# set-soft/ComfyUI-FLOAT_Optimized

Measured on AMD Instinct MI355X. Metric: 512x512 frames/sec end-to-end audio->video @50 ODE steps, higher is better.
Workload: dtype fp16; 1 GPU; configs[1]: 10 s audio + 512x512 portrait in HBM -> 250 frames in pinned host memory; appearance encoder + wav2vec2 audio encoder + FMT sampling (50 Euler evaluations/window, CFG a=2.0 e=1.0) + decode + D2H, through InferenceAgent.infer_device (the product call); nfe=51, frames_per_clip=250, fmt_dtype=fp16, dec_dtype=fp16, decode_batch=32, hip_graph=True, parallelism=replicas x1 (one clip per GPU), stage_overlap=off

## Files before the change

### comfyui-float_optimized_amd/csrc/fmt_api.hip

```cpp
#include <math.h>
#include <stdlib.h>

#include "fmt_gemm.hpp"
#include "fmt_kernels.hpp"
#include "fmt_rb_kernels.hpp"
#include "fmt_big_kernels.hpp"
#include "fmt_launch.hpp"

namespace {

struct Blk {
  Lin qkv, proj, fc1, fc2;
};

constexpr int kMaxTok = 80;
constexpr int kMaxSteps = 1024;

}

struct float_fmt {
  float_fmt_cfg_t cfg;
  DevicePool pool;
  int D, ntok, Mpad, Kc, Ntot, Kx;
  int Bmax = 1;
  Lin x_embed, t0, t2, c_embed, adaln_all, final_lin;
  std::vector<Blk> blk;
  float* pos = nullptr;
  float* freqs = nullptr;
  u16 *cond16, *sc16, *h16, *hfin16, *qkv16, *att16, *hid16, *xin16, *tsin16, *th16;
  float *ccond, *xres, *xcur, *temb, *vout;
  unsigned long long* sat = nullptr;
  float* slab = nullptr;
  float *wa_c, *we_c, *prev_x, *prev_wa, *prev_we, *x0_c;
  float* wr_c = nullptr;
  int method = 0;
  FmtTune tune;
  int n_cu = 0;
  struct MegaPlan {
    MegaStage* dev = nullptr;
    int nstage = 0, bc = 0, tried = 0;
    MegaCtx ctx{};
  } mega[5];
  unsigned* mega_sync = nullptr;
  unsigned* mega_err_host = nullptr;
  u16* mega_ws = nullptr;
  float* kbuf = nullptr;
  float* modall = nullptr;
  int Mmod = 0;
  size_t mod_zs = 0;
  struct GraphKey {
    int nfe, bc, we_len, method;
    int prio;
    float a, r, e;
    bool operator==(const GraphKey& o) const { return memcmp(this, &o, sizeof(GraphKey)) == 0; }
  };
  struct GraphEntry {
    GraphKey key;
    hipGraphExec_t exec[kFmtMaxClips + 1];
    uint64_t used;
  };
  std::vector<GraphEntry> graphs;
  uint64_t graph_clock = 0;
  hipStream_t cap_stream = nullptr;
  int cap_prio = 0;
  struct {
    const float *wr, *wa, *we, *noise;
    float* r_d;
    int T, we_len, nfe, include_r, next, n_chunks, B;
    int first = 0, total = 0;
    const float *hist_x = nullptr, *hist_wa = nullptr, *hist_we = nullptr;
    float a, r, e;
    std::vector<float> ts;
    bool active = false;
    bool ragged = false;
    FmtClipTab<const float*> rg_wr, rg_wa, rg_we, rg_noise;
    FmtClipTab<float*> rg_rd;
    int rg_win[kFmtMaxClips];
  } job;
};

#include "fmt_mega.hpp"

namespace {

int dev_copy2d(float* dst, size_t dpitch, const float* src, size_t spitch, int width, int rows, hipStream_t s) {
  if (width <= 0 || rows <= 0) return FLOAT_OK;
  hipLaunchKernelGGL(fmt_copy_kernel, dim3((unsigned)(((size_t)rows * width + 255) / 256)), dim3(256), 0, s, dst, dpitch, src, spitch, width, rows);
  FH_CHECK_HIP(hipGetLastError());
  return FLOAT_OK;
}
int dev_copy(float* dst, const float* src, size_t n, hipStream_t s) { return dev_copy2d(dst, n, src, n, (int)n, 1, s); }
int dev_zero(float* dst, size_t n, hipStream_t s) { return dev_copy2d(dst, n, nullptr, n, (int)n, 1, s); }
int copy_or_zero(float* dst, const float* src, size_t n, hipStream_t s) { return src ? dev_copy(dst, src, n, s) : dev_zero(dst, n, s); }

FmtLaunch launch_ctx(const float_fmt* h, hipStream_t s) {
  return FmtLaunch{h->tune, s, h->sat, h->xres, h->slab, h->h16, h->qkv16, h->att16, h->D, h->ntok, h->Ntot, h->Mpad, h->cfg.heads,
                   h->cfg.attn_window};
}


constexpr int kScSteps = 64;

static int stream_priority(hipStream_t s) {
  int prio = 0;
  if (hipStreamGetPriority(s, &prio) != hipSuccess) {
    (void)hipGetLastError();
    prio = 0;
  }
  return prio;
}

template <class T>
int run_mod_all(float_fmt* h, int M, int e0, int n, hipStream_t s) {
  const int D = h->D;
  const FmtTune& tn = h->tune;
  FH_REQUIRE(n >= 1 && n <= kScSteps, "modulation batch of %d evaluations (max %d)", n, kScSteps);
  const int prio = (s == h->cap_stream && s) ? h->cap_prio : stream_priority(s);
  const bool big = !T::is32 && tn.wide && prio == 0 && big_shape_ok(tn, n * M, h->adaln_all.N, h->adaln_all.K, h->n_cu);
  hipLaunchKernelGGL((fmt_silu_c_kernel<T>), dim3((M * D / 8 + 255) / 256, n), dim3(256), 0, s, h->sc16, h->temb + (size_t)e0 * D,
                     h->ccond, M, D, (size_t)h->Mpad * D, big ? M : 0, h->sat);
  h->mod_zs = big ? (size_t)M * h->Ntot : (size_t)h->Mmod * h->Ntot;
  if constexpr (!T::is32) {
    if (big) return launch_big4<T>(h->sc16, h->adaln_all, h->modall, n * M, h->Ntot, h->n_cu, s);
  }
  GemmArgs g = base_args(h->sc16, h->adaln_all, M);
  g.sat = h->sat, g.out_f32 = h->modall, g.ldo = h->Ntot, g.zcount = n;
  const bool dma = (tn.wide_variant == 6 || tn.wide_variant == 7) && (M + 15) / 16 > 4 && dma_shape_ok(g, 320);
  g.zgroup = tn.zgroup > 0 ? tn.zgroup : (dma ? 2 : 4);
  g.a_zstride = (size_t)h->Mpad * D;
  g.o_zstride = (size_t)h->Mmod * h->Ntot;
  if constexpr (!T::is32) {
    if (tn.wide && g.N % 128 == 0 && g.K % 128 == 0) return launch_wide<T>(g, tn.wide_variant, s);
  }
  for (int z = 0; z < n; ++z) {
    GemmArgs gz = g;
    gz.A = g.A + (size_t)z * g.a_zstride * (sizeof(typename T::elem) / sizeof(u16));
    gz.out_f32 = g.out_f32 + (size_t)z * g.o_zstride;
    gz.zcount = 0;
    int rc = run_gemm<T, EPI_F32>(tn, gz, s);
    if (rc) return rc;
  }
  return FLOAT_OK;
}

bool split_ok(int ks, const Lin& L) { return (ks == 1 || ks == 2 || ks == 4) && L.K % (128 * ks) == 0; }

template <class T>
int run_proj(const FmtLaunch& cx, const Blk& B, int M, const float* gate, const RbPlan& rb, PendingRed* pend) {
  const FmtTune& tn = cx.tn;
  const int hpw = attnproj_hpw(tn, cx.D, cx.heads);
  const int ks = rb.shape >= 0 ? rb.ksplit : (hpw ? cx.heads / hpw : (split_ok(tn.proj_split, B.proj) ? tn.proj_split : 0));
  int rc;
  if (rb.shape < 0 && hpw) {
    rc = launch_attnproj<T>(cx, M, B.proj);
  } else {
    launch_attn<T>(cx, M, (!ks && (tn.touch & 2)) ? &B.proj : nullptr);
    GemmArgs g = base_args(cx.att16, B.proj, M);
    if (rb.shape >= 0) {
      to_slab(g, cx.slab, cx.Mpad, ks);
      rc = launch_rbs<T, EPI_PARTIAL>(g, rb.shape, cx.s);
    } else if (ks) {
      rc = run_gemm_partial<T>(cx, g, ks);
    } else {
      g.sat = cx.sat, g.out_f32 = cx.xres, g.ldo = cx.D;
      g.gate = gate, g.ldg = cx.Ntot;
      if (tn.touch & 16) g.touch = make_touch(tn, B.fc1, M, 0, gemm_lanes_per_xcd(tn, M, g.N, g.K), 2);
      rc = run_gemm<T, EPI_GATE_RES>(tn, g, cx.s, false, &tn.plan_layer[RB_PROJ]);
    }
  }
  if (!rc && ks) *pend = pending_red(cx.slab, cx.Mpad, cx.D, B.proj.b, gate, ks);
  return rc;
}

template <class T>
int run_fc2(const FmtLaunch& cx, const Blk& B, const u16* hid16, int M, const float* gate, const RbPlan& rb, const Lin& after,
            int after_nt, PendingRed* pend) {
  const FmtTune& tn = cx.tn;
  const int ks = rb.shape >= 0 ? rb.ksplit : (split_ok(tn.fc2_split, B.fc2) ? tn.fc2_split : 0);
  GemmArgs g = base_args(hid16, B.fc2, M);
  int rc;
  if (rb.shape >= 0) {
    to_slab(g, cx.slab, cx.Mpad, ks);
    rc = launch_rbs<T, EPI_PARTIAL>(g, rb.shape, cx.s);
  } else if (ks) {
    g.sat = cx.sat;
    if (tn.touch & 32) g.touch = make_touch(tn, after, M, 0, gemm_lanes_per_xcd(tn, M, g.N * ks, g.K / ks), 2, after_nt);
    rc = run_gemm_partial<T>(cx, g, ks, &tn.plan_layer[RB_FC2]);
  } else {
    g.sat = cx.sat, g.out_f32 = cx.xres, g.ldo = cx.D;
    g.gate = gate, g.ldg = cx.Ntot;
    rc = run_gemm<T, EPI_GATE_RES>(tn, g, cx.s);
  }
  if (!rc && ks) *pend = pending_red(cx.slab, cx.Mpad, cx.D, B.fc2.b, gate, ks);
  return rc;
}

template <class T>
int run_blocks(float_fmt* h, int nclip, int bc, const float* modbuf, bool euler, float dt, float a, float r, float e, hipStream_t s,
               float* vout_to = nullptr) {
  const float_fmt_cfg_t& c = h->cfg;
  const FmtTune& tn = h->tune;
  const FmtLaunch cx = launch_ctx(h, s);
  const int D = h->D, ntok = h->ntok, M = nclip * bc * ntok;
  int rc;
  if constexpr (!T::is32) {
    if (bc <= 4 && mega_shape_ok<T>(h, nclip, bc)) {
      if (h->mega[bc].dev) return run_mega<T>(h, bc, modbuf, euler, dt, a, r, e, s, vout_to);
    }
  }
  {
    GemmArgs g = base_args(h->xin16, h->x_embed, nclip * ntok);
    g.sat = h->sat, g.out_f32 = h->xres, g.ldo = D;
    g.pos = h->pos, g.bc = bc, g.ntok = ntok;
    if ((rc = run_gemm<T, EPI_XEMBED>(tn, g, s))) return rc;
  }
  PendingRed pend;
  RbPlan rb_qkv, rb_proj, rb_fc1, rb_fc2;
  if constexpr (!T::is32) {
    rb_qkv = pick_rb(tn, RB_QKV, M), rb_proj = pick_rb(tn, RB_PROJ, M), rb_fc1 = pick_rb(tn, RB_FC1, M), rb_fc2 = pick_rb(tn, RB_FC2, M);
  }
  const int hpw = attnproj_hpw(tn, D, c.heads);
  for (int b = 0; b < c.depth; ++b) {
    const float* mod = modbuf + (size_t)b * 6 * D;
    const Blk& B = h->blk[b];
    const bool last = b + 1 == c.depth;
    if ((rc = launch_lnmod<T>(cx, M, mod, mod + D, &pend, &B.qkv, nullptr, 0, 128, rb_qkv.shape))) return rc;
    {
      GemmArgs g = base_args(h->h16, B.qkv, M);
      g.sat = h->sat, g.out16 = h->qkv16, g.ldo16 = 3 * D;
      if ((tn.touch & 8) && hpw) g.touch = make_touch(tn, B.proj, M, c.heads / hpw, gemm_lanes_per_xcd(tn, M, g.N, g.K), 2, 8 / hpw);
      else if ((tn.touch & 8) && !split_ok(tn.proj_split, B.proj)) g.touch = make_touch(tn, B.proj, M, 0, gemm_lanes_per_xcd(tn, M, g.N, g.K), 2);
      if (rb_qkv.shape >= 0) rc = launch_rbs<T, EPI_T16>(g, rb_qkv.shape, s);
      else rc = run_gemm<T, EPI_T16>(tn, g, s, false, &tn.plan_layer[RB_QKV]);
      if (rc) return rc;
    }
    if ((rc = run_proj<T>(cx, B, M, mod + 2 * D, rb_proj, &pend))) return rc;
    if ((rc = launch_lnmod<T>(cx, M, mod + 3 * D, mod + 4 * D, &pend, &B.fc1, nullptr, 0, 64, rb_fc1.shape))) return rc;
    {
      GemmArgs g = base_args(h->h16, B.fc1, M);
      g.sat = h->sat, g.out16 = h->hid16, g.ldo16 = B.fc2.K / 32;
      if ((tn.touch & 4) && rb_fc2.shape < 0)
        g.touch = make_touch(tn, B.fc2, M, split_ok(tn.fc2_split, B.fc2) ? tn.fc2_split : 0, gemm_lanes_per_xcd(tn, M, g.N, g.K), 2);
      if (rb_fc1.shape >= 0) rc = launch_rbs<T, EPI_GELU_P16>(g, rb_fc1.shape, s);
      else rc = run_gemm<T, EPI_GELU_P16>(tn, g, s, false, &tn.plan_layer[RB_FC1]);
      if (rc) return rc;
    }
    if ((rc = run_fc2<T>(cx, B, h->hid16, M, mod + 5 * D, rb_fc2, last ? h->final_lin : h->blk[b + 1].qkv, last ? 1 : 0, &pend))) return rc;
  }
  {
    const float* mod = modbuf + (size_t)c.depth * 6 * D;
    const bool tokblk = (!tn.no_tokblk || nclip > 1) && (bc == 1 || bc == 3 || bc == 4) && h->final_lin.K % 256 == 0;
    FH_REQUIRE(tokblk || nclip == 1, "batched sampling needs the token-blocked head GEMM");
    const int nblk = (ntok + 15) / 16, seqs = nclip * bc;
    if ((rc = launch_lnmod<T>(cx, M, mod, mod + D, &pend, nullptr, tokblk ? h->hfin16 : nullptr, tokblk ? seqs * 16 : 0))) return rc;
    GemmArgs g = base_args(tokblk ? h->hfin16 : h->h16, h->final_lin, tokblk ? nblk * seqs * 16 : M);
    g.sat = h->sat, g.tokblk = tokblk ? 1 : 0;
    g.nclip = nclip, g.bc = bc, g.ntok = ntok, g.n_prev = c.n_prev;
    g.a_cfg = a, g.r_cfg = r, g.e_cfg = e, g.dt = dt;
    if (euler) g.xcur = h->xcur, g.xin16 = h->xin16, g.ldx = h->Kx / 32;
    else g.vout = vout_to ? vout_to : h->vout;
    if (tokblk) rc = launch_gemm<T, EPI_CFG>(g, bc, 1, 8, s);
    else rc = run_gemm<T, EPI_CFG>(tn, g, s, true);
    if (rc) return rc;
  }
  FH_CHECK_HIP(hipGetLastError());
  return FLOAT_OK;
}

void linspace01(int n, std::vector<float>* ts) {
  ts->resize(n);
  if (n == 1) {
    (*ts)[0] = 0.f;
    return;
  }
  const float step = 1.0f / (float)(n - 1);
  const int half = n / 2;
  for (int i = 0; i < n; ++i) (*ts)[i] = (i < half) ? (0.f + step * (float)i) : (1.0f - step * (float)(n - 1 - i));
}

struct TimeSpec {
  float t;
  int nfe, stages;
  float c[4];
};
template <class T>
int prepare_time(float_fmt* h, const TimeSpec& ts, int n, hipStream_t s) {
  int rc;
  hipLaunchKernelGGL((fmt_tsin_kernel<T>), dim3(n), dim3(256), 0, s, h->tsin16, h->freqs, n, ts.t, ts.nfe, ts.stages, ts.c[0],
                     ts.c[1], ts.c[2], ts.c[3]);
  GemmArgs g = base_args(h->tsin16, h->t0, n);
  g.sat = h->sat, g.out16 = h->th16, g.ldo16 = h->t2.K / 32;
  if ((rc = launch_gemm<T, EPI_SILU_P16>(g, 4, 1, T::is32 ? 4 : pick_nw(g.K, 0), s))) return rc;
  GemmArgs g2 = base_args(h->th16, h->t2, n);
  g2.sat = h->sat, g2.out_f32 = h->temb, g2.ldo = h->D;
  if ((rc = launch_gemm<T, EPI_F32>(g2, 4, 1, T::is32 ? 4 : pick_nw(g2.K, 0), s))) return rc;
  return FLOAT_OK;
}

struct CfgMode {
  int bc;
  unsigned wr_mask, wa_mask, we_mask;
  int nclip = 1;
};

CfgMode cfg_mode(float a, float r, float e, int include_r) {
  if (a == 1.0f && r == 1.0f && e == 1.0f) return {1, 1u, 1u, 1u, 1};
  if (!include_r) return {3, 0b111u, 0b110u, 0b010u, 1};
  return {4, 0b1110u, 0b1100u, 0b0100u, 1};
}

template <class T>
int stage_window(float_fmt* h, const CfgMode& m, const float* x0, const float* wa, const float* wr, const float* we,
                 int we_len, const float* prev_x, const float* prev_wa, const float* prev_we, hipStream_t s) {
  const float_fmt_cfg_t& c = h->cfg;
  const int M = m.nclip * m.bc * h->ntok;
  hipLaunchKernelGGL((fmt_build_cond_kernel<T>), dim3(M), dim3(256), 0, s, h->cond16, h->Kc, m.bc, h->ntok, c.n_prev,
                     c.dim_w, c.dim_a, c.dim_e, wr, wa, prev_wa, we, we_len, prev_we, m.wr_mask, m.wa_mask, m.we_mask, h->sat);
  GemmArgs g = base_args(h->cond16, h->c_embed, M);
  g.sat = h->sat, g.out_f32 = h->ccond, g.ldo = h->D;
  int rc;
  if ((rc = run_gemm<T, EPI_F32>(h->tune, g, s))) return rc;
  const int n = m.nclip * h->ntok * c.dim_w;
  hipLaunchKernelGGL((fmt_init_x_kernel<T>), dim3((n + 255) / 256), dim3(256), 0, s, h->xcur, h->xin16, h->Kx / 32, x0, prev_x,
                     c.n_prev, c.n_cur, c.dim_w, m.nclip, h->sat);
  FH_CHECK_HIP(hipGetLastError());
  return FLOAT_OK;
}

int check_cfg_rows(const float_fmt* h, const CfgMode& m) {
  FH_REQUIRE(!h->tune.no_tokblk || m.bc * h->ntok <= 240,
             "%d-way CFG of %d tokens is %d rows; the all-rows CFG epilogue GEMM holds at most 240 (15 row tiles)", m.bc, h->ntok,
             m.bc * h->ntok);
  return FLOAT_OK;
}

int check_common(float_fmt* h, const void* we, int we_len, const void* prev_we) {
  FH_REQUIRE(h != nullptr, "null FMT handle");
  FH_REQUIRE(we_len == 1 || we_len == h->cfg.n_cur,
             "Dynamic emotion latent `we` time dimension (%d) does not match audio latent `wa` time dimension (%d).",
             we_len, h->cfg.n_cur);
  FH_REQUIRE(!(we_len > 1 && prev_we == nullptr),
             "`we` is dynamic (T>1), but prev_we was not provided with prev_x/prev_wa.");
  (void)we;
  return FLOAT_OK;
}

struct Tableau {
  int s;
  float c[4], a[4][3], b[4];
};
const Tableau& tableau(int method) {
  static const Tableau T[5] = {
      {1, {0.f}, {{0.f}}, {1.f}},
      {2, {0.f, 0.5f}, {{0.f}, {0.5f}}, {0.f, 1.f}},
      {4, {0.f, 1.f / 3, 2.f / 3, 1.f}, {{0.f}, {1.f / 3}, {-1.f / 3, 1.f}, {1.f, -1.f, 1.f}}, {0.125f, 0.375f, 0.375f, 0.125f}},
      {2, {0.f, 1.f}, {{0.f}, {1.f}}, {0.5f, 0.5f}},
      {3, {0.f, 1.f / 3, 2.f / 3}, {{0.f}, {1.f / 3}, {0.f, 2.f / 3}}, {0.25f, 0.f, 0.75f}},
  };
  return T[method];
}

TimeSpec time_spec(int method, int nfe) {
  const Tableau& tb = tableau(method);
  TimeSpec ts{};
  ts.nfe = nfe;
  ts.stages = tb.s;
  for (int j = 0; j < 4; ++j) ts.c[j] = tb.c[j];
  return ts;
}
int n_evals(int method, int nfe) { return (nfe - 1) * tableau(method).s; }

template <class T>
int run_window_steps(float_fmt* h, const CfgMode& m, int nfe, const std::vector<float>& ts, float a, float r, float e,
                     hipStream_t s) {
  const Tableau& tb = tableau(h->method);
  const float_fmt_cfg_t& c = h->cfg;
  const size_t kstride = (size_t)h->Bmax * kMaxTok * c.dim_w;
  const int n = m.nclip * c.n_cur * c.dim_w, rows = m.nclip * m.bc * h->ntok;
  const int nev = n_evals(h->method, nfe), batch = h->tune.hoist ? kScSteps : 1;
  const bool euler = h->method == FLOAT_ODE_EULER;
  int rc;
  for (int ev = 0; ev < nev; ++ev) {
    const int i = ev / tb.s, j = ev - i * tb.s, z = ev % batch;
    const float dt = ts[i + 1] - ts[i];
    if (z == 0 && (rc = run_mod_all<T>(h, rows, ev, std::min(batch, nev - ev), s))) return rc;
    const float* mod = h->modall + (size_t)z * h->mod_zs;
    if (euler) {
      if ((rc = run_blocks<T>(h, m.nclip, m.bc, mod, true, dt, a, r, e, s))) return rc;
      continue;
    }
    if (j > 0) {
      hipLaunchKernelGGL((fmt_rk_combine_kernel<T>), dim3((n + 255) / 256), dim3(256), 0, s, h->xcur, h->kbuf, kstride, j,
                         dt * tb.a[j][0], dt * tb.a[j][1], dt * tb.a[j][2], 0.f, 0, h->xin16, h->Kx / 32, c.n_prev, c.n_cur,
                         c.dim_w, m.nclip, h->sat);
    }
    if ((rc = run_blocks<T>(h, m.nclip, m.bc, mod, false, 0.f, a, r, e, s, h->kbuf + (size_t)j * kstride))) return rc;
    if (j == tb.s - 1) {
      hipLaunchKernelGGL((fmt_rk_combine_kernel<T>), dim3((n + 255) / 256), dim3(256), 0, s, h->xcur, h->kbuf, kstride, tb.s,
                         dt * tb.b[0], dt * tb.b[1], dt * tb.b[2], dt * tb.b[3], 1, h->xin16, h->Kx / 32, c.n_prev, c.n_cur,
                         c.dim_w, m.nclip, h->sat);
    }
  }
  FH_CHECK_HIP(hipGetLastError());
  return FLOAT_OK;
}

constexpr size_t kMaxGraphs = 8;
void destroy_graphs(float_fmt::GraphEntry& g) {
  for (hipGraphExec_t& e : g.exec)
    if (e) {
      (void)hipGraphExecDestroy(e);
      e = nullptr;
    }
}
template <class T>
int run_window_steps_graph(float_fmt* h, const CfgMode& m, int we_len, int nfe, const std::vector<float>& ts, float a,
                           float r, float e, hipStream_t s) {
  float_fmt::GraphKey key;
  memset(&key, 0, sizeof(key));
  key.nfe = nfe;
  key.method = h->method;
  key.bc = m.bc;
  key.we_len = we_len;
  key.a = a;
  key.r = r;
  key.e = e;
  key.prio = stream_priority(s);
  FH_REQUIRE(m.nclip >= 1 && m.nclip <= kFmtMaxClips, "chain of %d clips (max %d)", m.nclip, kFmtMaxClips);
  float_fmt::GraphEntry* hit = nullptr;
  for (auto& g : h->graphs)
    if (g.key == key) hit = &g;
  if (!hit || !hit->exec[m.nclip]) {
    if (!h->cap_stream) FH_CHECK_HIP(hipStreamCreateWithFlags(&h->cap_stream, hipStreamNonBlocking));
    hipGraph_t graph = nullptr;
    h->cap_prio = key.prio;
    FH_CHECK_HIP(hipStreamBeginCapture(h->cap_stream, hipStreamCaptureModeThreadLocal));
    int rc = run_window_steps<T>(h, m, nfe, ts, a, r, e, h->cap_stream);
    hipError_t ce = hipStreamEndCapture(h->cap_stream, &graph);
    if (rc) {
      if (graph) (void)hipGraphDestroy(graph);
      return rc;
    }
    FH_CHECK_HIP(ce);
    hipGraphExec_t exec = nullptr;
    FH_CHECK_HIP(hipGraphInstantiate(&exec, graph, nullptr, nullptr, 0));
    (void)hipGraphDestroy(graph);
    if (!hit) {
      if (h->graphs.size() >= kMaxGraphs) {
        size_t lru = 0;
        for (size_t i = 1; i < h->graphs.size(); ++i)
          if (h->graphs[i].used < h->graphs[lru].used) lru = i;
        hipError_t se = hipDeviceSynchronize();
        if (se != hipSuccess) {
          (void)hipGraphExecDestroy(exec);
          FH_CHECK_HIP(se);
        }
        destroy_graphs(h->graphs[lru]);
        h->graphs.erase(h->graphs.begin() + lru);
      }
      float_fmt::GraphEntry fresh;
      memset(&fresh, 0, sizeof(fresh));
      fresh.key = key;
      h->graphs.push_back(fresh);
      hit = &h->graphs.back();
    }
    hit->exec[m.nclip] = exec;
  }
  hit->used = ++h->graph_clock;
  FH_CHECK_HIP(hipGraphLaunch(hit->exec[m.nclip], s));
  return FLOAT_OK;
}

template <class T>
int window_impl(float_fmt* h, const float* x0, const float* wa, const float* wr, const float* we, int we_len,
                const float* prev_x, const float* prev_wa, const float* prev_we, int nfe, const std::vector<float>& ts,
                float a, float r, float e, int include_r, hipStream_t s, int nclip = 1) {
  CfgMode m = cfg_mode(a, r, e, include_r);
  m.nclip = nclip;
  int rc = check_cfg_rows(h, m);
  if (rc) return rc;
  if ((rc = stage_window<T>(h, m, x0, wa, wr, we, we_len, prev_x, prev_wa, prev_we, s))) return rc;
  if (nfe <= 1) return FLOAT_OK;
  hipStreamCaptureStatus cs = hipStreamCaptureStatusNone;
  if (hipStreamIsCapturing(s, &cs) != hipSuccess) {
    (void)hipGetLastError();
    cs = hipStreamCaptureStatusNone;
  }
  if (h->cfg.use_graph && !g_fh_profiling && cs == hipStreamCaptureStatusNone)
    return run_window_steps_graph<T>(h, m, we_len, nfe, ts, a, r, e, s);
  return run_window_steps<T>(h, m, nfe, ts, a, r, e, s);
}

template <class T>
int eval_impl(float_fmt* h, float t, const float* x, const float* wa, const float* wr, const float* we, int we_len,
              const float* prev_x, const float* prev_wa, const float* prev_we, float a, float r, float e, int include_r,
              float* out, hipStream_t s) {
  TimeSpec tsp{};
  tsp.t = t;
  int rc = prepare_time<T>(h, tsp, 1, s);
  if (rc) return rc;
  const CfgMode m = cfg_mode(a, r, e, include_r);
  if ((rc = check_cfg_rows(h, m))) return rc;
  if ((rc = stage_window<T>(h, m, x, wa, wr, we, we_len, prev_x, prev_wa, prev_we, s))) return rc;
  if ((rc = run_mod_all<T>(h, m.bc * h->ntok, 0, 1, s))) return rc;
  if ((rc = run_blocks<T>(h, 1, m.bc, h->modall, false, 0.f, a, r, e, s))) return rc;
  return dev_copy(out, h->vout, (size_t)h->ntok * h->cfg.dim_w, s);
}

template <class T>
int sample_window(float_fmt* h, int k, hipStream_t s) {
  const float_fmt_cfg_t& c = h->cfg;
  auto& J = h->job;
  const int L = c.n_cur, P = c.n_prev, Tn = J.T, B = J.B;
  const bool dynamic = J.we_len > 1;
  int rc;
  auto blocks = [](int n) { return dim3((n + 255) / 256); };
  if (k == J.first) {
    if ((rc = prepare_time<T>(h, time_spec(h->method, J.nfe), std::max(1, n_evals(h->method, J.nfe)), s))) return rc;
    if ((rc = copy_or_zero(h->prev_x, J.hist_x, (size_t)B * P * c.dim_w, s))) return rc;
    if ((rc = copy_or_zero(h->prev_wa, J.hist_wa, (size_t)B * P * c.dim_a, s))) return rc;
    if ((rc = copy_or_zero(h->prev_we, J.hist_we, (size_t)B * P * c.dim_e, s))) return rc;
  } else if (P > 0) {
    hipLaunchKernelGGL(fmt_tail_kernel, blocks(B * P * c.dim_w), dim3(256), 0, s, h->prev_x, h->xcur, P, L, c.dim_w, B);
    hipLaunchKernelGGL(fmt_tail_kernel, blocks(B * P * c.dim_a), dim3(256), 0, s, h->prev_wa, h->wa_c, P, L, c.dim_a, B);
    if (dynamic) hipLaunchKernelGGL(fmt_tail_kernel, blocks(B * P * c.dim_e), dim3(256), 0, s, h->prev_we, h->we_c, P, L, c.dim_e, B);
  }
  hipLaunchKernelGGL(fmt_slice_pad_kernel, blocks(B * L * c.dim_a), dim3(256), 0, s, h->wa_c, J.wa, k * L, Tn, L, c.dim_a, B);
  if (dynamic) hipLaunchKernelGGL(fmt_slice_pad_kernel, blocks(B * L * c.dim_e), dim3(256), 0, s, h->we_c, J.we, k * L, Tn, L, c.dim_e, B);
  if ((rc = dev_copy(h->x0_c, J.noise + (size_t)k * B * L * c.dim_w, (size_t)B * L * c.dim_w, s))) return rc;
  rc = window_impl<T>(h, h->x0_c, h->wa_c, J.wr, dynamic ? h->we_c : J.we, dynamic ? L : 1, h->prev_x, h->prev_wa,
                      dynamic ? h->prev_we : nullptr, J.nfe, J.ts, J.a, J.r, J.e, J.include_r, s, B);
  if (rc) return rc;
  const int rows = (k == J.total - 1) ? (Tn - k * L) : L;
  return dev_copy2d(J.r_d + (size_t)k * L * c.dim_w, (size_t)Tn * c.dim_w, h->xcur, (size_t)L * c.dim_w, rows * c.dim_w, B, s);
}

template <class T>
int sample_window_ragged(float_fmt* h, int k, hipStream_t s) {
  const float_fmt_cfg_t& c = h->cfg;
  auto& J = h->job;
  const int L = c.n_cur, P = c.n_prev;
  const bool dynamic = J.we_len > 1;
  int nact = 0;
  while (nact < J.B && J.rg_win[nact] > k) ++nact;
  int rc;
  auto blocks = [](int n) { return dim3((n + 255) / 256); };
  auto grid = [nact](int n) { return dim3((n + 255) / 256, nact); };
  if (k == 0) {
    if ((rc = prepare_time<T>(h, time_spec(h->method, J.nfe), std::max(1, n_evals(h->method, J.nfe)), s))) return rc;
    if ((rc = dev_zero(h->prev_x, (size_t)nact * P * c.dim_w, s))) return rc;
    if ((rc = dev_zero(h->prev_wa, (size_t)nact * P * c.dim_a, s))) return rc;
    if ((rc = dev_zero(h->prev_we, (size_t)nact * P * c.dim_e, s))) return rc;
    hipLaunchKernelGGL(fmt_gather_pad_kernel, grid(c.dim_w), dim3(256), 0, s, h->wr_c, J.rg_wr, 0, 1, c.dim_w);
    if (!dynamic) hipLaunchKernelGGL(fmt_gather_pad_kernel, grid(c.dim_e), dim3(256), 0, s, h->we_c, J.rg_we, 0, 1, c.dim_e);
  } else if (P > 0) {
    hipLaunchKernelGGL(fmt_tail_kernel, blocks(nact * P * c.dim_w), dim3(256), 0, s, h->prev_x, h->xcur, P, L, c.dim_w, nact);
    hipLaunchKernelGGL(fmt_tail_kernel, blocks(nact * P * c.dim_a), dim3(256), 0, s, h->prev_wa, h->wa_c, P, L, c.dim_a, nact);
    if (dynamic) hipLaunchKernelGGL(fmt_tail_kernel, blocks(nact * P * c.dim_e), dim3(256), 0, s, h->prev_we, h->we_c, P, L, c.dim_e, nact);
  }
  hipLaunchKernelGGL(fmt_gather_pad_kernel, grid(L * c.dim_a), dim3(256), 0, s, h->wa_c, J.rg_wa, k * L, L, c.dim_a);
  if (dynamic) hipLaunchKernelGGL(fmt_gather_pad_kernel, grid(L * c.dim_e), dim3(256), 0, s, h->we_c, J.rg_we, k * L, L, c.dim_e);
  hipLaunchKernelGGL(fmt_gather_pad_kernel, grid(L * c.dim_w), dim3(256), 0, s, h->x0_c, J.rg_noise, k * L, L, c.dim_w);
  FH_CHECK_HIP(hipGetLastError());
  rc = window_impl<T>(h, h->x0_c, h->wa_c, h->wr_c, h->we_c, dynamic ? L : 1, h->prev_x, h->prev_wa,
                      dynamic ? h->prev_we : nullptr, J.nfe, J.ts, J.a, J.r, J.e, J.include_r, s, nact);
  if (rc) return rc;
  hipLaunchKernelGGL(fmt_scatter_trim_kernel, grid(L * c.dim_w), dim3(256), 0, s, J.rg_rd, h->xcur, k * L, L, c.dim_w);
  FH_CHECK_HIP(hipGetLastError());
  return FLOAT_OK;
}

template <class T>
int create_impl(float_fmt* h, const TensorTable& tt) {
  const float_fmt_cfg_t& c = h->cfg;
  const int D = c.dim_h;
  int rc;
  prime_kernels<T>();
  auto pack = [&](const std::vector<std::string>& names, int N_each, int K, Lin* out) {
    return pack_linear_pool<T>(h->tune, &h->pool, tt, names, N_each, K, out);
  };
  if ((rc = pack({"x_embedder.proj"}, D, c.dim_w, &h->x_embed))) return rc;
  if ((rc = pack({"t_embedder.mlp.0"}, D, 256, &h->t0))) return rc;
  if ((rc = pack({"t_embedder.mlp.2"}, D, D, &h->t2))) return rc;
  if ((rc = pack({"c_embedder"}, D, c.dim_w + c.dim_a + c.dim_e, &h->c_embed))) return rc;
  h->blk.resize(c.depth);
  std::vector<std::string> ada;
  for (int b = 0; b < c.depth; ++b) {
    const std::string p = "blocks." + std::to_string(b) + ".";
    if ((rc = pack({p + "attn.qkv"}, 3 * D, D, &h->blk[b].qkv))) return rc;
    if ((rc = pack({p + "attn.proj"}, D, D, &h->blk[b].proj))) return rc;
    if ((rc = pack({p + "mlp.fc1"}, c.mlp_hidden, D, &h->blk[b].fc1))) return rc;
    if ((rc = pack({p + "mlp.fc2"}, D, c.mlp_hidden, &h->blk[b].fc2))) return rc;
    ada.push_back(p + "adaLN_modulation.1");
  }
  if ((rc = pack(ada, 6 * D, D, &h->adaln_all))) return rc;
  Lin tail;
  if ((rc = pack(std::vector<std::string>{"decoder.adaLN_modulation.1"}, 2 * D, D, &tail))) return rc;
  if ((rc = concat_linear_rows<T>(&h->pool, h->adaln_all, tail, &h->adaln_all))) return rc;
  if ((rc = pack({"decoder.linear"}, c.dim_w, D, &h->final_lin))) return rc;
  return FLOAT_OK;
}

}


int fmt_pack_linear(const FmtTune& tn, DevicePool* pool, int dtype, const TensorTable& tt, const std::vector<std::string>& names,
                    int N_each, int K, FmtLin* out) {
  FH_REQUIRE(dtype == FLOAT_DT_BF16 || dtype == FLOAT_DT_FP16 || dtype == FLOAT_DT_FP32, "the GEMM service: unknown dtype %d", dtype);
  return fmt_by_dtype(dtype, [&](auto t) { return pack_linear_pool<decltype(t)>(tn, pool, tt, names, N_each, K, out); });
}

int fmt_pack_linear_raw(const FmtTune& tn, DevicePool* pool, int dtype, const float* w, const float* b, int N, int K, FmtLin* out) {
  std::vector<float> zeros;
  if (!b) {
    zeros.assign(N, 0.f);
    b = zeros.data();
  }
  float_tensor_t t[2];
  memset(t, 0, sizeof(t));
  t[0].name = "raw.weight";
  t[0].data = w;
  t[0].ndim = 2;
  t[0].shape[0] = N;
  t[0].shape[1] = K;
  t[1].name = "raw.bias";
  t[1].data = b;
  t[1].ndim = 1;
  t[1].shape[0] = N;
  TensorTable tt(t, 2);
  return fmt_pack_linear(tn, pool, dtype, tt, {"raw"}, N, K, out);
}

GemmArgs fmt_gemm_args(const u16* A, const FmtLin& L, int M) { return base_args(A, L, M); }

void fmt_gemm_prime(int dtype) {
  fmt_by_dtype(dtype, [](auto t) { prime_kernels<decltype(t)>(); });
}

template <class T>
static int gemm_run_t(const FmtTune& tn, int epi, const GemmArgs& g, hipStream_t s) {
  switch (epi) {
    case EPI_F32: return run_gemm<T, EPI_F32>(tn, g, s);
    case EPI_T16: return run_gemm<T, EPI_T16>(tn, g, s);
    case EPI_SILU_P16: return run_gemm<T, EPI_SILU_P16>(tn, g, s);
    case EPI_GELU_P16: return run_gemm<T, EPI_GELU_P16>(tn, g, s);
    case EPI_GELUERF_P16: return run_gemm<T, EPI_GELUERF_P16>(tn, g, s);
    default: fh_set_error("fmt_gemm_run: epilogue %d is not exported", epi); return FLOAT_E_INVALID;
  }
}

int fmt_gemm_run(const FmtTune& tn, int dtype, int epi, GemmArgs g, hipStream_t s) {
  return fmt_by_dtype(dtype, [&](auto t) { return gemm_run_t<decltype(t)>(tn, epi, g, s); });
}

template <class T>
static int debug_impl(float_fmt* h, int what, const float* in, float* out, hipStream_t s) {
  const int D = h->D, ntok = h->ntok;
  if (what == 0) {
    return dev_copy(out, h->pos, (size_t)ntok * D, s);
  }
  if (what == 2) {
    FH_REQUIRE(h->mega_sync && h->mega[3].nstage > 0 && h->mega[3].nstage <= 64, "no persistent-kernel plan");
    FH_CHECK_HIP(hipStreamSynchronize(s));
    const int n = h->mega[3].nstage * 3;
    std::vector<unsigned long long> st(n);
    FH_CHECK_HIP(hipMemcpy(st.data(), h->mega_sync + 20 * 32, n * 8, hipMemcpyDeviceToHost));
    std::vector<float> us(n);
    for (int i = 0; i < n; ++i) us[i] = st[i] ? (float)((double)(st[i] - st[0]) * 0.01) : -1.f;
    FH_CHECK_HIP(hipMemcpy(out, us.data(), n * 4, hipMemcpyHostToDevice));
    return FLOAT_OK;
  }
  FH_REQUIRE(what == 1 && in != nullptr, "float_fmt_debug: unknown request %d (or null input)", what);
  const int n = ntok * 3 * D;
  hipLaunchKernelGGL((fmt_dbg_to16_kernel<T>), dim3((n + 255) / 256), dim3(256), 0, s, h->qkv16, in, n);
  launch_attn<T>(launch_ctx(h, s), ntok, nullptr);
  hipLaunchKernelGGL((fmt_dbg_unpack_kernel<T>), dim3((ntok * D + 255) / 256), dim3(256), 0, s, out, h->att16, ntok, D);
  FH_CHECK_HIP(hipGetLastError());
  return FLOAT_OK;
}

static int drain_job(float_fmt_t* h, void* stream) {
  int32_t left = 1;
  while (left > 0)
    if (int rc = float_fmt_sample_next(h, stream, nullptr, &left)) return rc;
  return FLOAT_OK;
}

extern "C" {

int float_fmt_create(const float_fmt_cfg_t* cfg, const float_tensor_t* tensors, int32_t n_tensors, float_fmt_t** out) {
  FH_REQUIRE(cfg && tensors && out, "null argument to float_fmt_create");
  FH_REQUIRE(cfg->dim_h % 256 == 0 && cfg->dim_h / 256 <= 8 && ((cfg->dim_h / 256) & (cfg->dim_h / 256 - 1)) == 0,
             "dim_h=%d unsupported", cfg->dim_h);
  FH_REQUIRE(cfg->dim_h / cfg->heads == 128, "head_dim must be 128 (dim_h=%d heads=%d)", cfg->dim_h, cfg->heads);
  FH_REQUIRE(cfg->dim_w % 128 == 0 && cfg->mlp_hidden % 128 == 0, "dim_w / mlp_hidden must be multiples of 128");
  FH_REQUIRE(cfg->n_prev + cfg->n_cur <= kMaxTok, "at most %d tokens per window (got %d)", kMaxTok, cfg->n_prev + cfg->n_cur);
  FH_REQUIRE(cfg->n_prev >= 0 && cfg->n_prev <= cfg->n_cur, "n_prev must be in [0, n_cur]");
  FH_REQUIRE(cfg->dtype == FLOAT_DT_BF16 || cfg->dtype == FLOAT_DT_FP16 || cfg->dtype == FLOAT_DT_FP32, "unknown dtype %d", cfg->dtype);
  FH_REQUIRE(cfg->max_batch >= 0 && cfg->max_batch <= 16, "max_batch must be in [0, 16] (got %d)", cfg->max_batch);
  float_fmt* h = new float_fmt();
  h->tune = FmtTune::from_env();
  h->cfg = *cfg;
  h->D = cfg->dim_h;
  h->ntok = cfg->n_prev + cfg->n_cur;
  h->Bmax = cfg->max_batch > 0 ? cfg->max_batch : 1;
  h->Mpad = 16 * ((h->Bmax * 4 * h->ntok + 15) / 16 + 12);
  h->Kc = round_up(cfg->dim_w + cfg->dim_a + cfg->dim_e, 128);
  h->Kx = round_up(cfg->dim_w, 128);
  {
    int dev = 0, ncu = 0;
    if (hipGetDevice(&dev) == hipSuccess && hipDeviceGetAttribute(&ncu, hipDeviceAttributeMultiprocessorCount, dev) == hipSuccess) h->n_cu = ncu;
    else (void)hipGetLastError();
  }
  h->Ntot = cfg->depth * 6 * h->D + 2 * h->D;
  TensorTable tt(tensors, n_tensors);
  int rc = fmt_by_dtype(cfg->dtype, [&](auto t) { return create_impl<decltype(t)>(h, tt); });
  const int D = h->D, Mp = h->Mpad;
  const size_t esz = cfg->dtype == FLOAT_DT_FP32 ? 2 : 1;
  auto A = [&](auto** p, size_t n) {
    if (!rc) rc = h->pool.alloc(p, std::is_same<std::remove_reference_t<decltype(**p)>, u16>::value ? n * esz : n, true);
  };
  A(&h->pos, (size_t)kMaxTok * D);
  A(&h->freqs, 128);
  A(&h->cond16, (size_t)Mp * h->Kc);
  A(&h->sc16, (size_t)kScSteps * Mp * D + (size_t)12 * 16 * D);
  A(&h->h16, (size_t)Mp * D);
  A(&h->hfin16, (size_t)h->Bmax * 64 * ((kMaxTok + 15) / 16) * D);
  A(&h->qkv16, (size_t)Mp * 3 * D);
  A(&h->att16, (size_t)Mp * D);
  A(&h->hid16, (size_t)Mp * cfg->mlp_hidden);
  A(&h->xin16, (size_t)(h->Bmax * kMaxTok + 6 * 16) * h->Kx);
  A(&h->tsin16, (size_t)kMaxSteps * 256);
  A(&h->th16, (size_t)kMaxSteps * D);
  A(&h->ccond, (size_t)Mp * D);
  h->Mmod = 16 * ((h->Bmax * 4 * h->ntok + 15) / 16);
  if (!rc) rc = h->pool.alloc(&h->modall, (size_t)kScSteps * h->Mmod * h->Ntot, false);
  A(&h->kbuf, (size_t)4 * h->Bmax * kMaxTok * cfg->dim_w);
  A(&h->xres, (size_t)Mp * D);
  A(&h->slab, (size_t)8 * Mp * D);
  A(&h->sat, 1);
  A(&h->xcur, (size_t)h->Bmax * cfg->n_cur * cfg->dim_w);
  A(&h->temb, (size_t)kMaxSteps * D);
  A(&h->vout, (size_t)h->Bmax * kMaxTok * cfg->dim_w);
  A(&h->wa_c, (size_t)h->Bmax * cfg->n_cur * cfg->dim_a);
  A(&h->we_c, (size_t)h->Bmax * cfg->n_cur * cfg->dim_e);
  A(&h->x0_c, (size_t)h->Bmax * cfg->n_cur * cfg->dim_w);
  A(&h->wr_c, (size_t)h->Bmax * cfg->dim_w);
  A(&h->prev_x, (size_t)h->Bmax * cfg->n_cur * cfg->dim_w);
  A(&h->prev_wa, (size_t)h->Bmax * cfg->n_cur * cfg->dim_a);
  A(&h->prev_we, (size_t)h->Bmax * cfg->n_cur * cfg->dim_e);
  if (!rc) {
    std::vector<float> pos((size_t)h->ntok * D);
    const float_tensor_t* pe = tt.find("pos_embed");
    if (pe && TensorTable::numel(pe) == (int64_t)h->ntok * D) {
      memcpy(pos.data(), pe->data, pos.size() * sizeof(float));
    } else {
      for (int p = 0; p < h->ntok; ++p)
        for (int j = 0; j < D; ++j) {
          const float ang = (float)((double)p / pow(10000.0, 2.0 * (double)(j / 2) / (double)D));
          pos[(size_t)p * D + j] = (j & 1) ? cosf(ang) : sinf(ang);
        }
    }
    std::vector<float> fr(128);
    for (int k = 0; k < 128; ++k) fr[k] = expf(-logf(10000.0f) * (float)k / 128.0f);
    if (hipMemcpy(h->pos, pos.data(), pos.size() * sizeof(float), hipMemcpyHostToDevice) != hipSuccess ||
        hipMemcpy(h->freqs, fr.data(), fr.size() * sizeof(float), hipMemcpyHostToDevice) != hipSuccess) {
      fh_set_error("hipMemcpy of FMT tables failed");
      rc = FLOAT_E_HIP;
    }
  }
  if (!rc) rc = fmt_by_dtype(cfg->dtype, [&](auto t) { return prepare_mega<decltype(t)>(h, 3); });
  if (rc) {
    float_fmt_destroy(h);
    return rc;
  }
  *out = h;
  return FLOAT_OK;
}

void float_fmt_destroy(float_fmt_t* h) {
  if (!h) return;
  for (auto& g : h->graphs) destroy_graphs(g);
  if (h->cap_stream) (void)hipStreamDestroy(h->cap_stream);
  if (h->mega_err_host) (void)hipHostFree(h->mega_err_host);
  h->pool.release();
  delete h;
}

int float_fmt_eval(float_fmt_t* h, float t, const float* x, const float* wa, const float* wr, const float* we,
                   int32_t we_len, const float* prev_x, const float* prev_wa, const float* prev_we, float a_cfg,
                   float r_cfg, float e_cfg, int32_t include_r_cfg, float* out, void* stream) {
  int rc = check_common(h, we, we_len, prev_we);
  if (rc) return rc;
  if ((rc = mega_poll(h))) return rc;
  FH_REQUIRE(x && wa && wr && we && prev_x && prev_wa && out, "null tensor argument to float_fmt_eval");
  hipStream_t s = (hipStream_t)stream;
  return fmt_by_dtype(h->cfg.dtype, [&](auto tag) {
    return eval_impl<decltype(tag)>(h, t, x, wa, wr, we, we_len, prev_x, prev_wa, prev_we, a_cfg, r_cfg, e_cfg, include_r_cfg, out, s);
  });
}

int float_fmt_sample_chunk(float_fmt_t* h, const float* x0, const float* wa, const float* wr, const float* we,
                           int32_t we_len, const float* prev_x, const float* prev_wa, const float* prev_we, int32_t nfe,
                           float a_cfg, float r_cfg, float e_cfg, int32_t include_r_cfg, float* out, void* stream) {
  int rc = check_common(h, we, we_len, prev_we);
  if (rc) return rc;
  if ((rc = mega_poll(h))) return rc;
  FH_REQUIRE(x0 && wa && wr && we && prev_x && prev_wa && out, "null tensor argument to float_fmt_sample_chunk");
  FH_REQUIRE(nfe >= 1 && n_evals(h->method, nfe) < kMaxSteps, "nfe=%d: too many evaluations (max %d)", nfe, kMaxSteps);
  hipStream_t s = (hipStream_t)stream;
  std::vector<float> ts;
  linspace01(nfe, &ts);
  const float_fmt_cfg_t& c = h->cfg;
  if ((rc = dev_copy(h->x0_c, x0, (size_t)c.n_cur * c.dim_w, s))) return rc;
  if ((rc = dev_copy(h->wa_c, wa, (size_t)c.n_cur * c.dim_a, s))) return rc;
  if ((rc = dev_copy(h->prev_x, prev_x, (size_t)c.n_prev * c.dim_w, s))) return rc;
  if ((rc = dev_copy(h->prev_wa, prev_wa, (size_t)c.n_prev * c.dim_a, s))) return rc;
  if (we_len > 1) {
    if ((rc = dev_copy(h->we_c, we, (size_t)c.n_cur * c.dim_e, s))) return rc;
    if ((rc = dev_copy(h->prev_we, prev_we, (size_t)c.n_prev * c.dim_e, s))) return rc;
  }
  const float* we_p = we_len > 1 ? h->we_c : we;
  const float* pwe_p = we_len > 1 ? h->prev_we : nullptr;
  const TimeSpec tsp = time_spec(h->method, nfe);
  const int nev = std::max(1, n_evals(h->method, nfe));
  rc = fmt_by_dtype(c.dtype, [&](auto t) {
    typedef decltype(t) T;
    if (int prc = prepare_time<T>(h, tsp, nev, s)) return prc;
    return window_impl<T>(h, h->x0_c, h->wa_c, wr, we_p, we_len, h->prev_x, h->prev_wa, pwe_p, nfe, ts, a_cfg, r_cfg, e_cfg,
                          include_r_cfg, s);
  });
  if (rc) return rc;
  return dev_copy(out, h->xcur, (size_t)c.n_cur * c.dim_w, s);
}

int float_fmt_debug(float_fmt_t* h, int32_t what, const float* in, float* out, void* stream) {
  FH_REQUIRE(h != nullptr && out != nullptr, "null argument to float_fmt_debug");
  return fmt_by_dtype(h->cfg.dtype, [&](auto t) { return debug_impl<decltype(t)>(h, what, in, out, (hipStream_t)stream); });
}

int float_fmt_saturation(float_fmt_t* h, uint64_t* total, int32_t reset, void* stream) {
  FH_REQUIRE(h && total, "null argument to float_fmt_saturation");
  FH_CHECK_HIP(hipStreamSynchronize((hipStream_t)stream));
  unsigned long long v = 0;
  FH_CHECK_HIP(hipMemcpy(&v, h->sat, sizeof(v), hipMemcpyDeviceToHost));
  *total = v;
  if (reset) {
    FH_CHECK_HIP(hipMemsetAsync(h->sat, 0, sizeof(v), (hipStream_t)stream));
    FH_CHECK_HIP(hipStreamSynchronize((hipStream_t)stream));
  }
  if (int rc = mega_poll(h)) return rc;
  return FLOAT_OK;
}

int float_fmt_set_method(float_fmt_t* h, int32_t method) {
  FH_REQUIRE(h != nullptr, "null FMT handle");
  FH_REQUIRE(method >= FLOAT_ODE_EULER && method <= FLOAT_ODE_HEUN3, "unknown ODE method %d", method);
  h->method = method;
  return FLOAT_OK;
}

int float_fmt_sample_begin(float_fmt_t* h, const float* wr, const float* wa, int32_t T, const float* we, int32_t we_len,
                           const float* noise, int32_t nfe, float a_cfg, float r_cfg, float e_cfg, int32_t include_r_cfg,
                           float* r_d) {
  FH_REQUIRE(h != nullptr, "null FMT handle");
  FH_REQUIRE(wr && wa && we && noise && r_d, "null tensor argument to float_fmt_sample");
  FH_REQUIRE(T >= 1, "T must be >= 1 (got %d)", T);
  FH_REQUIRE(we_len == 1 || we_len == T,
             "Dynamic emotion latent `we` time dimension (%d) does not match audio latent `wa` time dimension (%d).",
             we_len, T);
  FH_REQUIRE(nfe >= 1 && n_evals(h->method, nfe) < kMaxSteps, "nfe=%d: too many evaluations (max %d)", nfe, kMaxSteps);
  auto& J = h->job;
  J.wr = wr;
  J.wa = wa;
  J.we = we;
  J.noise = noise;
  J.r_d = r_d;
  J.T = T;
  J.we_len = we_len;
  J.nfe = nfe;
  J.include_r = include_r_cfg;
  J.a = a_cfg;
  J.r = r_cfg;
  J.e = e_cfg;
  J.B = 1;
  J.ragged = false;
  J.next = 0;
  J.n_chunks = (T + h->cfg.n_cur - 1) / h->cfg.n_cur;
  J.first = 0;
  J.total = J.n_chunks;
  J.hist_x = J.hist_wa = J.hist_we = nullptr;
  linspace01(nfe, &J.ts);
  J.active = true;
  return FLOAT_OK;
}

int float_fmt_sample_begin_range(float_fmt_t* h, const float* wr, const float* wa, int32_t T, const float* we, int32_t we_len,
                                 const float* noise, int32_t nfe, float a_cfg, float r_cfg, float e_cfg, int32_t include_r_cfg,
                                 float* r_d, int32_t first_window, int32_t end_window, const float* hist_x, const float* hist_wa,
                                 const float* hist_we) {
  int rc = float_fmt_sample_begin(h, wr, wa, T, we, we_len, noise, nfe, a_cfg, r_cfg, e_cfg, include_r_cfg, r_d);
  if (rc) return rc;
  auto& J = h->job;
  J.active = false;
  FH_REQUIRE(first_window >= 0 && first_window < end_window && end_window <= J.total,
             "window range [%d, %d) outside the clip's %d windows", first_window, end_window, J.total);
  FH_REQUIRE(we_len == 1 || hist_we != nullptr || hist_x == nullptr,
             "a dynamic-emotion job that starts from a history needs hist_we too");
  J.first = J.next = first_window;
  J.n_chunks = end_window;
  J.hist_x = hist_x;
  J.hist_wa = hist_wa;
  J.hist_we = we_len > 1 ? hist_we : nullptr;
  J.active = true;
  return FLOAT_OK;
}

int float_fmt_sample_next(float_fmt_t* h, void* stream, int32_t* window_done, int32_t* windows_left) {
  FH_REQUIRE(h != nullptr && h->job.active, "float_fmt_sample_next without float_fmt_sample_begin");
  if (int prc = mega_poll(h)) return prc;
  auto& J = h->job;
  hipStream_t s = (hipStream_t)stream;
  const int k = J.next;
  int rc = fmt_by_dtype(h->cfg.dtype, [&](auto t) {
    return J.ragged ? sample_window_ragged<decltype(t)>(h, k, s) : sample_window<decltype(t)>(h, k, s);
  });
  if (rc) {
    J.active = false;
    return rc;
  }
  J.next = k + 1;
  if (window_done) *window_done = k;
  if (windows_left) *windows_left = J.n_chunks - J.next;
  if (J.next >= J.n_chunks) J.active = false;
  return FLOAT_OK;
}

int float_fmt_sample_batch(float_fmt_t* h, int32_t n_clips, const float* wr, const float* wa, int32_t T, const float* we,
                           int32_t we_len, const float* noise, int32_t nfe, float a_cfg, float r_cfg, float e_cfg,
                           int32_t include_r_cfg, float* r_d, void* stream) {
  FH_REQUIRE(h != nullptr, "null FMT handle");
  FH_REQUIRE(n_clips >= 1 && n_clips <= h->Bmax, "batch of %d clips, the handle was created with max_batch = %d", n_clips, h->Bmax);
  int rc = float_fmt_sample_begin(h, wr, wa, T, we, we_len, noise, nfe, a_cfg, r_cfg, e_cfg, include_r_cfg, r_d);
  if (rc) return rc;
  h->job.B = n_clips;
  return drain_job(h, stream);
}

int float_fmt_sample_begin_ragged(float_fmt_t* h, int32_t n_clips, const int32_t* T, const float* const* wr,
                                  const float* const* wa, const float* const* we, int32_t we_dynamic,
                                  const float* const* noise, int32_t nfe, float a_cfg, float r_cfg, float e_cfg,
                                  int32_t include_r_cfg, float* const* r_d) {
  FH_REQUIRE(h != nullptr, "null FMT handle");
  FH_REQUIRE(T && wr && wa && we && noise && r_d, "null array argument to float_fmt_sample_begin_ragged");
  FH_REQUIRE(n_clips >= 1 && n_clips <= h->Bmax, "batch of %d clips, the handle was created with max_batch = %d", n_clips, h->Bmax);
  for (int i = 0; i < n_clips; ++i) {
    FH_REQUIRE(wr[i] && wa[i] && we[i] && noise[i] && r_d[i], "null tensor argument to float_fmt_sample_begin_ragged (clip %d)", i);
    FH_REQUIRE(T[i] >= 1, "T must be >= 1 (got %d for clip %d)", T[i], i);
  }
  FH_REQUIRE(nfe >= 1 && n_evals(h->method, nfe) < kMaxSteps, "nfe=%d: too many evaluations (max %d)", nfe, kMaxSteps);
  auto& J = h->job;
  J.active = false;
  const int L = h->cfg.n_cur;
  int order[kFmtMaxClips];
  for (int i = 0; i < n_clips; ++i) order[i] = i;
  std::stable_sort(order, order + n_clips, [&](int x, int y) { return (T[x] + L - 1) / L > (T[y] + L - 1) / L; });
  memset(&J.rg_wr, 0, sizeof(J.rg_wr));
  memset(&J.rg_wa, 0, sizeof(J.rg_wa));
  memset(&J.rg_we, 0, sizeof(J.rg_we));
  memset(&J.rg_noise, 0, sizeof(J.rg_noise));
  memset(&J.rg_rd, 0, sizeof(J.rg_rd));
  for (int q = 0; q < n_clips; ++q) {
    const int i = order[q], Ti = T[i], win = (Ti + L - 1) / L;
    J.rg_win[q] = win;
    J.rg_wr.p[q] = wr[i], J.rg_wr.T[q] = 1;
    J.rg_wa.p[q] = wa[i], J.rg_wa.T[q] = Ti;
    J.rg_we.p[q] = we[i], J.rg_we.T[q] = we_dynamic ? Ti : 1;
    J.rg_noise.p[q] = noise[i], J.rg_noise.T[q] = win * L;
    J.rg_rd.p[q] = r_d[i], J.rg_rd.T[q] = Ti;
  }
  J.wr = J.wa = J.we = J.noise = nullptr;
  J.r_d = nullptr;
  J.T = 0;
  J.we_len = we_dynamic ? L : 1;
  J.nfe = nfe;
  J.include_r = include_r_cfg;
  J.a = a_cfg;
  J.r = r_cfg;
  J.e = e_cfg;
  J.B = n_clips;
  J.ragged = true;
  J.next = J.first = 0;
  J.n_chunks = J.total = J.rg_win[0];
  J.hist_x = J.hist_wa = J.hist_we = nullptr;
  linspace01(nfe, &J.ts);
  J.active = true;
  return FLOAT_OK;
}

int float_fmt_sample_batch_ragged(float_fmt_t* h, int32_t n_clips, const int32_t* T, const float* const* wr,
                                  const float* const* wa, const float* const* we, int32_t we_dynamic,
                                  const float* const* noise, int32_t nfe, float a_cfg, float r_cfg, float e_cfg,
                                  int32_t include_r_cfg, float* const* r_d, void* stream) {
  int rc = float_fmt_sample_begin_ragged(h, n_clips, T, wr, wa, we, we_dynamic, noise, nfe, a_cfg, r_cfg, e_cfg, include_r_cfg, r_d);
  if (rc) return rc;
  return drain_job(h, stream);
}

int float_fmt_sample(float_fmt_t* h, const float* wr, const float* wa, int32_t T, const float* we, int32_t we_len,
                     const float* noise, int32_t nfe, float a_cfg, float r_cfg, float e_cfg, int32_t include_r_cfg,
                     float* r_d, void* stream) {
  int rc = float_fmt_sample_begin(h, wr, wa, T, we, we_len, noise, nfe, a_cfg, r_cfg, e_cfg, include_r_cfg, r_d);
  if (rc) return rc;
  return drain_job(h, stream);
}

}
```

### comfyui-float_optimized_amd/csrc/fmt_kernels.hpp

```cpp
#pragma once
#include "common.hpp"
#include "fmt_pack.hpp"

template <class T, int MTW, int NT, int NW, int EPI, bool COH>
__device__ __forceinline__ void fmt_gemm_body(const GemmArgs& g, const unsigned bid, const unsigned nblk) {
  constexpr int BN = NT * 16;
  constexpr int ROWS = MTW * 16;
  constexpr bool WT = NW >= 8 || COH;
  auto ldA = [](const typename T::elem* p) -> typename T::pack8 { return T::load8(p); };
  constexpr int NTHR = NW * 64;
  constexpr int PF = T::is32 ? 1 : ((MTW + NT <= 7) ? 4 : ((MTW + NT <= 8) ? 3 : 2));
  typedef typename T::elem E;
  typedef typename T::pack8 P8;
  extern __shared__ __attribute__((aligned(16))) float red[];
  const int lane = threadIdx.x & 63;
  const int w = threadIdx.x >> 6;
  const int r16 = lane & 15, q = lane >> 4;
  int bx, by, ks = 0;
  {
    const int nbn = g.N / BN, id = (int)bid;
    const int nbx = (EPI == EPI_PARTIAL) ? nbn * g.ksplit : nbn;
    if ((nbx & 7) == 0) {
      const int slot = id >> 3;
      by = slot % g.mblk;
      bx = (slot / g.mblk) * 8 + (id & 7);
    } else {
      bx = id % nbx;
      by = id / nbx;
    }
    if constexpr (EPI == EPI_PARTIAL) {
      if ((nbx & 7) == 0 && (8 % g.ksplit) == 0) {
        const int P = 8 / g.ksplit, x = bx & 7;
        ks = x / P;
        bx = (bx >> 3) * P + (x % P);
      } else {
        ks = bx / nbn;
        bx = bx % nbn;
      }
    }
  }
  const int nb0 = bx * NT;
  const int mt0 = by * MTW;
  const int n0 = nb0 * 16, m0 = mt0 * 16;

  f32x4 acc[MTW][NT];
#pragma unroll
  for (int i = 0; i < MTW; ++i)
#pragma unroll
    for (int j = 0; j < NT; ++j) acc[i][j] = f32x4{0.f, 0.f, 0.f, 0.f};

  const int KB = g.K >> 5;
  const int KBs = (EPI == EPI_PARTIAL) ? KB / g.ksplit : KB;
  const int KBw = KBs / NW;
  const E* Ap = reinterpret_cast<const E*>(g.A) + ((size_t)mt0 * KB + ks * KBs + w * KBw) * 512 + lane * 8;
  const E* Wp = reinterpret_cast<const E*>(g.W) + ((size_t)nb0 * KB + ks * KBs + w * KBw) * 512 + lane * 8;
  const size_t tstride = (size_t)KB * 512;
  constexpr bool kEarlyRes = (EPI == EPI_GATE_RES) && (MTW * 16 * (NT * 2) <= NW * 64);
  float4 res_pf[2], gate_pf[2];
  if constexpr (kEarlyRes) {
    const int r = threadIdx.x / (NT * 2), cg = threadIdx.x % (NT * 2);
    const int row = m0 + r, nb = n0 + cg * 8;
    if (r < ROWS && row < g.M) {
      const float* o = g.out_f32 + (size_t)row * g.ldo + nb;
      const float* gt = g.gate + (size_t)row * g.ldg + nb;
      res_pf[0] = fh_load_f4<COH>(o);
      res_pf[1] = fh_load_f4<COH>(o + 4);
      gate_pf[0] = fh_load_f4_stream(gt);
      gate_pf[1] = fh_load_f4_stream(gt + 4);
    }
  }

  P8 a[PF][MTW], b[PF][NT];
#pragma unroll
  for (int p = 0; p < PF; ++p) {
    if (p < KBw) {
#pragma unroll
      for (int j = 0; j < NT; ++j) b[p][j] = T::load8_nt(Wp + j * tstride + (size_t)p * 512);
#pragma unroll
      for (int i = 0; i < MTW; ++i) a[p][i] = ldA(Ap + i * tstride + (size_t)p * 512);
    }
  }
  constexpr bool kTouch = (EPI == EPI_GELU_P16 || EPI == EPI_T16 || EPI == EPI_GATE_RES || EPI == EPI_PARTIAL);
  unsigned touched[2] = {0u, 0u};
  if constexpr (kTouch) {
    if (g.touch.W) fmt_touch(g.touch, bid & 7, (bid >> 3) * NTHR + threadIdx.x, (nblk >> 3) * NTHR, touched);
  }
  for (int kb0 = 0; kb0 < KBw; kb0 += PF) {
#pragma unroll
    for (int p = 0; p < PF; ++p) {
      const int kb = kb0 + p;
      if (kb < KBw) {
#pragma unroll
        for (int i = 0; i < MTW; ++i)
#pragma unroll
          for (int j = 0; j < NT; ++j) acc[i][j] = T::mfma(a[p][i], b[p][j], acc[i][j]);
        if (kb + PF < KBw) {
#pragma unroll
          for (int j = 0; j < NT; ++j)
            b[p][j] = T::load8_nt(Wp + j * tstride + (size_t)(kb + PF) * 512);
#pragma unroll
          for (int i = 0; i < MTW; ++i) a[p][i] = ldA(Ap + i * tstride + (size_t)(kb + PF) * 512);
        }
      }
    }
  }

  if constexpr (kTouch) {
    if (g.touch.W) fmt_touch_retire(touched);
  }
  float* my = red + w * (ROWS * BN);
#pragma unroll
  for (int i = 0; i < MTW; ++i)
#pragma unroll
    for (int j = 0; j < NT; ++j)
#pragma unroll
      for (int r = 0; r < 4; ++r) my[(i * 16 + q * 4 + r) * BN + j * 16 + r16] = acc[i][j][r];
  __syncthreads();

  constexpr int S = ROWS * BN;
  constexpr int CG = BN / 8;
  unsigned rm = 0u;
  auto slab_sum = [&](int o) {
    float a = red[o];
#pragma unroll
    for (int ww = 1; ww < NW; ++ww) a += red[ww * S + o];
    return a;
  };
  if constexpr (EPI == EPI_CFG) {
    const int nclip = g.nclip > 1 ? g.nclip : 1;
    const int tb = g.tokblk ? by / nclip : 0, q = g.tokblk ? by - tb * nclip : 0;
    const int ni = g.tokblk ? 16 : g.ntok, i0 = tb * 16, rstride = g.tokblk ? 16 : g.ntok;
    float* const vout_q = g.vout ? g.vout + (size_t)q * g.ntok * g.N : nullptr;
    float* const xcur_q = g.xcur ? g.xcur + (size_t)q * (g.ntok - g.n_prev) * g.N : nullptr;
    for (int idx = threadIdx.x; idx < ni * BN; idx += NTHR) {
      const int il = idx / BN, i = i0 + il, c = idx % BN, n = n0 + c;
      if (i >= g.ntok) break;
      const float bias = g.bias[n];
      float v[4];
#pragma unroll
      for (int b2 = 0; b2 < 4; ++b2) {
        if (b2 < g.bc) {
          const int o = (b2 * rstride + il) * BN + c;
          v[b2] = slab_sum(o) + bias;
        } else {
          v[b2] = 0.f;
        }
      }
      float out;
      if (g.bc == 1) {
        out = v[0];
      } else if (g.bc == 3) {
        out = v[0] + g.a_cfg * (v[2] - v[0]) + g.e_cfg * (v[1] - v[2]);
      } else {
        out = v[0] + g.r_cfg * (v[1] - v[0]) + g.a_cfg * (v[3] - v[1]) + g.e_cfg * (v[2] - v[3]);
      }
      if (vout_q) vout_q[(size_t)i * g.N + n] = out;
      if (xcur_q && i >= g.n_prev) {
        const size_t xo = (size_t)(i - g.n_prev) * g.N + n;
        const float xn = xcur_q[xo] + g.dt * out;
        xcur_q[xo] = xn;
        reinterpret_cast<E*>(g.xin16)[fmt_pack_off(q * g.ntok + i, n, g.ldx)] = fh_cvt<T>(xn, rm);
      }
    }
  } else {
    for (int idx = threadIdx.x; idx < ROWS * CG; idx += NTHR) {
      const int r = idx / CG, cg = idx % CG;
      const int row = m0 + r, nb = n0 + cg * 8;
      if (row >= g.M) continue;
      float v[8];
      {
        const float* p0 = red + r * BN + cg * 8;
#pragma unroll
        for (int e = 0; e < 8; e += 4) {
          float4 a4 = *reinterpret_cast<const float4*>(p0 + e);
#pragma unroll
          for (int ww = 1; ww < NW; ++ww) {
            const float4 t4 = *reinterpret_cast<const float4*>(p0 + ww * S + e);
            a4.x += t4.x;
            a4.y += t4.y;
            a4.z += t4.z;
            a4.w += t4.w;
          }
          float4 bb = float4{0.f, 0.f, 0.f, 0.f};
          if constexpr (EPI != EPI_PARTIAL) bb = *reinterpret_cast<const float4*>(g.bias + nb + e);
          v[e + 0] = a4.x + bb.x;
          v[e + 1] = a4.y + bb.y;
          v[e + 2] = a4.z + bb.z;
          v[e + 3] = a4.w + bb.w;
        }
      }
      if constexpr (EPI == EPI_F32 || EPI == EPI_PARTIAL) {
        float* o = g.out_f32 + (size_t)ks * g.slab_stride + (size_t)row * g.ldo + nb;
        fh_store_f4_wt<fh_site<COH>(4), WT>(o, float4{v[0], v[1], v[2], v[3]});
        fh_store_f4_wt<fh_site<COH>(4), WT>(o + 4, float4{v[4], v[5], v[6], v[7]});
      } else if constexpr (EPI == EPI_T16 || EPI == EPI_SILU_P16 || EPI == EPI_GELU_P16 || EPI == EPI_GELUERF_P16) {
        P8 u;
#pragma unroll
        for (int i = 0; i < 8; ++i) {
          float x = v[i];
          if constexpr (EPI == EPI_SILU_P16) x = fh_silu(x);
          if constexpr (EPI == EPI_GELU_P16) x = fh_gelu_tanh(x);
          if constexpr (EPI == EPI_GELUERF_P16) x = fh_gelu_erf(x);
          T::set(u, i, x);
        }
        fh_track_pack<T>(rm, u);
        E* const o16 = reinterpret_cast<E*>(g.out16);
        if constexpr (EPI == EPI_T16) T::template store8_wt<fh_site<COH>(8), WT>(o16 + (size_t)row * g.ldo16 + nb, u);
        else T::template store8_wt<fh_site<COH>(8), WT>(o16 + fmt_pack_off(row, nb, g.ldo16), u);
      } else if constexpr (EPI == EPI_GATE_RES) {
        float* o = g.out_f32 + (size_t)row * g.ldo + nb;
        const float* gt = g.gate + (size_t)row * g.ldg + nb;
#pragma unroll
        for (int e = 0; e < 8; e += 4) {
          float4 x, gg;
          if constexpr (kEarlyRes) {
            x = res_pf[e / 4];
            gg = gate_pf[e / 4];
          } else {
            x = fh_load_f4<COH>(o + e);
            gg = fh_load_f4_stream(gt + e);
          }
          x.x += gg.x * v[e + 0];
          x.y += gg.y * v[e + 1];
          x.z += gg.z * v[e + 2];
          x.w += gg.w * v[e + 3];
          fh_store_f4_wt<fh_site<COH>(16), WT>(o + e, x);
        }
      } else if constexpr (EPI == EPI_XEMBED) {
        const int q = row / g.ntok, tok = row - q * g.ntok;
        const float* ps = g.pos + (size_t)tok * g.N + nb;
#pragma unroll
        for (int i = 0; i < 8; ++i) v[i] += ps[i];
        for (int b2 = 0; b2 < g.bc; ++b2) {
          float* o = g.out_f32 + (size_t)((q * g.bc + b2) * g.ntok + tok) * g.ldo + nb;
          fh_store_f4_wt<fh_site<COH>(32), WT>(o, float4{v[0], v[1], v[2], v[3]});
          fh_store_f4_wt<fh_site<COH>(32), WT>(o + 4, float4{v[4], v[5], v[6], v[7]});
        }
      }
    }
  }
  if constexpr (EPI == EPI_CFG || EPI == EPI_T16 || EPI == EPI_SILU_P16 || EPI == EPI_GELU_P16 || EPI == EPI_GELUERF_P16) fh_range_flush<T>(g.sat, rm);
}

template <class T, int MTW, int NT, int NW, int EPI>
__global__ __launch_bounds__(NW * 64) void fmt_gemm_kernel(GemmArgs g) {
  fmt_gemm_body<T, MTW, NT, NW, EPI, false>(g, blockIdx.x, gridDim.x);
}

template <class T, int MTW, int KCH , int NWV = 4>
__global__ __launch_bounds__(NWV * 64) void fmt_gemm_wide_kernel(GemmArgs g) {
  constexpr int EPI = EPI_F32;
  constexpr int NF = MTW * KCH;
  constexpr int NFW = (NF + NWV - 1) / NWV;
  constexpr int WR = NWV / 4, MTR = MTW / WR;
  static_assert(MTW % WR == 0, "row tiles must split evenly over the wave rows");
  extern __shared__ __attribute__((aligned(16))) unsigned char sA[];
  const int lane = threadIdx.x & 63, w = threadIdx.x >> 6, wc = w & 3, wr = w >> 2;
  const int r16 = lane & 15, q = lane >> 4;
  const int nbn = g.N >> 7;
  const int nbx = (EPI == EPI_PARTIAL) ? nbn * g.ksplit : nbn;
  int bx, by, bz = 0, ks = 0;
  {
    const int id = blockIdx.x;
    const int nz = g.zcount > 1 ? g.zcount : 1;
    if (nz > 1 && (nbx & 7) == 0 && g.zgroup > 1) {
      const int slot = id >> 3, G = g.zgroup, ncx = nbx >> 3, rows = g.mblk * nz;
      const int full = ncx / G, per_grp = G * rows;
      int grp = slot / per_grp, rem = slot - grp * per_grp, gw = G;
      if (grp >= full) {
        grp = full;
        rem = slot - full * per_grp;
        gw = ncx - full * G;
      }
      const int zy = rem / gw;
      bz = zy / g.mblk;
      by = zy - bz * g.mblk;
      bx = (grp * G + (rem - zy * gw)) * 8 + (id & 7);
    } else if ((nbx & 7) == 0) {
      const int slot = id >> 3, zy = slot % (g.mblk * nz);
      bz = zy / g.mblk;
      by = zy - bz * g.mblk;
      bx = (slot / (g.mblk * nz)) * 8 + (id & 7);
    } else {
      bx = id % nbx;
      const int zy = id / nbx;
      bz = zy / g.mblk;
      by = zy - bz * g.mblk;
    }
    if constexpr (EPI == EPI_PARTIAL) {
      if ((nbx & 7) == 0 && (8 % g.ksplit) == 0) {
        const int P = 8 / g.ksplit, x = bx & 7;
        ks = x / P;
        bx = (bx >> 3) * P + (x % P);
      } else {
        ks = bx / nbn;
        bx = bx % nbn;
      }
    }
  }
  const int mt0 = by * MTW;
  const int nb0 = bx * 8 + wc * 2;
  const int KB = g.K >> 5;
  const int KBs = (EPI == EPI_PARTIAL) ? KB / g.ksplit : KB;
  const int nchunk = KBs / KCH;
  const size_t tstride = (size_t)KB * 512;
  const u16* Wp = g.W + (size_t)nb0 * tstride + (size_t)ks * KBs * 512 + lane * 8;
  const u16* Ag = g.A + (size_t)bz * g.a_zstride + (size_t)mt0 * tstride + (size_t)ks * KBs * 512 + lane * 8;
  float* const outz = g.out_f32 + (size_t)bz * g.o_zstride + (size_t)ks * g.slab_stride;

  f32x4 acc[MTR][2];
#pragma unroll
  for (int i = 0; i < MTR; ++i) acc[i][0] = acc[i][1] = f32x4{0.f, 0.f, 0.f, 0.f};

  u32x4 an[NFW], bn[KCH][2], bc[KCH][2];
  auto issue = [&](int c) {
    const int kc = c * KCH;
#pragma unroll
    for (int f = 0; f < NFW; ++f) {
      const int fi = f * NWV + w;
      if (fi < NF) {
        const int i = fi / KCH, kk = fi % KCH;
        an[f] = *reinterpret_cast<const u32x4*>(Ag + i * tstride + (size_t)(kc + kk) * 512);
      }
    }
#pragma unroll
    for (int kk = 0; kk < KCH; ++kk) {
      bn[kk][0] = __builtin_nontemporal_load(reinterpret_cast<const u32x4*>(Wp + (size_t)(kc + kk) * 512));
      bn[kk][1] = __builtin_nontemporal_load(reinterpret_cast<const u32x4*>(Wp + tstride + (size_t)(kc + kk) * 512));
    }
  };
  auto commit = [&](int buf) {
#pragma unroll
    for (int f = 0; f < NFW; ++f) {
      const int fi = f * NWV + w;
      if (fi < NF) *reinterpret_cast<u32x4*>(sA + (buf * NF + fi) * 1024 + lane * 16) = an[f];
    }
#pragma unroll
    for (int kk = 0; kk < KCH; ++kk) {
      bc[kk][0] = bn[kk][0];
      bc[kk][1] = bn[kk][1];
    }
  };
  issue(0);
  commit(0);
  __syncthreads();
  for (int c = 0; c < nchunk; ++c) {
    const int buf = c & 1;
    if (c + 1 < nchunk) issue(c + 1);
#pragma unroll
    for (int kk = 0; kk < KCH; ++kk) {
#pragma unroll
      for (int i = 0; i < MTR; ++i) {
        const u32x4 a = *reinterpret_cast<const u32x4*>(sA + (buf * NF + (wr * MTR + i) * KCH + kk) * 1024 + lane * 16);
        acc[i][0] = T::mfma(bc[kk][0], a, acc[i][0]);
        acc[i][1] = T::mfma(bc[kk][1], a, acc[i][1]);
      }
    }
    if (c + 1 < nchunk) {
      commit(buf ^ 1);
      __syncthreads();
    }
  }
#pragma unroll
  for (int i = 0; i < MTR; ++i) {
    const int row = (mt0 + wr * MTR + i) * 16 + r16;
    if (row >= g.M) continue;
#pragma unroll
    for (int j = 0; j < 2; ++j) {
      const int n = (nb0 + j) * 16 + q * 4;
      float4 o = float4{acc[i][j][0], acc[i][j][1], acc[i][j][2], acc[i][j][3]};
      if constexpr (EPI != EPI_PARTIAL) {
        const float4 bb = *reinterpret_cast<const float4*>(g.bias + n);
        o.x += bb.x;
        o.y += bb.y;
        o.z += bb.z;
        o.w += bb.w;
      }
      if constexpr (EPI == EPI_F32 || EPI == EPI_PARTIAL) {
        *reinterpret_cast<float4*>(outz + (size_t)row * g.ldo + n) = o;
      } else if constexpr (EPI == EPI_T16) {
        T::store4(g.out16 + (size_t)row * g.ldo16 + n, o.x, o.y, o.z, o.w);
      } else {
        static_assert(EPI == EPI_GELU_P16, "epilogue not built for the wide GEMM");
        T::store4(g.out16 + fmt_pack_off(row, n, g.ldo16), fh_gelu_tanh(o.x), fh_gelu_tanh(o.y), fh_gelu_tanh(o.z), fh_gelu_tanh(o.w));
      }
    }
  }
}

template <int OFF>
__device__ __forceinline__ u32x4 fh_ds_read128(unsigned addr) {
  u32x4 v;
  asm volatile("ds_read_b128 %0, %1 offset:%2" : "=v"(v) : "v"(addr), "n"(OFF));
  return v;
}
template <int N>
__device__ __forceinline__ void fh_wait_vmcnt() {
  asm volatile("s_waitcnt vmcnt(%0)" ::"n"(N) : "memory");
}

template <class T, int NWC , int NS ,
          int STG >
__global__ __launch_bounds__(NWC * 128) void fmt_gemm_dma_kernel(GemmArgs g) {
  constexpr int RT = 12, CT = 5 * NWC, NF = RT + CT, NW = 2 * NWC, STAGE = NF * 1024;
  constexpr int IMAX = (NF + NW - 1) / NW, ILO = NF / NW, NHI = NF % NW;
  static_assert(NS >= 3 && NS <= 4, "ring of 3 or 4 stages");
  extern __shared__ __attribute__((aligned(1024))) unsigned char ring[];
  const int lane = threadIdx.x & 63, w = threadIdx.x >> 6, wr = w / NWC, wc = w % NWC;
  const int r16 = lane & 15, q = lane >> 4;
  const int nbx = g.N / (CT * 16);
  int bx, by, bz;
  {
    const int id = blockIdx.x, nz = g.zcount > 1 ? g.zcount : 1;
    if ((nbx & 7) == 0 && g.zgroup > 1) {
      const int slot = id >> 3, G = g.zgroup, ncx = nbx >> 3, rows = g.mblk * nz;
      const int full = ncx / G, per_grp = G * rows;
      int grp = slot / per_grp, rem = slot - grp * per_grp, gw = G;
      if (grp >= full) {
        grp = full;
        rem = slot - full * per_grp;
        gw = ncx - full * G;
      }
      const int zy = rem / gw;
      bz = zy / g.mblk;
      by = zy - bz * g.mblk;
      bx = (grp * G + (rem - zy * gw)) * 8 + (id & 7);
    } else {
      bx = id % nbx;
      const int zy = id / nbx;
      bz = zy / g.mblk;
      by = zy - bz * g.mblk;
    }
  }
  const int KB = g.K >> 5;
  const size_t tstride = (size_t)KB * 512;
  const u16* src[IMAX];
#pragma unroll
  for (int i = 0; i < IMAX; ++i) {
    const int fi = min(w + NW * i, NF - 1);
    src[i] = (fi < RT ? g.A + (size_t)bz * g.a_zstride + (size_t)(by * RT + fi) * tstride
                      : g.W + (size_t)(bx * CT + fi - RT) * tstride) + lane * 8;
  }
  auto issue = [&](int s) {
    unsigned char* dst = ring + (s % NS) * STAGE + w * 1024;
#pragma unroll
    for (int i = 0; i < IMAX; ++i)
      if (i < ILO || w < NHI)
        __builtin_amdgcn_global_load_lds((const __attribute__((address_space(1))) void*)(src[i] + (size_t)s * 512),
                                         (__attribute__((address_space(3))) void*)(dst + i * NW * 1024), 16, 0, 0);
  };
#define DMA_WAIT(K)                                   \
  do {                                                \
    if (NHI == 0 || w < NHI) fh_wait_vmcnt<(K)*IMAX>(); \
    else fh_wait_vmcnt<(K)*ILO>();                    \
  } while (0)
  const unsigned abase = (unsigned)(lane * 16 + wr * 6 * 1024), bbase = (unsigned)(lane * 16 + (RT + wc * 5) * 1024);

  f32x4 acc[6][5];
#pragma unroll
  for (int i = 0; i < 6; ++i)
#pragma unroll
    for (int j = 0; j < 5; ++j) acc[i][j] = f32x4{0.f, 0.f, 0.f, 0.f};
  u32x4 a0[6], b0[5], a1[6], b1[5];

#define DMA_READ(S, AR, BR)                                        \
  do {                                                             \
    const unsigned so = (unsigned)(((S) % NS) * STAGE);            \
    AR[0] = fh_ds_read128<0>(abase + so);                          \
    AR[1] = fh_ds_read128<1024>(abase + so);                       \
    AR[2] = fh_ds_read128<2048>(abase + so);                       \
    AR[3] = fh_ds_read128<3072>(abase + so);                       \
    AR[4] = fh_ds_read128<4096>(abase + so);                       \
    AR[5] = fh_ds_read128<5120>(abase + so);                       \
    BR[0] = fh_ds_read128<0>(bbase + so);                          \
    BR[1] = fh_ds_read128<1024>(bbase + so);                       \
    BR[2] = fh_ds_read128<2048>(bbase + so);                       \
    BR[3] = fh_ds_read128<3072>(bbase + so);                       \
    BR[4] = fh_ds_read128<4096>(bbase + so);                       \
  } while (0)
#define DMA_STEP(S, AC, BC, AN, BN)                                                            \
  do {                                                                                         \
    const int s_ = (S);                                                                        \
    if (s_ + 1 < KB) {                                                                         \
      const int rem = KB - 2 - s_;                               \
      if (NS == 4 && rem >= 2) DMA_WAIT(2);                                                    \
      else if (rem >= 1) DMA_WAIT(1);                                                          \
      else DMA_WAIT(0);                                                                        \
    }                                                                                          \
    __builtin_amdgcn_s_barrier();                                                              \
    if (s_ + NS < KB) issue(s_ + NS);                                                          \
    if (s_ + 1 < KB) DMA_READ(s_ + 1, AN, BN);                                                 \
    __builtin_amdgcn_sched_barrier(0);                                                         \
    _Pragma("unroll") for (int i = 0; i < 6; ++i)                                              \
      _Pragma("unroll") for (int j = 0; j < 5; ++j) acc[i][j] = T::mfma(BC[j], AC[i], acc[i][j]); \
    __builtin_amdgcn_sched_barrier(0);                                                         \
    asm volatile("s_waitcnt lgkmcnt(0)" ::: "memory");                                         \
    __builtin_amdgcn_sched_barrier(0);                                                         \
  } while (0)

#define DMA_WAIT_UPTO(K)                      \
  do {                                        \
    const int k_ = (K);                       \
    if (NS == 4 && k_ >= 2) DMA_WAIT(2);      \
    else if (k_ >= 1) DMA_WAIT(1);            \
    else DMA_WAIT(0);                         \
  } while (0)
#define DMA_STEP_STG(S, AC, BC, AN, BN)                                                        \
  do {                                                                                         \
    const int s_ = (S);                                                                        \
    if (!g1 && s_ + 1 < KB) DMA_WAIT_UPTO(KB - 2 - s_);                                        \
    __builtin_amdgcn_s_barrier();                                                              \
    if (s_ + NS < KB) issue(s_ + NS);                                                          \
    if (s_ + 1 < KB) DMA_READ(s_ + 1, AN, BN);                                                 \
    asm volatile("s_waitcnt lgkmcnt(0)" ::: "memory");                                         \
    __builtin_amdgcn_sched_barrier(0);                                                         \
    if (g1 && s_ + 2 < KB) {                                                                   \
      DMA_WAIT_UPTO(KB - 3 - s_);                                                              \
    }                                                                                          \
    __builtin_amdgcn_s_barrier();                                                              \
    __builtin_amdgcn_sched_barrier(0);                                                         \
    _Pragma("unroll") for (int i = 0; i < 6; ++i)                                              \
      _Pragma("unroll") for (int j = 0; j < 5; ++j) acc[i][j] = T::mfma(BC[j], AC[i], acc[i][j]); \
    __builtin_amdgcn_sched_barrier(0);                                                         \
  } while (0)

  const bool g1 = wr == 1;
#ifdef DMA_CLK
  const unsigned long long c0 = clock64(), w0 = wall_clock64();
#endif
#pragma unroll
  for (int s = 0; s < NS; ++s) issue(s);
  if constexpr (STG) DMA_WAIT(NS - 2);
  else DMA_WAIT(NS - 1);
  __builtin_amdgcn_s_barrier();
  DMA_READ(0, a0, b0);
  asm volatile("s_waitcnt lgkmcnt(0)" ::: "memory");
  __builtin_amdgcn_sched_barrier(0);
  if constexpr (STG) {
    if (g1) __builtin_amdgcn_s_barrier();
    for (int s = 0; s < KB; s += 2) {
      DMA_STEP_STG(s, a0, b0, a1, b1);
      DMA_STEP_STG(s + 1, a1, b1, a0, b0);
    }
    if (!g1) __builtin_amdgcn_s_barrier();
  } else {
    for (int s = 0; s < KB; s += 2) {
      DMA_STEP(s, a0, b0, a1, b1);
      DMA_STEP(s + 1, a1, b1, a0, b0);
    }
  }
#ifdef DMA_CLK
  if ((blockIdx.x == 3000 || blockIdx.x == 6001) && threadIdx.x == 0) {
    const unsigned long long c1 = clock64(), w1 = wall_clock64();
    printf("tile loop: %llu core clocks, %llu wall ticks\n", c1 - c0, w1 - w0);
  }
#endif
#undef DMA_STEP_STG
#undef DMA_WAIT_UPTO
#undef DMA_STEP
#undef DMA_READ
#undef DMA_WAIT
  float* const outz = g.out_f32 + (size_t)bz * g.o_zstride;
  constexpr int OW = CT * 16, OSTR = OW + 4, C4 = OW / 4, NTHR = NW * 64;
  static_assert(96 * OSTR * 4 <= NS * STAGE, "output staging does not fit the ring");
  float* const so = reinterpret_cast<float*>(ring);
  float4 bb[5];
#pragma unroll
  for (int j = 0; j < 5; ++j) bb[j] = *reinterpret_cast<const float4*>(g.bias + (bx * CT + wc * 5 + j) * 16 + q * 4);
#pragma unroll
  for (int p = 0; p < 2; ++p) {
    if (wr == p) {
#pragma unroll
      for (int i = 0; i < 6; ++i)
#pragma unroll
        for (int j = 0; j < 5; ++j)
          *reinterpret_cast<float4*>(so + (i * 16 + r16) * OSTR + (wc * 5 + j) * 16 + q * 4) =
              float4{acc[i][j][0] + bb[j].x, acc[i][j][1] + bb[j].y, acc[i][j][2] + bb[j].z, acc[i][j][3] + bb[j].w};
    }
    __syncthreads();
    {
#pragma unroll
      for (int k = 0; k < (96 * C4) / NTHR; ++k) {
        const int idx = k * NTHR + threadIdx.x, rl = idx / C4, c4 = idx - rl * C4;
        const int row = by * (RT * 16) + p * 96 + rl;
        if (row < g.M)
          *reinterpret_cast<float4*>(outz + (size_t)row * g.ldo + bx * OW + c4 * 4) = *reinterpret_cast<const float4*>(so + rl * OSTR + c4 * 4);
      }
    }
    if (p == 0) __syncthreads();
  }
}

struct LnRed {
  const float* slab;
  size_t slab_stride;
  const float* bias;
  const float* gate;
};

constexpr int kLnTouch = 6;

template <class T, int NV, int KS, bool TOUCH, bool WT_, bool COH>
__device__ __forceinline__ void fmt_lnmod_body(float* __restrict__ x, int M, const float* __restrict__ shift,
                                               const float* __restrict__ scale, int ldm, u16* __restrict__ out, const LnRed& red,
                                               const TouchSpec& pf, int ntok, int perm, unsigned long long* sat, const unsigned bid,
                                               const unsigned nblk, const int wpb) {
  constexpr int D = NV * 256;
  constexpr bool WT = WT_ || COH;
  const int lane = threadIdx.x & 63;
  int row = bid * wpb + (threadIdx.x >> 6);
  unsigned touched[kLnTouch] = {};
  const unsigned tfirst = (bid >> 3) * 64 + lane, tstride = (nblk >> 3) * 64;
  const bool touch = TOUCH && wpb == 1;
  if (wpb == 1) {
    const int x = bid & 7, j = bid >> 3;
    row = (((j >> 3) * 8 + x) << 3) + (j & 7);
  }
  if (row >= M) {
    if (touch) {
      fmt_touch(pf, bid & 7, tfirst, tstride, touched);
      fmt_touch_retire(touched);
    }
    return;
  }
  float* xr = x + (size_t)row * D;
#ifdef FMT_DIAG_HOTMOD
  const size_t mrow = 0;
#else
  const size_t mrow = (size_t)row;
#endif
  const float* sh = shift + mrow * ldm;
  const float* sc = scale + mrow * ldm;
  float4 v[NV], a[NV], b[NV];
  float s = 0.f;
#pragma unroll
  for (int i = 0; i < NV; ++i) {
    const int c = i * 256 + lane * 4;
    v[i] = fh_load_f4<COH>(xr + c);
    a[i] = fh_load_f4_stream(sh + c);
    b[i] = fh_load_f4_stream(sc + c);
  }
  if (KS == 0 && touch) fmt_touch(pf, bid & 7, tfirst, tstride, touched);
  if constexpr (KS > 0) {
    float4 p[KS][NV], gt[NV], bi[NV];
#pragma unroll
    for (int i = 0; i < NV; ++i) {
      const int c = i * 256 + lane * 4;
#pragma unroll
      for (int k = 0; k < KS; ++k) {
        const float* ps = red.slab + k * red.slab_stride + (size_t)row * D + c;
        if constexpr (COH) p[k][i] = fh_load_f4<true>(ps);
        else p[k][i] = fh_load_f4_stream(ps);
      }
      gt[i] = fh_load_f4_stream(red.gate + mrow * ldm + c);
      bi[i] = *reinterpret_cast<const float4*>(red.bias + c);
    }
    if (touch) fmt_touch(pf, bid & 7, tfirst, tstride, touched);
#pragma unroll
    for (int i = 0; i < NV; ++i) {
      float4 t = p[0][i];
#pragma unroll
      for (int k = 1; k < KS; ++k) {
        t.x += p[k][i].x;
        t.y += p[k][i].y;
        t.z += p[k][i].z;
        t.w += p[k][i].w;
      }
      v[i].x += gt[i].x * (t.x + bi[i].x);
      v[i].y += gt[i].y * (t.y + bi[i].y);
      v[i].z += gt[i].z * (t.z + bi[i].z);
      v[i].w += gt[i].w * (t.w + bi[i].w);
      fh_store_f4_wt<fh_site<COH>(1), WT>(xr + i * 256 + lane * 4, v[i]);
    }
  }
#pragma unroll
  for (int i = 0; i < NV; ++i) s += (v[i].x + v[i].y) + (v[i].z + v[i].w);
  const float mu = wave_sum(s) * (1.f / D);
  float s2 = 0.f;
#pragma unroll
  for (int i = 0; i < NV; ++i) {
    const float d0 = v[i].x - mu, d1 = v[i].y - mu, d2 = v[i].z - mu, d3 = v[i].w - mu;
    s2 += (d0 * d0 + d1 * d1) + (d2 * d2 + d3 * d3);
  }
  const float rstd = rsqrtf(wave_sum(s2) * (1.f / D) + 1e-6f);
  unsigned rm = 0u;
  int orow = row;
  if (perm) {
    const int b = row / ntok, i = row - b * ntok;
    orow = (i >> 4) * perm + b * 16 + (i & 15);
  }
#pragma unroll
  for (int i = 0; i < NV; ++i) {
    const int c = i * 256 + lane * 4;
    fh_store4_wt<T, fh_site<COH>(1), WT>(reinterpret_cast<typename T::elem*>(out) + fmt_pack_off(orow, c, D / 32),
              (v[i].x - mu) * rstd * (1.f + b[i].x) + a[i].x, (v[i].y - mu) * rstd * (1.f + b[i].y) + a[i].y,
              (v[i].z - mu) * rstd * (1.f + b[i].z) + a[i].z, (v[i].w - mu) * rstd * (1.f + b[i].w) + a[i].w, rm);
  }
  fh_range_flush<T>(sat, rm);
  if (touch) fmt_touch_retire(touched);
}

template <class T, int NV, int KS, bool TOUCH, bool WT>
__global__ __launch_bounds__(256) void fmt_lnmod_kernel(float* __restrict__ x, int M, const float* __restrict__ shift,
                                                        const float* __restrict__ scale, int ldm, u16* __restrict__ out,
                                                        LnRed red, TouchSpec pf, int ntok, int perm, unsigned long long* sat) {
  fmt_lnmod_body<T, NV, KS, TOUCH, WT, false>(x, M, shift, scale, ldm, out, red, pf, ntok, perm, sat, blockIdx.x, gridDim.x,
                                              (int)(blockDim.x >> 6));
}

template <class T, int LPQ, bool TOUCH, bool WT_, bool COH>
__device__ __forceinline__ void fmt_attn_body(const u16* __restrict__ qkv, int ld, u16* __restrict__ out, int ntok, int M, int D,
                                              int window, const TouchSpec& pf, unsigned long long* sat, const int h, const int run,
                                              const int nthr, const unsigned lin, const unsigned nwg) {
  constexpr int HD = 128, PD = HD / LPQ, NU = PD / 8;
  constexpr bool WT = WT_ || COH;
  auto ld8 = [](const typename T::elem* p) -> typename T::pack8 {
    if constexpr (COH && !T::is32) return fh_load16<true>(p);
    else return T::load8(p);
  };
  const int row_ = run * (nthr / LPQ) + threadIdx.x / LPQ, part = threadIdx.x % LPQ;
  unsigned touched[2] = {0u, 0u};
  auto touch = [&]() {
    if constexpr (TOUCH) {
      fmt_touch(pf, lin & 7, (lin >> 3) * nthr + threadIdx.x, (nwg >> 3) * nthr, touched);
    }
  };
  if (row_ >= M) {
    touch();
    if constexpr (TOUCH) fmt_touch_retire(touched);
    return;
  }
  const int b = row_ / ntok, qi = row_ - b * ntok;
  const int d0 = h * HD + part * PD;
  const float scale = rsqrtf((float)HD);
  typedef typename T::elem E;
  typedef typename T::pack8 P8;
  const E* base = reinterpret_cast<const E*>(qkv) + (size_t)(b * ntok) * ld + d0;
  float qf[PD], o[PD];
#pragma unroll
  for (int u = 0; u < NU; ++u) {
    const P8 uu = ld8(base + (size_t)qi * ld + u * 8);
#pragma unroll
    for (int j = 0; j < 8; ++j) qf[u * 8 + j] = T::get(uu, j) * scale;
  }
#pragma unroll
  for (int i = 0; i < PD; ++i) o[i] = 0.f;
  float m = -INFINITY, l = 0.f;
  auto fold = [&](const P8* k, const P8* v, bool valid) {
    float dot = 0.f;
#pragma unroll
    for (int u = 0; u < NU; ++u) {
#pragma unroll
      for (int j = 0; j < 8; ++j) dot += qf[u * 8 + j] * T::get(k[u], j);
    }
#pragma unroll
    for (int d = 1; d < LPQ; d <<= 1) dot += __shfl_xor(dot, d, 64);
    if (!valid) return;
    const float mn = fmaxf(m, dot);
    const float alpha = __expf(m - mn), p = __expf(dot - mn);
    l = l * alpha + p;
    m = mn;
#pragma unroll
    for (int u = 0; u < NU; ++u) {
#pragma unroll
      for (int j = 0; j < 8; ++j) o[u * 8 + j] = o[u * 8 + j] * alpha + p * T::get(v[u], j);
    }
  };
  if (window <= 2) {
    P8 kk[5][NU], vv[5][NU];
#pragma unroll
    for (int t = 0; t < 5; ++t) {
      const int kj = min(max(qi + t - 2, 0), ntok - 1);
      const E* kp = base + (size_t)kj * ld + D;
#pragma unroll
      for (int u = 0; u < NU; ++u) {
        kk[t][u] = ld8(kp + u * 8);
        vv[t][u] = ld8(kp + D + u * 8);
      }
    }
    touch();
#pragma unroll
    for (int t = 0; t < 5; ++t) {
      const int kj = qi + t - 2;
      const bool valid = kj >= 0 && kj < ntok && (t - 2 >= -window) && (t - 2 <= window);
      fold(kk[t], vv[t], valid);
    }
  } else {
    touch();
    for (int kj = qi - window; kj <= qi + window; ++kj) {
      const int kc = min(max(kj, 0), ntok - 1);
      const E* kp = base + (size_t)kc * ld + D;
      P8 k[NU], v[NU];
#pragma unroll
      for (int u = 0; u < NU; ++u) {
        k[u] = ld8(kp + u * 8);
        v[u] = ld8(kp + D + u * 8);
      }
      fold(k, v, kj >= 0 && kj < ntok);
    }
  }
  const float inv = 1.f / l;
  const int row = b * ntok + qi;
  unsigned rm = 0u;
#pragma unroll
  for (int u = 0; u < NU; ++u) {
    P8 uo;
#pragma unroll
    for (int j = 0; j < 8; ++j) T::set(uo, j, o[u * 8 + j] * inv);
    fh_track_pack<T>(rm, uo);
    T::template store8_wt<fh_site<COH>(2), WT>(reinterpret_cast<E*>(out) + fmt_pack_off(row, d0 + u * 8, D / 32), uo);
  }
  fh_range_flush<T>(sat, rm);
  if constexpr (TOUCH) fmt_touch_retire(touched);
}

template <class T, int LPQ, bool TOUCH, bool WT>
__global__ __launch_bounds__(512) void fmt_attn_kernel(const u16* __restrict__ qkv, int ld, u16* __restrict__ out, int ntok,
                                                       int M, int D, int window, TouchSpec pf, unsigned long long* sat) {
  fmt_attn_body<T, LPQ, TOUCH, WT, false>(qkv, ld, out, ntok, M, D, window, pf, sat, blockIdx.x, blockIdx.y, blockDim.x,
                                          blockIdx.x + gridDim.x * blockIdx.y, gridDim.x * gridDim.y);
}

__device__ __forceinline__ float fh_sum8_dpp(float v) {
  v += __builtin_bit_cast(float, __builtin_amdgcn_mov_dpp(__builtin_bit_cast(int, v), 0xB1, 0xF, 0xF, true));
  v += __builtin_bit_cast(float, __builtin_amdgcn_mov_dpp(__builtin_bit_cast(int, v), 0x4E, 0xF, 0xF, true));
  v += __builtin_bit_cast(float, __builtin_amdgcn_mov_dpp(__builtin_bit_cast(int, v), 0x141, 0xF, 0xF, true));
  return v;
}

template <class T, int MTW, int HPW >
__global__ __launch_bounds__(512) void fmt_attnproj_kernel(const u16* __restrict__ qkv, int ld, GemmArgs g, int ntok, int D, int window) {
  constexpr int HD = 128, LPQ = 8, NU = HD / (LPQ * 8), KBH = HD / 32, NWV = 8, ROWS = MTW * 16;
  constexpr int NCT = NWV / HPW;
  constexpr int NPAIR = ROWS * HPW, NPASS = (NPAIR * LPQ + NWV * 64 - 1) / (NWV * 64);
  typedef typename T::elem E;
  typedef typename T::pack8 P8;
  __shared__ __attribute__((aligned(16))) E sO[HPW * MTW * KBH * 512];
  __shared__ __attribute__((aligned(16))) float sR[(HPW > 1 ? (HPW - 1) : 1) * NCT * MTW * 256];
  const int lane = threadIdx.x & 63, w = threadIdx.x >> 6, r16 = lane & 15, q4 = lane >> 4;
  const int ct = w % NCT, hh = w / NCT;
  int ks, bx, by;
  {
    const int id = blockIdx.x, nbn = g.N / (NCT * 16), nbx = nbn * g.ksplit;
    if ((nbx & 7) == 0 && (8 % g.ksplit) == 0) {
      const int slot = id >> 3, P = 8 / g.ksplit, x = id & 7;
      by = slot % g.mblk;
      ks = x / P;
      bx = (slot / g.mblk) * P + (x % P);
    } else {
      const int bxl = id % nbx;
      by = id / nbx;
      ks = bxl / nbn;
      bx = bxl - ks * nbn;
    }
  }
  const int KB = g.K >> 5;
  const int h0 = ks * HPW;
  const int nt = bx * NCT + ct;
  const E* Wp = reinterpret_cast<const E*>(g.W) + ((size_t)nt * KB + (h0 + hh) * KBH) * 512 + lane * 8;
  P8 b[KBH];
#pragma unroll
  for (int kk = 0; kk < KBH; ++kk) b[kk] = T::load8_nt(Wp + (size_t)kk * 512);

  const float scale = rsqrtf((float)HD);
  unsigned rm = 0u;
#pragma unroll
  for (int pass = 0; pass < NPASS; ++pass) {
    const int pair = pass * (NWV * 64 / LPQ) + threadIdx.x / LPQ, part = threadIdx.x % LPQ;
    if (pair < NPAIR) {
      const int ah = pair / ROWS, qslot = pair - ah * ROWS;
      const int row_ = by * ROWS + qslot;
      P8 uo[NU];
#pragma unroll
      for (int u = 0; u < NU; ++u) uo[u] = T::zero8();
      if (row_ < g.M) {
        const int bq = row_ / ntok, qi = row_ - bq * ntok;
        const E* base = reinterpret_cast<const E*>(qkv) + (size_t)(bq * ntok) * ld + (h0 + ah) * HD + part * 8;
        float qf[NU * 8], o[NU * 8];
        P8 qq[NU];
#pragma unroll
        for (int u = 0; u < NU; ++u) qq[u] = T::load8(base + (size_t)qi * ld + u * 64);
#pragma unroll
        for (int i = 0; i < NU * 8; ++i) o[i] = 0.f;
        float l = 0.f;
        auto dotk = [&](const P8* k) {
          float dot = 0.f;
#pragma unroll
          for (int u = 0; u < NU; ++u) {
#pragma unroll
            for (int j = 0; j < 8; ++j) dot += qf[u * 8 + j] * T::get(k[u], j);
          }
          return fh_sum8_dpp(dot);
        };
        if (window <= 2) {
          P8 kk[5][NU], vv[5][NU];
#pragma unroll
          for (int t = 0; t < 5; ++t) {
            const int kj = min(max(qi + t - 2, 0), ntok - 1);
            const E* kp = base + (size_t)kj * ld + D;
#pragma unroll
            for (int u = 0; u < NU; ++u) {
              kk[t][u] = T::load8(kp + u * 64);
              vv[t][u] = T::load8(kp + D + u * 64);
            }
          }
#pragma unroll
          for (int u = 0; u < NU; ++u) {
#pragma unroll
            for (int j = 0; j < 8; ++j) qf[u * 8 + j] = T::get(qq[u], j) * scale;
          }
          float dot[5], m = -INFINITY;
#pragma unroll
          for (int t = 0; t < 5; ++t) {
            const int kj = qi + t - 2;
            const bool valid = kj >= 0 && kj < ntok && (t - 2 >= -window) && (t - 2 <= window);
            dot[t] = valid ? dotk(kk[t]) : -INFINITY;
            m = fmaxf(m, dot[t]);
          }
#pragma unroll
          for (int t = 0; t < 5; ++t) {
            const float p = __expf(dot[t] - m);
            l += p;
#pragma unroll
            for (int u = 0; u < NU; ++u) {
#pragma unroll
              for (int j = 0; j < 8; ++j) o[u * 8 + j] += p * T::get(vv[t][u], j);
            }
          }
        } else {
#pragma unroll
          for (int u = 0; u < NU; ++u) {
#pragma unroll
            for (int j = 0; j < 8; ++j) qf[u * 8 + j] = T::get(qq[u], j) * scale;
          }
          float m = -INFINITY;
          for (int kj = max(qi - window, 0); kj <= min(qi + window, ntok - 1); ++kj) {
            const E* kp = base + (size_t)kj * ld + D;
            P8 k[NU], v[NU];
#pragma unroll
            for (int u = 0; u < NU; ++u) {
              k[u] = T::load8(kp + u * 64);
              v[u] = T::load8(kp + D + u * 64);
            }
            const float dot = dotk(k);
            const float mn = fmaxf(m, dot);
            const float alpha = __expf(m - mn), p = __expf(dot - mn);
            l = l * alpha + p;
            m = mn;
#pragma unroll
            for (int u = 0; u < NU; ++u) {
#pragma unroll
              for (int j = 0; j < 8; ++j) o[u * 8 + j] = o[u * 8 + j] * alpha + p * T::get(v[u], j);
            }
          }
        }
        const float inv = 1.f / l;
#pragma unroll
        for (int u = 0; u < NU; ++u) {
#pragma unroll
          for (int j = 0; j < 8; ++j) T::set(uo[u], j, o[u * 8 + j] * inv);
          fh_track_pack<T>(rm, uo[u]);
        }
      }
#pragma unroll
      for (int u = 0; u < NU; ++u) T::store8(sO + ah * (MTW * KBH * 512) + fmt_pack_off(qslot, u * 64 + part * 8, KBH), uo[u]);
    }
  }
  fh_range_flush<T>(g.sat, rm);
  __syncthreads();

  f32x4 acc[MTW];
#pragma unroll
  for (int i = 0; i < MTW; ++i) acc[i] = f32x4{0.f, 0.f, 0.f, 0.f};
  const E* const sOh = sO + hh * (MTW * KBH * 512);
#pragma unroll
  for (int kk = 0; kk < KBH; ++kk) {
#pragma unroll
    for (int i = 0; i < MTW; ++i) acc[i] = T::mfma(b[kk], T::load8(sOh + (i * KBH + kk) * 512 + lane * 8), acc[i]);
  }
  if constexpr (HPW > 1) {
    if (hh > 0) {
#pragma unroll
      for (int i = 0; i < MTW; ++i) *reinterpret_cast<f32x4*>(sR + (((hh - 1) * NCT + ct) * MTW + i) * 256 + lane * 4) = acc[i];
    }
    __syncthreads();
    if (hh > 0) return;
#pragma unroll
    for (int o = 1; o < HPW; ++o) {
#pragma unroll
      for (int i = 0; i < MTW; ++i) {
        const f32x4 t = *reinterpret_cast<const f32x4*>(sR + (((o - 1) * NCT + ct) * MTW + i) * 256 + lane * 4);
        acc[i] += t;
      }
    }
  }
  float* const outp = g.out_f32 + (size_t)ks * g.slab_stride + nt * 16 + q4 * 4;
#pragma unroll
  for (int i = 0; i < MTW; ++i) {
    const int row = (by * MTW + i) * 16 + r16;
    if (row < g.M) __builtin_nontemporal_store(acc[i], reinterpret_cast<f32x4*>(outp + (size_t)row * g.ldo));
  }
}

enum { MS_XEMBED = 0, MS_LN, MS_QKV, MS_ATTN, MS_PROJ, MS_FC1, MS_FC2, MS_HEAD };
struct MegaStage {
  int kind;
  unsigned nblk;
  GemmArgs g;
  long long gate_off;
  long long shift_off, scale_off, red_gate_off;
  int ks;
  const float* red_bias;
  u16* ln_out;
  int perm;
  TouchSpec pf;
  u16* att_out;
};
struct MegaCtx {
  float* xres;
  const u16* qkv16;
  const float* slab;
  size_t slab_stride;
  int M, D, ntok, ldm, window, heads;
  unsigned long long* sat;
};
struct MegaDyn {
  const float* mod;
  float dt, a, r, e;
  int euler;
  float* vout;
};
struct MegaSync {
  unsigned* grp;
  unsigned* top;
  unsigned* rel;
  unsigned* seq;
  unsigned* err;
  unsigned* err_host;
  unsigned long long* stamps;
  unsigned stamp_wg;
};

__device__ __forceinline__ bool fmt_grid_barrier(const MegaSync& sy, unsigned gen, unsigned nwg) {
  typedef __attribute__((address_space(1))) unsigned int gu32;
  const unsigned g = blockIdx.x & 7u, per = nwg >> 3;
  const unsigned old = __hip_atomic_fetch_add((gu32*)(sy.grp + g * 32), 1u, __ATOMIC_RELAXED, __HIP_MEMORY_SCOPE_AGENT);
  if (old + 1u == gen * per) {
    const unsigned t = __hip_atomic_fetch_add((gu32*)sy.top, 1u, __ATOMIC_RELAXED, __HIP_MEMORY_SCOPE_AGENT);
    if (t + 1u == gen * 8u) {
#pragma unroll
      for (int i = 0; i < 8; ++i) __hip_atomic_store((gu32*)(sy.rel + i * 32), gen, __ATOMIC_RELAXED, __HIP_MEMORY_SCOPE_AGENT);
    }
  }
  unsigned spins = 0;
  while ((int)(__hip_atomic_load((gu32*)(sy.rel + g * 32), __ATOMIC_RELAXED, __HIP_MEMORY_SCOPE_AGENT) - gen) < 0) {
    if (++spins > (1u << 18) || ((spins & 63u) == 0u && __hip_atomic_load((gu32*)sy.err, __ATOMIC_RELAXED, __HIP_MEMORY_SCOPE_AGENT) != 0u)) {
      __hip_atomic_store((gu32*)sy.err, 1u, __ATOMIC_RELAXED, __HIP_MEMORY_SCOPE_AGENT);
      if (sy.err_host) __hip_atomic_store((gu32*)sy.err_host, 1u, __ATOMIC_RELAXED, __HIP_MEMORY_SCOPE_SYSTEM);
      return false;
    }
    __builtin_amdgcn_s_sleep(1);
  }
  return true;
}

template <class T>
__global__ __launch_bounds__(512) void fmt_mega_kernel(const MegaStage* __restrict__ tab, int nstage, MegaDyn d, MegaCtx c,
                                                       MegaSync sy) {
  typedef __attribute__((address_space(1))) unsigned int gu32;
  __shared__ unsigned s_flag[2];
  const unsigned bid = blockIdx.x, nwg = gridDim.x;
  if (threadIdx.x == 0) {
    s_flag[0] = __hip_atomic_load((gu32*)sy.seq, __ATOMIC_RELAXED, __HIP_MEMORY_SCOPE_AGENT);
    s_flag[1] = 1u;
  }
  __syncthreads();
  const unsigned seq0 = s_flag[0];
  const unsigned gen0 = seq0 * (unsigned)(nstage - 1);
#ifdef MEGA_STAMPS
#define MEGA_STAMP(k) do { if (sy.stamps && bid == sy.stamp_wg && threadIdx.x == 0) sy.stamps[s * 3 + (k)] = __builtin_amdgcn_s_memrealtime(); } while (0)
#else
#define MEGA_STAMP(k) do { } while (0)
#endif
  for (int s = 0; s < nstage; ++s) {
    const MegaStage& st = tab[s];
    MEGA_STAMP(0);
    if (bid < st.nblk) {
      switch (st.kind) {
        case MS_XEMBED:
          fmt_gemm_body<T, 4, 1, 8, EPI_XEMBED, true>(st.g, bid, st.nblk);
          break;
        case MS_LN:
          if (threadIdx.x < 64) {
            const LnRed red{c.slab, c.slab_stride, st.red_bias, d.mod + st.red_gate_off};
            if (st.ks == 0)
              fmt_lnmod_body<T, 4, 0, true, true, true>(c.xres, c.M, d.mod + st.shift_off, d.mod + st.scale_off, c.ldm, st.ln_out, red,
                                                        st.pf, c.ntok, st.perm, c.sat, bid, st.nblk, 1);
            else
              fmt_lnmod_body<T, 4, 4, true, true, true>(c.xres, c.M, d.mod + st.shift_off, d.mod + st.scale_off, c.ldm, st.ln_out, red,
                                                        st.pf, c.ntok, st.perm, c.sat, bid, st.nblk, 1);
          }
          break;
        case MS_QKV:
          fmt_gemm_body<T, 3, 4, 8, EPI_T16, true>(st.g, bid, st.nblk);
          break;
        case MS_ATTN:
          if (threadIdx.x < 128)
            fmt_attn_body<T, 16, true, true, true>(c.qkv16, 3 * c.D, st.att_out, c.ntok, c.M, c.D, c.window, st.pf, c.sat,
                                                   (int)(bid % (unsigned)c.heads), (int)(bid / (unsigned)c.heads), 128, bid, st.nblk);
          break;
        case MS_PROJ: {
          GemmArgs g = st.g;
          g.gate = d.mod + st.gate_off;
          fmt_gemm_body<T, 3, 1, 8, EPI_GATE_RES, true>(g, bid, st.nblk);
          break;
        }
        case MS_FC1:
          fmt_gemm_body<T, 3, 4, 8, EPI_GELU_P16, true>(st.g, bid, st.nblk);
          break;
        case MS_FC2:
          fmt_gemm_body<T, 3, 4, 8, EPI_PARTIAL, true>(st.g, bid, st.nblk);
          break;
        default: {
          GemmArgs g = st.g;
          g.a_cfg = d.a;
          g.r_cfg = d.r;
          g.e_cfg = d.e;
          g.dt = d.dt;
          if (!d.euler) {
            g.xcur = nullptr;
            g.xin16 = nullptr;
            g.vout = d.vout;
          }
          fmt_gemm_body<T, 3, 1, 8, EPI_CFG, true>(g, bid, st.nblk);
          break;
        }
      }
    }
    MEGA_STAMP(1);
    if (s + 1 < nstage) {
      asm volatile("s_waitcnt vmcnt(0)" ::: "memory");
      __syncthreads();
      MEGA_STAMP(2);
      if (threadIdx.x == 0) {
        int pre = 0;
#pragma unroll
        for (int i = 0; i < (int)(sizeof(MegaStage) + 63) / 64; ++i) pre ^= reinterpret_cast<const int*>(&tab[s + 1])[i * 16];
        asm volatile("" ::"s"(pre));
        if (!fmt_grid_barrier(sy, gen0 + (unsigned)s + 1u, nwg)) s_flag[1] = 0u;
      }
      __syncthreads();
      if (s_flag[1] == 0u) return;
    }
  }
  if (bid == 0 && threadIdx.x == 0) __hip_atomic_store((gu32*)sy.seq, seq0 + 1u, __ATOMIC_RELAXED, __HIP_MEMORY_SCOPE_AGENT);
}

template <class T>
__global__ void fmt_build_cond_kernel(u16* __restrict__ out, int ld, int bc, int ntok, int n_prev, int dim_w, int dim_a,
                                      int dim_e, const float* __restrict__ wr, const float* __restrict__ wa,
                                      const float* __restrict__ prev_wa, const float* __restrict__ we, int we_len,
                                      const float* __restrict__ prev_we, unsigned wr_mask, unsigned wa_mask,
                                      unsigned we_mask, unsigned long long* sat) {
  const int row = blockIdx.x;
  const int s = row / ntok, i = row % ntok, q = s / bc, b = s - q * bc, n_cur = ntok - n_prev;
  const bool on_r = (wr_mask >> b) & 1, on_a = (wa_mask >> b) & 1, on_e = (we_mask >> b) & 1;
  wr += (size_t)q * dim_w;
  wa += (size_t)q * n_cur * dim_a;
  prev_wa += (size_t)q * n_prev * dim_a;
  we += (size_t)q * we_len * dim_e;
  if (prev_we) prev_we += (size_t)q * n_prev * dim_e;
  unsigned rm = 0u;
  for (int c = threadIdx.x; c < ld; c += blockDim.x) {
    float v = 0.f;
    if (c < dim_w) {
      v = on_r ? wr[c] : 0.f;
    } else if (c < dim_w + dim_a) {
      const int k = c - dim_w;
      if (i < n_prev) v = prev_wa[i * dim_a + k];
      else if (on_a) v = wa[(i - n_prev) * dim_a + k];
    } else if (c < dim_w + dim_a + dim_e) {
      const int k = c - dim_w - dim_a;
      if (on_e) {
        if (we_len == 1) v = we[k];
        else v = (i < n_prev) ? prev_we[i * dim_e + k] : we[(i - n_prev) * dim_e + k];
      }
    }
    reinterpret_cast<typename T::elem*>(out)[fmt_pack_off(row, c, ld / 32)] = fh_cvt<T>(v, rm);
  }
  fh_range_flush<T>(sat, rm);
}

__device__ __forceinline__ float fmt_linspace01(int i, int n) {
  if (n <= 1) return 0.f;
  const float step = __fdiv_rn(1.0f, (float)(n - 1));
  return (i < n / 2) ? __fmul_rn(step, (float)i) : __fsub_rn(1.0f, __fmul_rn(step, (float)(n - 1 - i)));
}
template <class T>
__global__ void fmt_tsin_kernel(u16* __restrict__ out, const float* __restrict__ freqs, int n_steps, float t0, int nfe,
                                int stages, float c0, float c1, float c2, float c3) {
  const int s = blockIdx.x;
  if (s >= n_steps) return;
  float t = t0;
  if (nfe > 0) {
    const int i = s / stages, j = s - i * stages;
    const float gi = fmt_linspace01(i, nfe);
    t = gi;
    if (j > 0) {
      const float cj = j == 1 ? c1 : (j == 2 ? c2 : c3);
      t = __fadd_rn(gi, __fmul_rn(__fsub_rn(fmt_linspace01(i + 1, nfe), gi), cj));
    }
  }
  (void)c0;
  const int k = threadIdx.x;
  const float arg = t * freqs[k & 127];
  reinterpret_cast<typename T::elem*>(out)[fmt_pack_off(s, k, 8)] = T::from_float(k < 128 ? cosf(arg) : sinf(arg));
}

template <class T>
__global__ void fmt_silu_c_kernel(u16* __restrict__ out, const float* __restrict__ temb, const float* __restrict__ ccond,
                                  int M, int D, size_t step_stride, int dense_rows, unsigned long long* sat) {
  const int idx = (blockIdx.x * blockDim.x + threadIdx.x) * 8;
  if (idx >= M * D) return;
  const int c = idx % D, row = idx / D + (int)blockIdx.y * dense_rows;
  typename T::elem* const o = reinterpret_cast<typename T::elem*>(out) + (dense_rows ? (size_t)0 : (size_t)blockIdx.y * step_stride);
  temb += (size_t)blockIdx.y * D;
  typename T::pack8 u;
#pragma unroll
  for (int h = 0; h < 2; ++h) {
    const float4 a = *reinterpret_cast<const float4*>(ccond + idx + 4 * h);
    const float4 t = *reinterpret_cast<const float4*>(temb + c + 4 * h);
    T::set(u, 4 * h + 0, fh_silu(a.x + t.x));
    T::set(u, 4 * h + 1, fh_silu(a.y + t.y));
    T::set(u, 4 * h + 2, fh_silu(a.z + t.z));
    T::set(u, 4 * h + 3, fh_silu(a.w + t.w));
  }
  unsigned rm = 0u;
  fh_track_pack<T>(rm, u);
  fh_range_flush<T>(sat, rm);
  T::store8(o + fmt_pack_off(row, c, D / 32), u);
}

template <class T>
__global__ void fmt_init_x_kernel(float* __restrict__ xcur, u16* __restrict__ xin16, int ldx, const float* __restrict__ x0,
                                  const float* __restrict__ prev_x, int n_prev, int n_cur, int dim_w, int nclip,
                                  unsigned long long* sat) {
  const int idx = blockIdx.x * blockDim.x + threadIdx.x;
  const int ntok = n_prev + n_cur;
  if (idx >= nclip * ntok * dim_w) return;
  const int q = idx / (ntok * dim_w), r = idx - q * ntok * dim_w;
  const int i = r / dim_w, c = r % dim_w;
  float v;
  if (i < n_prev) {
    v = prev_x[((size_t)q * n_prev + i) * dim_w + c];
  } else {
    v = x0[((size_t)q * n_cur + (i - n_prev)) * dim_w + c];
    xcur[((size_t)q * n_cur + (i - n_prev)) * dim_w + c] = v;
  }
  unsigned rm = 0u;
  reinterpret_cast<typename T::elem*>(xin16)[fmt_pack_off(q * ntok + i, c, ldx)] = fh_cvt<T>(v, rm);
  fh_range_flush<T>(sat, rm);
}

template <class T>
__global__ void fmt_rk_combine_kernel(float* __restrict__ xcur, const float* __restrict__ kbuf, size_t kstride, int nk, float c0,
                                      float c1, float c2, float c3, int final, u16* __restrict__ xin16, int ldx, int n_prev,
                                      int n_cur, int W, int nclip, unsigned long long* sat) {
  const int idx = blockIdx.x * blockDim.x + threadIdx.x;
  if (idx >= nclip * n_cur * W) return;
  const int q = idx / (n_cur * W), r = idx - q * n_cur * W;
  const int i = r / W, c = r % W, ntok = n_prev + n_cur;
  const float cf[4] = {c0, c1, c2, c3};
  float y = xcur[idx];
  for (int m = 0; m < nk; ++m) y += cf[m] * kbuf[(size_t)m * kstride + ((size_t)q * ntok + n_prev + i) * W + c];
  if (final) xcur[idx] = y;
  unsigned rm = 0u;
  reinterpret_cast<typename T::elem*>(xin16)[fmt_pack_off(q * ntok + n_prev + i, c, ldx)] = fh_cvt<T>(y, rm);
  fh_range_flush<T>(sat, rm);
}

__global__ void fmt_slice_pad_kernel(float* __restrict__ dst, const float* __restrict__ src, int t0, int T, int n, int dim,
                                     int nclip) {
  const int idx = blockIdx.x * blockDim.x + threadIdx.x;
  if (idx >= nclip * n * dim) return;
  const int q = idx / (n * dim), r = idx - q * n * dim;
  const int i = r / dim, c = r % dim;
  const int t = min(t0 + i, T - 1);
  dst[idx] = src[((size_t)q * T + t) * dim + c];
}

__global__ void fmt_tail_kernel(float* __restrict__ dst, const float* __restrict__ src, int n_prev, int n_cur, int dim, int nclip) {
  const int idx = blockIdx.x * blockDim.x + threadIdx.x;
  if (idx >= nclip * n_prev * dim) return;
  const int q = idx / (n_prev * dim), r = idx - q * n_prev * dim;
  dst[idx] = src[((size_t)q * n_cur + (n_cur - n_prev)) * dim + r];
}

constexpr int kFmtMaxClips = 16;
template <class P>
struct FmtClipTab {
  P p[kFmtMaxClips];
  int T[kFmtMaxClips];
};

__global__ void fmt_gather_pad_kernel(float* __restrict__ dst, const FmtClipTab<const float*> src, int t0, int n, int dim) {
  const int r = blockIdx.x * blockDim.x + threadIdx.x, q = blockIdx.y;
  if (r >= n * dim) return;
  const int i = r / dim, c = r - i * dim;
  const int t = min(t0 + i, src.T[q] - 1);
  dst[(size_t)q * n * dim + r] = src.p[q][(size_t)t * dim + c];
}

__global__ void fmt_scatter_trim_kernel(const FmtClipTab<float*> dst, const float* __restrict__ src, int t0, int n, int dim) {
  const int r = blockIdx.x * blockDim.x + threadIdx.x, q = blockIdx.y;
  if (r >= n * dim) return;
  const int i = r / dim, c = r - i * dim;
  if (t0 + i >= dst.T[q]) return;
  dst.p[q][(size_t)(t0 + i) * dim + c] = src[(size_t)q * n * dim + r];
}

template <class T>
__global__ void fmt_dbg_to16_kernel(u16* __restrict__ dst, const float* __restrict__ src, int n) {
  const int i = blockIdx.x * blockDim.x + threadIdx.x;
  if (i < n) reinterpret_cast<typename T::elem*>(dst)[i] = T::from_float(src[i]);
}
template <class T>
__global__ void fmt_dbg_unpack_kernel(float* __restrict__ dst, const u16* __restrict__ src, int rows, int D) {
  const int i = blockIdx.x * blockDim.x + threadIdx.x;
  if (i >= rows * D) return;
  const int r = i / D, c = i - r * D;
  dst[i] = T::to_float(reinterpret_cast<const typename T::elem*>(src)[fmt_pack_off(r, c, D / 32)]);
}

__global__ void fmt_copy_kernel(float* __restrict__ dst, size_t dpitch, const float* __restrict__ src, size_t spitch, int width, int rows) {
  const int idx = blockIdx.x * blockDim.x + threadIdx.x;
  if (idx >= rows * width) return;
  const int r = idx / width, c = idx - r * width;
  dst[(size_t)r * dpitch + c] = src ? src[(size_t)r * spitch + c] : 0.f;
}
```

### comfyui-float_optimized_amd/csrc/fmt_launch.hpp

```cpp
#pragma once
#include <type_traits>

#include "fmt_weights.hpp"

namespace {

constexpr int kLdsMax = 160 * 1024;
constexpr int kWtRows = 256;

typedef void (*GemmKernel)(GemmArgs);

template <class K>
void raise_lds(K kern, int bytes) {
  if (hipFuncSetAttribute(reinterpret_cast<const void*>(kern), hipFuncAttributeMaxDynamicSharedMemorySize, bytes) != hipSuccess)
    (void)hipGetLastError();
}

template <int... Vs, class F>
bool with_const(int v, F&& f) {
  return ((v == Vs && (f(std::integral_constant<int, Vs>{}), true)) || ...);
}

struct FmtLaunch {
  const FmtTune& tn;
  hipStream_t s;
  unsigned long long* sat;
  float *xres, *slab;
  u16 *h16, *qkv16, *att16;
  int D, ntok, Ntot, Mpad, heads, attn_window;
};


template <int MTW, int NT>
struct Tile {};
template <class T, int EPI, int NW, class F, int... MTW, int... NT>
void gemm_tiles(F& f, Tile<MTW, NT>...) {
  (f(fmt_gemm_kernel<T, MTW, NT, NW, EPI>, MTW, NT, NW, NW * MTW * 16 * NT * 16 * (int)sizeof(float)), ...);
}
template <class T, int EPI, int NW, class F>
void gemm_split_tiles(F& f) {
  gemm_tiles<T, EPI, NW>(f, Tile<3, 1>{}, Tile<3, 2>{}, Tile<3, 4>{}, Tile<5, 1>{}, Tile<5, 2>{}, Tile<5, 4>{}, Tile<4, 1>{},
                         Tile<4, 2>{}, Tile<6, 2>{}, Tile<2, 1>{}, Tile<1, 1>{});
}
template <class T, int EPI, class F>
void for_each_gemm(F&& f) {
  if constexpr (T::is32) {
    gemm_tiles<T, EPI, 4>(f, Tile<1, 1>{}, Tile<2, 1>{}, Tile<3, 1>{}, Tile<4, 1>{}, Tile<5, 1>{});
    if constexpr (EPI == EPI_CFG) gemm_tiles<T, EPI, 8>(f, Tile<1, 1>{}, Tile<3, 1>{}, Tile<4, 1>{});
  } else {
    gemm_split_tiles<T, EPI, 4>(f);
    gemm_split_tiles<T, EPI, 8>(f);
    gemm_split_tiles<T, EPI, 16>(f);
    if constexpr (EPI == EPI_F32 || EPI == EPI_CFG) {
      gemm_tiles<T, EPI, 4>(f, Tile<12, 2>{}, Tile<15, 2>{}, Tile<12, 1>{}, Tile<15, 1>{});
      gemm_tiles<T, EPI, 8>(f, Tile<12, 1>{}, Tile<15, 1>{});
    }
  }
}
template <int MTW, int KCH, int NWV>
struct WideTile {};
template <class T, class F, int... MTW, int... KCH, int... NWV>
void wide_tiles(F& f, WideTile<MTW, KCH, NWV>...) {
  (f(fmt_gemm_wide_kernel<T, MTW, KCH, NWV>, MTW, KCH, NWV, 2 * MTW * KCH * 1024), ...);
}
template <class T, class F>
void for_each_wide(F&& f) {
  wide_tiles<T>(f, WideTile<4, 4, 4>{}, WideTile<5, 4, 4>{}, WideTile<6, 4, 4>{}, WideTile<6, 2, 4>{}, WideTile<12, 2, 4>{},
                WideTile<12, 4, 4>{}, WideTile<12, 2, 8>{}, WideTile<12, 4, 8>{});
}
template <class T, int NWC, int NS, int STG, class F>
void dma_tile(F& f) {
  f(fmt_gemm_dma_kernel<T, NWC, NS, STG>, NWC, NS, STG, NS * (12 + 5 * NWC) * 1024);
}
template <class T, class F>
void for_each_dma(F&& f) {
  dma_tile<T, 4, 4, 0>(f);
  dma_tile<T, 4, 4, 1>(f);
}
template <class T, int EPI, int MI, int NJ, int KPS, int NS, class F>
void rbs_tile(F& f, int shape) {
  f(fmt_gemm_rbs_kernel<T, MI, NJ, KPS, NS, EPI>, shape, 32 * MI, 32 * NJ, KPS, fmt_rb_smem(MI, NJ, KPS, NS));
}
template <class T, int EPI, class F>
void for_each_rbs(F&& f) {
  rbs_tile<T, EPI, 3, 2, 2, 4>(f, 0);
  rbs_tile<T, EPI, 3, 4, 2, 4>(f, 1);
  rbs_tile<T, EPI, 6, 4, 2, 3>(f, 2);
}

constexpr int kBigSmem = 4 * 28 * 1024 + 4 * 4096;
constexpr int kMegaWgs = 256, kMegaSmem = 8 * 48 * 64 * 4;

template <class T>
void prime_kernels() {
  auto raise = [](GemmKernel kern, int, int, int, int smem) {
    if (smem <= kLdsMax) raise_lds(kern, smem);
  };
  for_each_gemm<T, EPI_F32>(raise);
  for_each_gemm<T, EPI_T16>(raise);
  for_each_gemm<T, EPI_SILU_P16>(raise);
  for_each_gemm<T, EPI_GELU_P16>(raise);
  for_each_gemm<T, EPI_GATE_RES>(raise);
  for_each_gemm<T, EPI_XEMBED>(raise);
  for_each_gemm<T, EPI_CFG>(raise);
  for_each_gemm<T, EPI_PARTIAL>(raise);
  for_each_gemm<T, EPI_GELUERF_P16>(raise);
  if constexpr (!T::is32) {
    auto raise_rb = [](GemmKernel kern, int, int, int, int, int smem) { raise_lds(kern, smem); };
    raise_lds(fmt_gemm_big4_kernel<T, 4>, kBigSmem);
    for_each_dma<T>(raise);
    for_each_wide<T>(raise);
    for_each_rbs<T, EPI_T16>(raise_rb);
    for_each_rbs<T, EPI_GELU_P16>(raise_rb);
    for_each_rbs<T, EPI_PARTIAL>(raise_rb);
    raise_lds(fmt_mega_kernel<T>, kMegaSmem);
  }
}


template <class T>
int launch_wide_tile(GemmArgs g, int mtw, int kch, int nwv, hipStream_t s) {
  GemmKernel kern = nullptr;
  int smem = 0;
  for_each_wide<T>([&](GemmKernel k, int m, int c, int w, int bytes) {
    if (m == mtw && c == kch && w == nwv) kern = k, smem = bytes;
  });
  FH_REQUIRE(kern, "no wide GEMM tiling (%d row tiles, %d k-blocks per chunk, %d waves)", mtw, kch, nwv);
  const int mt_total = (g.M + 15) / 16;
  g.mblk = (mt_total + mtw - 1) / mtw;
  g.ksplit = 1;
  const dim3 grid((g.N / 128) * g.mblk * (g.zcount > 1 ? g.zcount : 1));
  fh_launch_prof(2, kern, grid, dim3(nwv * 64), smem, s, g);
  FH_CHECK_HIP(hipGetLastError());
  return FLOAT_OK;
}
template <class T>
int launch_dma(GemmArgs g, int nwc, int ns, int stg, hipStream_t s) {
  GemmKernel kern = nullptr;
  int smem = 0;
  for_each_dma<T>([&](GemmKernel k, int c, int n, int st, int bytes) {
    if (c == nwc && n == ns && st == stg) kern = k, smem = bytes;
  });
  FH_REQUIRE(kern, "no LDS-DMA GEMM tile (%d wave columns, ring of %d, stagger %d)", nwc, ns, stg);
  g.mblk = ((g.M + 15) / 16 + 11) / 12;
  const dim3 grid((g.N / (80 * nwc)) * g.mblk * (g.zcount > 1 ? g.zcount : 1));
  fh_launch_prof(2, kern, grid, dim3(nwc * 128), smem, s, g);
  FH_CHECK_HIP(hipGetLastError());
  return FLOAT_OK;
}
bool dma_shape_ok(const GemmArgs& g, int bn) { return g.N % bn == 0 && g.K % 64 == 0 && g.K >= 128; }

constexpr int kBigMinRows = 1536;
bool big_shape_ok(const FmtTune& tn, int rows_total, int N, int K, int n_cu) {
  return tn.big && rows_total >= kBigMinRows && N % 2048 == 0 && K % 64 == 0 && K >= 128 && n_cu >= 8;
}
template <class T>
int launch_big4(const u16* A, const FmtLin& L, float* out, int rows_total, int ldo, int n_cu, hipStream_t s) {
  if constexpr (T::is32) {
    fh_set_error("the fp32 verification mode has no persistent projection kernel");
    return FLOAT_E_INVALID;
  } else {
    BigArgs g{A, L.W, L.b, out, rows_total, L.N, L.K, ldo, (rows_total + 191) / 192, L.N / 256};
    const dim3 grid((unsigned)((n_cu / 8) * 8));
    fh_launch_prof(2, fmt_gemm_big4_kernel<T, 4>, grid, dim3(256), kBigSmem, s, g);
    FH_CHECK_HIP(hipGetLastError());
    return FLOAT_OK;
  }
}

template <class T>
int launch_wide(const GemmArgs& g, int variant, hipStream_t s) {
  const int mt = (g.M + 15) / 16;
  if ((variant == 6 || variant == 7) && mt > 4 && dma_shape_ok(g, 320)) return launch_dma<T>(g, 4, 4, variant == 7 ? 1 : 0, s);
  if (mt <= 4) return launch_wide_tile<T>(g, 4, 4, 4, s);
  if (variant == 6 || variant == 7) variant = 2;
  static const int by_variant[6][3] = {{6, 4, 4}, {6, 2, 4}, {12, 2, 4}, {12, 4, 4}, {12, 2, 8}, {12, 4, 8}};
  if (mt <= 12 || variant == 2 || variant >= 4) {
    const int* t = by_variant[variant >= 1 && variant <= 5 ? variant : 0];
    return launch_wide_tile<T>(g, t[0], t[1], t[2], s);
  }
  return launch_wide_tile<T>(g, 5, 4, 4, s);
}

template <class T, int EPI>
int launch_gemm(GemmArgs g, int mtw, int nt, int nw, hipStream_t s) {
  FH_REQUIRE(g.N % (nt * 16) == 0 && g.K % (32 * nw * ((EPI == EPI_PARTIAL && g.ksplit > 1) ? g.ksplit : 1)) == 0,
             "gemm shape N=%d K=%d not tileable by %d columns / %d waves", g.N, g.K, nt * 16, nw);
  GemmKernel kern = nullptr;
  int smem = 0;
  for_each_gemm<T, EPI>([&](GemmKernel k, int m, int n, int w, int bytes) {
    if (m == mtw && n == nt && w == nw) kern = k, smem = bytes;
  });
  FH_REQUIRE(kern, "no GEMM tiling (%d x %d tiles, %d waves) for epilogue %d", mtw, nt, nw, EPI);
  FH_REQUIRE(smem <= kLdsMax, "GEMM tiling %dx%d tiles with %d waves needs %d B of LDS", mtw, nt, nw, smem);
  const int mt_total = (g.M + 15) / 16;
  g.mblk = (mt_total + mtw - 1) / mtw;
  if (EPI != EPI_PARTIAL || g.ksplit < 1) g.ksplit = 1;
  dim3 grid((g.N / (nt * 16)) * g.mblk * g.ksplit);
  fh_launch_prof(0, kern, grid, dim3(nw * 64), smem, s, g);
  FH_CHECK_HIP(hipGetLastError());
  return FLOAT_OK;
}

template <class T, int EPI>
int launch_rbs(GemmArgs g, int shape, hipStream_t s) {
  if constexpr (T::is32) {
    fh_set_error("the fp32 verification mode has no row-blocked tiling");
    return FLOAT_E_INVALID;
  } else {
    GemmKernel kern = nullptr;
    int rows = 0, bn = 0, kps = 0, smem = 0;
    const int want = (shape == 0 || shape == 1) ? shape : 2;
    for_each_rbs<T, EPI>([&](GemmKernel k, int sh, int r, int c, int kp, int bytes) {
      if (sh == want) kern = k, rows = r, bn = c, kps = kp, smem = bytes;
    });
    if (EPI != EPI_PARTIAL || g.ksplit < 1) g.ksplit = 1;
    FH_REQUIRE(g.N % bn == 0 && (g.K / 32) % (g.ksplit * kps) == 0 && g.K / 32 / g.ksplit / kps >= 1,
               "row-blocked GEMM: N=%d K=%d not tileable by %d columns / %d K slices of %d-k-block stages", g.N, g.K, bn, g.ksplit, kps);
    g.mblk = (g.M + rows - 1) / rows;
    g.touch.W = nullptr;
    const dim3 grid((unsigned)((g.N / bn) * g.mblk * g.ksplit));
    fh_launch_prof(3, kern, grid, dim3(512), smem, s, g);
    FH_CHECK_HIP(hipGetLastError());
    return FLOAT_OK;
  }
}
constexpr int kRbMinRows = 300;
struct RbPlan {
  int shape = -1, ksplit = 1;
};
RbPlan pick_rb(const FmtTune& tn, int layer, int M) {
  RbPlan p;
  if (!tn.rb || M < kRbMinRows) return p;
  const int tier = M < 540 ? 0 : (M < 1100 ? 1 : (M < 2200 ? 2 : 3));
  static const int shapes[4][4] = { {0, 1, 0, 2},  {-1, 0, 0, 2},  {0, 1, 2, 2},  {0, 1, 2, 2}};
  p.shape = shapes[layer][tier];
  p.ksplit = layer == RB_PROJ ? 2 : (layer == RB_FC2 ? (tier == 3 ? 2 : 4) : 1);
  const FmtTune::Rb& o = tn.rb_layer[layer];
  if (o.n >= 1) {
    p.shape = o.shape;
    const int ks = o.ksplit;
    if (o.n >= 2 && (layer == RB_PROJ || layer == RB_FC2) && (ks == 1 || ks == 2 || ks == 4 || ks == 8)) p.ksplit = ks;
  }
  return p;
}

struct Tiling {
  int mtw, nt, nw;
};
int pick_nw(int K, int forced) {
  const int KB = K / 32;
  if (forced && KB % forced == 0) return forced;
  if (KB >= 128 && KB % 16 == 0) return 16;
  if (KB >= 32 && KB % 8 == 0) return 8;
  return 4;
}
Tiling pick_tiling(const FmtTune& tn, int M, int N, int K, bool need_full_rows) {
  const int mt = (M + 15) / 16;
  if (need_full_rows) {
    if (mt <= 4) return {4, 1, pick_nw(K, 0)};
    return {mt <= 12 ? 12 : 15, 1, (tn.full_nw == 8 && (K / 32) % 8 == 0) ? 8 : 4};
  }
  int split = mt <= 4 ? 4 : (mt <= 12 ? 3 : 5);
  if (mt <= 2) split = mt;
  const int blocks = (mt + split - 1) / split;
  const bool wide = N >= 16384;
  if (mt >= 12) {
    const int* o = tn.plan + (wide ? 3 : 0);
    if (o[0]) {
      int nw = o[0] >= 12 ? 4 : pick_nw(K, o[2]);
      while (nw > 4 && nw * o[0] * 16 * o[1] * 16 * 4 > kLdsMax) nw >>= 1;
      return {o[0], o[1], nw};
    }
  }
  if (wide) return {mt <= 4 ? 4 : 6, 2, std::min(8, pick_nw(K, 0))};
  if (mt > 15 && N % 64 == 0) return {3, 4, 4};
  int nt = 1;
  if (mt >= 5) {
    if ((N / 64) * blocks >= 192 && N % 64 == 0) nt = 4;
    else if ((N / 32) * blocks >= 192 && N % 32 == 0) nt = 2;
  } else if ((N / 16) * blocks > 512) {
    nt = 2;
  }
  return {split, nt, pick_nw(K, 0)};
}
Tiling pick_tiling32(int M) {
  const int mt = (M + 15) / 16;
  return {mt <= 5 ? mt : (mt <= 12 ? 3 : 5), 1, 4};
}

GemmArgs base_args(const u16* A, const Lin& L, int M) {
  GemmArgs g;
  memset(&g, 0, sizeof(g));
  g.A = A, g.W = L.W, g.bias = L.b;
  g.K = L.K, g.N = L.N, g.M = M;
  return g;
}

template <class T, int EPI>
int run_gemm(const FmtTune& tn, GemmArgs g, hipStream_t s, bool need_full_rows = false, const LayerPlan* plan = nullptr) {
  if constexpr (T::is32) {
    FH_REQUIRE(!need_full_rows, "the fp32 mode has no all-rows CFG epilogue tiling (token-blocked head only)");
    const Tiling t = pick_tiling32(g.M);
    g.touch.W = nullptr;
    return launch_gemm<T, EPI>(g, t.mtw, t.nt, t.nw, s);
  }
  if (plan && plan->on() && (g.M + 15) / 16 <= 15) {
    g.touch.W = nullptr;
    return launch_gemm<T, EPI>(g, plan->v[0], plan->v[1], plan->v[2], s);
  }
  const Tiling t = pick_tiling(tn, g.M, g.N, g.K, need_full_rows);
  return launch_gemm<T, EPI>(g, t.mtw, t.nt, t.nw, s);
}

struct PendingRed {
  int ks = 0;
  LnRed red{};
};
void to_slab(GemmArgs& g, float* slab, int Mpad, int ks) {
  g.ksplit = ks, g.out_f32 = slab, g.ldo = g.N, g.slab_stride = (size_t)Mpad * g.N;
}
PendingRed pending_red(float* slab, int Mpad, int D, const float* bias, const float* gate, int ks) {
  return PendingRed{ks, LnRed{slab, (size_t)Mpad * D, bias, gate}};
}
template <class T>
int run_gemm_partial(const FmtLaunch& cx, GemmArgs g, int ksplit, const LayerPlan* plan = nullptr) {
  to_slab(g, cx.slab, cx.Mpad, ksplit);
  if (plan && plan->on() && !T::is32 && (g.M + 15) / 16 <= 15) {
    g.touch.W = nullptr;
    return launch_gemm<T, EPI_PARTIAL>(g, plan->v[0], plan->v[1], plan->v[2], cx.s);
  }
  Tiling t = T::is32 ? pick_tiling32(g.M) : pick_tiling(cx.tn, g.M, g.N * ksplit, g.K / ksplit, false);
  while (t.nt > 1 && g.N % (t.nt * 16)) t.nt >>= 1;
  if (T::is32) g.touch.W = nullptr;
  return launch_gemm<T, EPI_PARTIAL>(g, t.mtw, t.nt, t.nw, cx.s);
}

int log2_exact(unsigned v) {
  int n = 0;
  while ((1u << n) < v) ++n;
  return (1u << n) == v ? n : -1;
}

TouchSpec make_touch(const FmtTune& tn, const Lin& L, int M, int ksplit, unsigned lanes, unsigned per_lane, int force_nt = 0) {
  TouchSpec t{};
  Tiling tl = ksplit ? pick_tiling(tn, M, L.N * ksplit, L.K / ksplit, false) : pick_tiling(tn, M, L.N, L.K, false);
  if (force_nt) tl.nt = force_nt;
  if (ksplit)
    while (tl.nt > 1 && L.N % (tl.nt * 16)) tl.nt >>= 1;
  const int ks = ksplit ? ksplit : 1;
  if (L.N % (tl.nt * 16) || L.K % (32 * ks) || 8 % ks) return t;
  const int nbn = L.N / (tl.nt * 16);
  if ((nbn * ks) % 8) return t;
  const unsigned P = 8 / ks, run_lines = (unsigned)(L.K / 32 / ks) * 8u;
  if (log2_exact(run_lines) < 0 || log2_exact((unsigned)tl.nt) < 0) return t;
  t.run_shift = (unsigned)log2_exact(run_lines);
  t.nt_shift = (unsigned)log2_exact((unsigned)tl.nt);
  t.p_shift = (unsigned)log2_exact(P);
  t.tile_bytes = (unsigned)(L.K / 32) * 1024u;
  t.total = ((unsigned)nbn / P) * (unsigned)tl.nt * run_lines;
  if ((size_t)t.total > (size_t)lanes * per_lane) return t;
  t.W = reinterpret_cast<const char*>(L.W);
  return t;
}

TouchSpec make_touch_rb(const Lin& L, int shape, int kb, unsigned lanes, unsigned per_lane) {
  TouchSpec t{};
  const int ct = shape == 0 ? 4 : 8;
  if (kb <= 0 || (kb & (kb - 1)) || L.N % (ct * 16) || (L.N / (ct * 16)) % 8 || L.K / 32 < kb) return t;
  const unsigned run_lines = (unsigned)kb * 8u;
  t.run_shift = (unsigned)log2_exact(run_lines);
  t.nt_shift = (unsigned)log2_exact((unsigned)ct);
  t.p_shift = 3;
  t.tile_bytes = (unsigned)(L.K / 32) * 1024u;
  t.total = (unsigned)(L.N / (ct * 16) / 8) * (unsigned)ct * run_lines;
  if ((size_t)t.total > (size_t)lanes * per_lane) return t;
  t.W = reinterpret_cast<const char*>(L.W);
  return t;
}

unsigned gemm_lanes_per_xcd(const FmtTune& tn, int M, int N, int K) {
  const Tiling t = pick_tiling(tn, M, N, K, false);
  const int mblk = ((M + 15) / 16 + t.mtw - 1) / t.mtw;
  return (unsigned)((N / (t.nt * 16)) * mblk / 8) * (unsigned)(t.nw * 64);
}


template <class T>
int launch_lnmod(const FmtLaunch& cx, int M, const float* shift, const float* scale, PendingRed* pend = nullptr,
                 const Lin* next = nullptr, u16* out = nullptr, int perm = 0, int touch_bit = 1, int rb_shape = -1) {
  const int rpw = cx.tn.ln_rows;
  dim3 grid(rpw == 1 ? ((M + 63) / 64) * 64 : (M + rpw - 1) / rpw), block(64 * rpw);
  const int ks = pend ? pend->ks : 0;
  const bool wt = M <= kWtRows;
  LnRed red{};
  if (ks) red = pend->red;
  TouchSpec pf{};
  if (next && (cx.tn.touch & (1 | touch_bit)) && rpw == 1 && !T::is32)
    pf = rb_shape >= 0 ? make_touch_rb(*next, rb_shape, cx.tn.rb_touch, (grid.x / 8) * 64, 6)
                       : make_touch(cx.tn, *next, M, 0, (grid.x / 8) * 64, 6);
  decltype(&fmt_lnmod_kernel<T, 1, 0, false, false>) kern = nullptr;
  with_const<1, 2, 4, 8>(cx.D / 256, [&](auto NV) {
    with_const<0, 1, 2, 4, 8>((ks == 0 || ks == 1 || ks == 2 || ks == 4) ? ks : 8, [&](auto KS) {
      with_const<0, 1>(pf.W != nullptr, [&](auto TOUCH) {
        with_const<0, 1>(wt, [&](auto WT) {
          kern = fmt_lnmod_kernel<T, decltype(NV)::value, decltype(KS)::value, decltype(TOUCH)::value != 0, decltype(WT)::value != 0>;
        });
      });
    });
  });
  FH_REQUIRE(kern, "dim_h %d unsupported (must be 256*{1,2,4,8})", cx.D);
  hipLaunchKernelGGL(kern, grid, block, 0, cx.s, cx.xres, M, shift, scale, cx.Ntot, out ? out : cx.h16, red, pf, cx.ntok, perm, cx.sat);
  if (pend) pend->ks = 0;
  FH_CHECK_HIP(hipGetLastError());
  return FLOAT_OK;
}

template <class T>
void launch_attn(const FmtLaunch& cx, int M, const Lin* pull) {
  const int qpw = cx.tn.attn_qpw, lpq = cx.tn.attn_lpq;
  dim3 grid(cx.heads, (M + qpw - 1) / qpw), block(qpw * lpq);
  TouchSpec pf{};
  if (pull && !T::is32) pf = make_touch(cx.tn, *pull, M, 0, (grid.x * grid.y / 8) * block.x, 2);
  decltype(&fmt_attn_kernel<T, 8, false, false>) kern = nullptr;
  with_const<16, 8>(lpq == 16 ? 16 : 8, [&](auto LPQ) {
    with_const<0, 1>(pf.W != nullptr, [&](auto TOUCH) {
      with_const<0, 1>(M <= kWtRows, [&](auto WT) {
        kern = fmt_attn_kernel<T, decltype(LPQ)::value, decltype(TOUCH)::value != 0, decltype(WT)::value != 0>;
      });
    });
  });
  hipLaunchKernelGGL(kern, grid, block, 0, cx.s, cx.qkv16, 3 * cx.D, cx.att16, cx.ntok, M, cx.D, cx.attn_window, pf, cx.sat);
}

int attnproj_hpw(const FmtTune& tn, int D, int heads) {
  const int hpw = tn.attnproj;
  if (hpw <= 0 || D != heads * 128 || heads % hpw) return 0;
  const int ks = heads / hpw;
  return (ks == 1 || ks == 2 || ks == 4 || ks == 8) && (hpw == 1 || hpw == 2) ? hpw : 0;
}
template <class T>
int launch_attnproj(const FmtLaunch& cx, int M, const Lin& proj) {
  const int hpw = attnproj_hpw(cx.tn, cx.D, cx.heads);
  GemmArgs g = base_args(nullptr, proj, M);
  g.sat = cx.sat;
  to_slab(g, cx.slab, cx.Mpad, cx.heads / hpw);
  g.mblk = ((M + 15) / 16 + 2) / 3;
  const dim3 grid((unsigned)(g.ksplit * (g.N / (128 / hpw)) * g.mblk));
  fh_launch_prof(0, hpw == 2 ? fmt_attnproj_kernel<T, 3, 2> : fmt_attnproj_kernel<T, 3, 1>, grid, dim3(512), 0, cx.s, cx.qkv16, 3 * cx.D, g,
                 cx.ntok, cx.D, cx.attn_window);
  FH_CHECK_HIP(hipGetLastError());
  return FLOAT_OK;
}

}
```

### comfyui-float_optimized_amd/csrc/fmt_mega.hpp

```cpp
#pragma once
#include "fmt_launch.hpp"

namespace {

MegaSync mega_sync_of(const float_fmt* h) {
  unsigned* m = h->mega_sync;
  return MegaSync{m, m + 8 * 32, m + 9 * 32, m + 17 * 32, m + 18 * 32, h->mega_err_host, reinterpret_cast<unsigned long long*>(m + 20 * 32), (unsigned)h->tune.mega_stamp_wg};
}
int mega_poll(float_fmt* h) {
  if (!h->mega_err_host || *reinterpret_cast<volatile unsigned*>(h->mega_err_host) == 0u) return FLOAT_OK;
  FH_CHECK_HIP(hipDeviceSynchronize());
  for (auto& gr : h->graphs)
    for (hipGraphExec_t e : gr.exec)
      if (e) (void)hipGraphExecDestroy(e);
  h->graphs.clear();
  if (h->mega_sync) FH_CHECK_HIP(hipMemset(h->mega_sync, 0, (size_t)(32 * 20) * sizeof(unsigned)));
  *reinterpret_cast<volatile unsigned*>(h->mega_err_host) = 0u;
  h->tune.mega = 0;
  h->job.active = false;
  fh_set_error("fmt_mega_kernel: a grid barrier timed out in an earlier call (not all %d workgroups were resident) - the results of "
               "that call are invalid; the handle falls back to the launch chain (FLOAT_FMT_MEGA=0 selects it from the start)", 256);
  return FLOAT_E_HIP;
}
template <class T>
bool mega_shape_ok(const float_fmt* h, int nclip, int bc) {
  const FmtTune& tn = h->tune;
  if (T::is32 || !tn.mega || nclip != 1 || bc != 3 || h->D != 1024 || h->cfg.heads != 8 || h->n_cu < kMegaWgs) return false;
  if (attnproj_hpw(tn, h->D, h->cfg.heads) || tn.fc2_split != 4 || tn.proj_split != 0) return false;
  const int M = bc * h->ntok;
  auto is = [](Tiling t, int a, int b, int c) { return t.mtw == a && t.nt == b && t.nw == c; };
  const Blk& B = h->blk[0];
  return (M + 15) / 16 == 12 && (h->ntok + 15) / 16 == 4 && h->x_embed.K % 256 == 0 && h->final_lin.K % 256 == 0 &&
         is(pick_tiling(tn, M, B.qkv.N, B.qkv.K, false), 3, 4, 8) && is(pick_tiling(tn, M, B.proj.N, B.proj.K, false), 3, 1, 8) &&
         is(pick_tiling(tn, M, B.fc1.N, B.fc1.K, false), 3, 4, 8) && is(pick_tiling(tn, M, B.fc2.N * 4, B.fc2.K / 4, false), 3, 4, 8) &&
         B.fc2.K % 512 == 0;
}

template <class T>
int build_mega(float_fmt* h, int bc) {
  float_fmt::MegaPlan& P = h->mega[bc];
  P.tried = 1;
  {
    int per_cu = 0;
    if (hipOccupancyMaxActiveBlocksPerMultiprocessor(&per_cu, reinterpret_cast<const void*>(fmt_mega_kernel<T>), 512, kMegaSmem) != hipSuccess) {
      (void)hipGetLastError();
      per_cu = 0;
    }
    if (per_cu * h->n_cu < kMegaWgs) {
      h->tune.mega = 0;
      return FLOAT_OK;
    }
  }
  const float_fmt_cfg_t& c = h->cfg;
  const FmtTune& tn = h->tune;
  const int D = h->D, ntok = h->ntok, M = bc * ntok;
  std::vector<MegaStage> st;
  const size_t esz = sizeof(typename T::elem) / sizeof(u16);
  const size_t n_h = (size_t)h->Mpad * D * esz, n_hid = (size_t)h->Mpad * c.mlp_hidden * esz;
  if (!h->mega_ws) {
    int rc0 = h->pool.alloc(&h->mega_ws, (size_t)c.depth * (3 * n_h + n_hid), true);
    if (rc0) return rc0;
  }
  auto ws_h1 = [&](int b) { return h->mega_ws + (size_t)b * (3 * n_h + n_hid); };
  auto ws_h2 = [&](int b) { return ws_h1(b) + n_h; };
  auto ws_att = [&](int b) { return ws_h1(b) + 2 * n_h; };
  auto ws_hid = [&](int b) { return ws_h1(b) + 3 * n_h; };
  auto gemm_stage = [&](int kind, GemmArgs g, int mtw, int nt) {
    MegaStage m;
    memset(&m, 0, sizeof(m));
    m.kind = kind;
    g.sat = h->sat;
    g.mblk = ((g.M + 15) / 16 + mtw - 1) / mtw;
    if (g.ksplit < 1) g.ksplit = 1;
    m.g = g;
    m.nblk = (unsigned)((g.N / (nt * 16)) * g.mblk * g.ksplit);
    return m;
  };
  auto ln_stage = [&](int b_mod, int which, int ks, const float* bias, int gate_col, const Lin* next, int touch_bit, u16* out, int perm) {
    MegaStage m;
    memset(&m, 0, sizeof(m));
    m.kind = MS_LN;
    m.nblk = (unsigned)(((M + 63) / 64) * 64);
    m.shift_off = (long long)b_mod * 6 * D + (long long)which * D;
    m.scale_off = m.shift_off + D;
    m.ks = ks;
    m.red_bias = bias;
    m.red_gate_off = (long long)b_mod * 6 * D + (long long)gate_col * D;
    m.ln_out = out ? out : h->h16;
    m.perm = perm;
    if (next && (tn.touch & (1 | touch_bit))) m.pf = make_touch(tn, *next, M, 0, (m.nblk / 8) * 64, 6);
    return m;
  };
  {
    GemmArgs g = base_args(h->xin16, h->x_embed, ntok);
    g.out_f32 = h->xres;
    g.ldo = D;
    g.pos = h->pos;
    g.bc = bc;
    g.ntok = ntok;
    st.push_back(gemm_stage(MS_XEMBED, g, 4, 1));
  }
  for (int b = 0; b < c.depth; ++b) {
    const Blk& B = h->blk[b];
    if (b == 0) st.push_back(ln_stage(b, 0, 0, nullptr, 0, &B.qkv, 128, ws_h1(b), 0));
    else {
      MegaStage m = ln_stage(b, 0, 4, h->blk[b - 1].fc2.b, 0, &B.qkv, 128, ws_h1(b), 0);
      m.red_gate_off = (long long)(b - 1) * 6 * D + 5LL * D;
      st.push_back(m);
    }
    {
      GemmArgs g = base_args(ws_h1(b), B.qkv, M);
      g.out16 = h->qkv16;
      g.ldo16 = 3 * D;
      if (tn.touch & 8) g.touch = make_touch(tn, B.proj, M, 0, gemm_lanes_per_xcd(tn, M, g.N, g.K), 2);
      st.push_back(gemm_stage(MS_QKV, g, 3, 4));
    }
    {
      MegaStage m;
      memset(&m, 0, sizeof(m));
      m.kind = MS_ATTN;
      m.nblk = (unsigned)(c.heads * ((M + 7) / 8));
      if (tn.touch & 2) m.pf = make_touch(tn, B.proj, M, 0, (m.nblk / 8) * 128, 2);
      m.att_out = ws_att(b);
      st.push_back(m);
    }
    {
      GemmArgs g = base_args(ws_att(b), B.proj, M);
      g.out_f32 = h->xres;
      g.ldo = D;
      g.ldg = h->Ntot;
      if (tn.touch & 16) g.touch = make_touch(tn, B.fc1, M, 0, gemm_lanes_per_xcd(tn, M, g.N, g.K), 2);
      MegaStage m = gemm_stage(MS_PROJ, g, 3, 1);
      m.gate_off = (long long)b * 6 * D + 2LL * D;
      st.push_back(m);
    }
    st.push_back(ln_stage(b, 3, 0, nullptr, 0, &B.fc1, 64, ws_h2(b), 0));
    {
      GemmArgs g = base_args(ws_h2(b), B.fc1, M);
      g.out16 = ws_hid(b);
      g.ldo16 = B.fc2.K / 32;
      if (tn.touch & 4) g.touch = make_touch(tn, B.fc2, M, 4, gemm_lanes_per_xcd(tn, M, g.N, g.K), 2);
      st.push_back(gemm_stage(MS_FC1, g, 3, 4));
    }
    {
      GemmArgs g = base_args(ws_hid(b), B.fc2, M);
      to_slab(g, h->slab, h->Mpad, 4);
      if (tn.touch & 32) {
        const unsigned lanes = gemm_lanes_per_xcd(tn, M, g.N * 4, g.K / 4);
        if (b + 1 < c.depth) g.touch = make_touch(tn, h->blk[b + 1].qkv, M, 0, lanes, 2);
        else g.touch = make_touch(tn, h->final_lin, M, 0, lanes, 2, 1);
      }
      st.push_back(gemm_stage(MS_FC2, g, 3, 4));
    }
  }
  {
    const int nblk = (ntok + 15) / 16, seqs = bc;
    MegaStage m = ln_stage(c.depth, 0, 4, h->blk[c.depth - 1].fc2.b, 0, nullptr, 0, h->hfin16, seqs * 16);
    m.red_gate_off = (long long)(c.depth - 1) * 6 * D + 5LL * D;
    st.push_back(m);
    GemmArgs g = base_args(h->hfin16, h->final_lin, nblk * seqs * 16);
    g.tokblk = 1;
    g.nclip = 1;
    g.bc = bc;
    g.ntok = ntok;
    g.n_prev = c.n_prev;
    g.xcur = h->xcur;
    g.xin16 = h->xin16;
    g.ldx = h->Kx / 32;
    st.push_back(gemm_stage(MS_HEAD, g, bc, 1));
  }
  for (const MegaStage& m : st) FH_REQUIRE(m.nblk <= (unsigned)kMegaWgs, "persistent kernel: a stage needs %u workgroups", m.nblk);
  int rc;
  if (!h->mega_sync && (rc = h->pool.alloc(&h->mega_sync, 32 * 20 + 2 * 3 * 64, true))) return rc;
  if (!h->mega_err_host) {
    FH_CHECK_HIP(hipHostMalloc(reinterpret_cast<void**>(&h->mega_err_host), 64, hipHostMallocMapped));
    memset(h->mega_err_host, 0, 64);
  }
  if ((rc = h->pool.alloc(&P.dev, st.size(), false))) return rc;
  FH_CHECK_HIP(hipMemcpy(P.dev, st.data(), st.size() * sizeof(MegaStage), hipMemcpyHostToDevice));
  P.nstage = (int)st.size();
  P.bc = bc;
  P.ctx = MegaCtx{h->xres, h->qkv16, h->slab, (size_t)h->Mpad * D, M, D, ntok, h->Ntot, c.attn_window, c.heads, h->sat};
  return FLOAT_OK;
}

template <class T>
int run_mega(float_fmt* h, int bc, const float* modbuf, bool euler, float dt, float a, float r, float e, hipStream_t s, float* vout_to) {
  float_fmt::MegaPlan& P = h->mega[bc];
  MegaDyn d{modbuf, dt, a, r, e, euler ? 1 : 0, vout_to ? vout_to : h->vout};
  fh_launch_prof(0, (fmt_mega_kernel<T>), dim3(kMegaWgs), dim3(512), kMegaSmem, s, P.dev, P.nstage, d, P.ctx, mega_sync_of(h));
  FH_CHECK_HIP(hipGetLastError());
  return FLOAT_OK;
}

template <class T>
int prepare_mega(float_fmt* h, int bc) {
  if constexpr (T::is32) return FLOAT_OK;
  else return mega_shape_ok<T>(h, 1, bc) ? build_mega<T>(h, bc) : FLOAT_OK;
}

}
```

### comfyui-float_optimized_amd/csrc/fmt_pack.hpp

```cpp
#pragma once
#include "common.hpp"

enum {
  EPI_F32 = 0,
  EPI_T16 = 1,
  EPI_SILU_P16 = 2,
  EPI_GELU_P16 = 3,
  EPI_GATE_RES = 4,
  EPI_XEMBED = 5,
  EPI_CFG = 6,
  EPI_PARTIAL = 7,
  EPI_GELUERF_P16 = 8
};

__host__ __device__ __forceinline__ size_t fmt_pack_off(int row, int k, int KB) {
  return ((size_t)((row >> 4) * KB + (k >> 5)) * 64 + (row & 15) + 16 * ((k >> 3) & 3)) * 8 + (k & 7);
}

struct TouchSpec {
  const char* W;
  unsigned run_shift;
  unsigned nt_shift;
  unsigned p_shift;
  unsigned tile_bytes;
  unsigned total;
};

__device__ __forceinline__ unsigned fmt_touch_line(const TouchSpec& t, unsigned xcd, unsigned l) {
  if (l >= t.total) return 0u;
  const unsigned r = l >> t.run_shift, off = l & ((1u << t.run_shift) - 1u);
  const unsigned cb = r >> t.nt_shift, jn = r & ((1u << t.nt_shift) - 1u);
  const unsigned ks = xcd >> t.p_shift, bx = (cb << t.p_shift) + (xcd & ((1u << t.p_shift) - 1u));
  return *reinterpret_cast<const unsigned*>(t.W + (size_t)((bx << t.nt_shift) + jn) * t.tile_bytes +
                                            ((size_t)((ks << t.run_shift) + off) << 7));
}
template <int N>
__device__ __forceinline__ void fmt_touch(const TouchSpec& t, unsigned xcd, unsigned first, unsigned stride, unsigned (&v)[N]) {
#pragma unroll
  for (int i = 0; i < N; ++i) v[i] = fmt_touch_line(t, xcd, first + (unsigned)i * stride);
}
template <int N>
__device__ __forceinline__ void fmt_touch_retire(const unsigned (&v)[N]) {
  unsigned o = 0u;
#pragma unroll
  for (int i = 0; i < N; ++i) o |= v[i];
  asm volatile("" ::"v"(o));
}

struct GemmArgs {
  const u16* A;
  const u16* W;
  const float* bias;
  int K, M, N;
  int mblk;
  float* out_f32;
  int ldo;
  u16* out16;
  int ldo16;
  const float* gate;
  int ldg;
  const float* pos;
  int bc, ntok, n_prev;
  int nclip;
  float a_cfg, r_cfg, e_cfg, dt;
  float* vout;
  float* xcur;
  u16* xin16;
  int ldx;
  int ksplit;
  size_t slab_stride;
  TouchSpec touch;
  int zcount, zgroup;
  size_t a_zstride, o_zstride;
  int tokblk;
  unsigned long long* sat;
};
```

### comfyui-float_optimized_amd/csrc/tuning.hpp

```cpp
#pragma once
#include <stdio.h>
#include <stdlib.h>
#include <string.h>

#include <algorithm>
#include <string>

inline int env_int(const char* name, int dflt, int lo, int hi) {
  const char* v = getenv(name);
  if (!v || !*v) return dflt;
  char* end = nullptr;
  const long x = strtol(v, &end, 10);
  return (end && *end == 0 && x >= lo && x <= hi) ? (int)x : dflt;
}
inline int env_atoi(const char* name, int dflt) {
  const char* v = getenv(name);
  return v ? atoi(v) : dflt;
}
inline bool env_set(const char* name) { return getenv(name) != nullptr; }
inline int env_scan(const char* s, int* v) { int n = 0; return sscanf(s, "%d%n", v, &n) == 1 ? n : 0; }
inline int env_scan(const char* s, double* v) { int n = 0; return sscanf(s, "%lf%n", v, &n) == 1 ? n : 0; }
template <class V>
int env_list(const char* name, V* v, int n, char sep = ',') {
  const char* s = getenv(name);
  int got = 0;
  while (s && got < n) {
    const int used = env_scan(s, v + got);
    if (!used) break;
    ++got;
    s += used;
    if (sep == ',' && *s++ != ',') break;
  }
  return got;
}

struct LayerPlan {
  int v[3] = {0, 0, 0};
  bool on() const { return v[0] > 0; }
};

enum { RB_QKV = 0, RB_PROJ, RB_FC1, RB_FC2 };

struct FmtTune {
  bool wide = true;
  int wide_variant = 7;
  bool big = true;
  bool rb = true;
  int rb_touch = 16;
  struct Rb {
    int n = 0, shape = -1, ksplit = 1;
  } rb_layer[4];
  int full_nw = 8;
  int plan[6] = {0, 0, 0, 0, 0, 0};
  LayerPlan plan_layer[4];
  int fc2_split = 4;
  int proj_split = 0;
  int touch = 230;
  bool hoist = true;
  int zgroup = 0;
  int ln_rows = 1;
  int attn_qpw = 8, attn_lpq = 16;
  bool no_tokblk = false;
  int attnproj = 0;
  int mega = 0;
  int mega_stamp_wg = 0;
  bool pack_host = false;

  static FmtTune from_env() {
    FmtTune t;
    t.wide = env_atoi("FLOAT_FMT_WIDE", 1) != 0;
    t.wide_variant = env_atoi("FLOAT_FMT_WIDE_VARIANT", t.wide_variant);
    t.big = env_atoi("FLOAT_FMT_BIG", 1) != 0;
    t.rb = env_atoi("FLOAT_FMT_RB", 1) != 0;
    t.rb_touch = env_atoi("FLOAT_FMT_RB_TOUCH", t.rb_touch);
    static const char* const layers[4] = {"QKV", "PROJ", "FC1", "FC2"};
    for (int l = 0; l < 4; ++l) {
      const std::string s = layers[l];
      int rb[2] = {-1, 1};
      t.rb_layer[l].n = env_list(("FLOAT_FMT_RB_" + s).c_str(), rb, 2);
      t.rb_layer[l].shape = rb[0];
      t.rb_layer[l].ksplit = rb[1];
      env_list(("FLOAT_FMT_PLAN_" + s).c_str(), t.plan_layer[l].v, 3);
    }
    t.full_nw = env_atoi("FLOAT_FMT_FULL_NW", t.full_nw);
    env_list("FLOAT_FMT_PLAN", t.plan, 6);
    t.fc2_split = env_atoi("FLOAT_FMT_FC2_SPLIT", t.fc2_split);
    t.proj_split = env_atoi("FLOAT_FMT_PROJ_SPLIT", t.proj_split);
    t.touch = env_atoi("FLOAT_FMT_TOUCH", t.touch);
    t.hoist = env_atoi("FLOAT_FMT_HOIST", 1) != 0;
    t.zgroup = std::max(0, env_atoi("FLOAT_FMT_ZGROUP", 0));
    t.ln_rows = std::max(1, std::min(4, env_atoi("FLOAT_FMT_LN_ROWS", 1)));
    int attn[2] = {t.attn_qpw, t.attn_lpq};
    env_list("FLOAT_FMT_ATTN", attn, 2);
    t.attn_lpq = attn[1] == 16 ? 16 : 8;
    t.attn_qpw = std::max(1, std::min(512 / t.attn_lpq, attn[0]));
    t.no_tokblk = env_set("FLOAT_FMT_NO_TOKBLK");
    t.attnproj = env_atoi("FLOAT_FMT_ATTNPROJ", 0);
    t.mega = env_atoi("FLOAT_FMT_MEGA", 0);
    t.mega_stamp_wg = env_atoi("FLOAT_FMT_MEGA_STAMP_WG", 0);
    t.pack_host = env_atoi("FLOAT_PACK_HOST", 0) != 0;
    return t;
  }
};

struct DecTune {
  int lds_pad = 0;
  unsigned ride_wgs = 16;
  int ride_min_res = 64;
  unsigned ride_pace = 3;
  bool ride_equal = false;
  double ride_w[4][3] = {{170, 140, 50}, {170, 155, 100}, {220, 200, 180}, {300, 250, 120}};
  int ride_tail = 0;
#ifdef DEC_STAMPS
  int ride_test = 0;
#endif
  bool cb_order = true;
  int conv_bn = 64, conv_bn_lo = 32;
  int tpw = 0;
  int conv_db = 0;
  bool no_zfuse = false;
  int zblur_min = 64;
  int flow_pix = 0;
  int flow_wgs = 2048;
  bool flow_epi = true;
  bool yuv_fused = true;
  bool write_pyr = false;
  bool copy_memcpy = false;
  bool short_first = true;
  bool style_norm = true;

  static DecTune from_env() {
    DecTune t;
    t.lds_pad = env_int("FLOAT_DEC_LDS_PAD", 0, 0, 160 * 1024);
    t.ride_wgs = (unsigned)env_int("FLOAT_DEC_RIDE_WGS", 16, 0, 64) / 8 * 8;
    t.ride_min_res = env_int("FLOAT_DEC_RIDE_MIN_RES", 64, 64, 512);
    t.ride_pace = (unsigned)env_int("FLOAT_DEC_RIDE_PACE", 3, 0, 64);
    t.ride_equal = env_set("FLOAT_DEC_RIDE_EQUAL");
    double w[12];
    if (env_list("FLOAT_DEC_RIDE_W", w, 12, ' ') == 12)
      for (int i = 0; i < 12; ++i)
        if (w[i] > 0.0 && w[i] < 1e6) t.ride_w[i / 3][i % 3] = w[i];
    t.ride_tail = env_atoi("FLOAT_DEC_RIDE_TAIL", 0);
#ifdef DEC_STAMPS
    t.ride_test = env_int("FLOAT_DEC_RIDE_TEST", 0, 0, 2);
#endif
    t.cb_order = env_atoi("FLOAT_DEC_CB_ORDER", 1) != 0;
    t.conv_bn = env_int("FLOAT_DEC_CONV_BN", 64, 32, 64);
    t.conv_bn_lo = env_int("FLOAT_DEC_CONV_BN_LO", 32, 32, 64);
    t.tpw = env_int("FLOAT_DEC_TPW", 0, 0, 4096);
    t.conv_db = env_int("FLOAT_DEC_CONV_DB", 0, 0, 3);
    t.no_zfuse = env_set("FLOAT_DEC_NO_ZFUSE");
    t.zblur_min = env_int("FLOAT_DEC_ZBLUR_MIN", 64, 16, 4096);
    t.flow_pix = env_int("FLOAT_DEC_FLOW_PIX", 0, 0, 4);
    t.flow_wgs = env_int("FLOAT_DEC_FLOW_WGS", 2048, 8, 1 << 20);
    t.flow_epi = env_int("FLOAT_DEC_FLOW_EPI", 1, 0, 1) != 0;
    t.yuv_fused = env_int("FLOAT_DEC_YUV_FUSED", 1, 0, 1) != 0;
    t.write_pyr = env_set("FLOAT_DEC_WRITE_PYR");
    const char* copy = getenv("FLOAT_DEC_COPY");
    t.copy_memcpy = copy && !strcmp(copy, "memcpy");
    t.short_first = env_int("FLOAT_DEC_SHORT_FIRST", 1, 0, 1) != 0;
    t.style_norm = env_int("FLOAT_DEC_STYLE_NORM", 1, 0, 1) != 0;
    return t;
  }
};

struct EncTune {
  bool no_tiles = false;
  static EncTune from_env() { return EncTune{env_set("FLOAT_ENC_NO_TILES")}; }
};

struct AudTune {
  bool attn_mfma = true;
  static AudTune from_env() { return AudTune{env_atoi("FLOAT_AUD_ATTN_MFMA", 1) != 0}; }
};
```

Before: 2384 frames/s.

## Deduplicate adaLN modulation rows shared across CFG branches via a row map

Adds a ModMap that collapses modulation rows which are identical across CFG branches and across current-window tokens into one shared row per group. The adaLN modulation GEMM then runs on fewer rows, and the layernorm-modulate, gate-residual epilogues and the persistent mega kernel look up each row's modulation through an index remap. The goal is less modulation GEMM work and smaller modulation buffers, paid for with extra integer index math in hot epilogues. By default the map only turns on when more than one clip is batched, and it also moves the residual loads ahead of the shift/scale loads in the layernorm kernel.

```diff
diff --git a/comfyui-float_optimized_amd/csrc/fmt_api.hip b/comfyui-float_optimized_amd/csrc/fmt_api.hip
--- a/comfyui-float_optimized_amd/csrc/fmt_api.hip
+++ b/comfyui-float_optimized_amd/csrc/fmt_api.hip
@@ -50,6 +50,7 @@
   size_t mod_zs = 0;
   struct GraphKey {
     int nfe, bc, we_len, method;
+    int modrows;
     int prio;
     float a, r, e;
     bool operator==(const GraphKey& o) const { return memcmp(this, &o, sizeof(GraphKey)) == 0; }
@@ -93,9 +94,9 @@
 int dev_zero(float* dst, size_t n, hipStream_t s) { return dev_copy2d(dst, n, nullptr, n, (int)n, 1, s); }
 int copy_or_zero(float* dst, const float* src, size_t n, hipStream_t s) { return src ? dev_copy(dst, src, n, s) : dev_zero(dst, n, s); }
 
-FmtLaunch launch_ctx(const float_fmt* h, hipStream_t s) {
+FmtLaunch launch_ctx(const float_fmt* h, hipStream_t s, const ModMap& mm = ModMap{}) {
   return FmtLaunch{h->tune, s, h->sat, h->xres, h->slab, h->h16, h->qkv16, h->att16, h->D, h->ntok, h->Ntot, h->Mpad, h->cfg.heads,
-                   h->cfg.attn_window};
+                   h->cfg.attn_window, mm};
 }
 
 
@@ -111,15 +112,16 @@
 }
 
 template <class T>
-int run_mod_all(float_fmt* h, int M, int e0, int n, hipStream_t s) {
-  const int D = h->D;
+int run_mod_all(float_fmt* h, const ModMap& mm, int nclip, int e0, int n, hipStream_t s) {
+  const int D = h->D, M = nclip * (int)mm.rpc;
+  FH_REQUIRE(M >= 1 && M <= h->Mmod, "%d modulation rows (the workspace holds %d)", M, h->Mmod);
   const FmtTune& tn = h->tune;
   FH_REQUIRE(n >= 1 && n <= kScSteps, "modulation batch of %d evaluations (max %d)", n, kScSteps);
   const int prio = (s == h->cap_stream && s) ? h->cap_prio : stream_priority(s);
   const bool big = !T::is32 && tn.wide && prio == 0 && big_shape_ok(tn, n * M, h->adaln_all.N, h->adaln_all.K, h->n_cu);
   hipLaunchKernelGGL((fmt_silu_c_kernel<T>), dim3((M * D / 8 + 255) / 256, n), dim3(256), 0, s, h->sc16, h->temb + (size_t)e0 * D,
-                     h->ccond, M, D, (size_t)h->Mpad * D, big ? M : 0, h->sat);
-  h->mod_zs = big ? (size_t)M * h->Ntot : (size_t)h->Mmod * h->Ntot;
+                     h->ccond, M, D, (size_t)h->Mpad * D, big ? M : 0, h->sat, mm);
+  h->mod_zs = (size_t)M * h->Ntot;
   if constexpr (!T::is32) {
     if (big) return launch_big4<T>(h->sc16, h->adaln_all, h->modall, n * M, h->Ntot, h->n_cu, s);
   }
@@ -128,7 +130,7 @@
   const bool dma = (tn.wide_variant == 6 || tn.wide_variant == 7) && (M + 15) / 16 > 4 && dma_shape_ok(g, 320);
   g.zgroup = tn.zgroup > 0 ? tn.zgroup : (dma ? 2 : 4);
   g.a_zstride = (size_t)h->Mpad * D;
-  g.o_zstride = (size_t)h->Mmod * h->Ntot;
+  g.o_zstride = h->mod_zs;
   if constexpr (!T::is32) {
     if (tn.wide && g.N % 128 == 0 && g.K % 128 == 0) return launch_wide<T>(g, tn.wide_variant, s);
   }
@@ -163,7 +165,7 @@
       rc = run_gemm_partial<T>(cx, g, ks);
     } else {
       g.sat = cx.sat, g.out_f32 = cx.xres, g.ldo = cx.D;
-      g.gate = gate, g.ldg = cx.Ntot;
+      g.gate = gate, g.ldg = cx.Ntot, g.mm = cx.mm;
       if (tn.touch & 16) g.touch = make_touch(tn, B.fc1, M, 0, gemm_lanes_per_xcd(tn, M, g.N, g.K), 2);
       rc = run_gemm<T, EPI_GATE_RES>(tn, g, cx.s, false, &tn.plan_layer[RB_PROJ]);
     }
@@ -188,7 +190,7 @@
     rc = run_gemm_partial<T>(cx, g, ks, &tn.plan_layer[RB_FC2]);
   } else {
     g.sat = cx.sat, g.out_f32 = cx.xres, g.ldo = cx.D;
-    g.gate = gate, g.ldg = cx.Ntot;
+    g.gate = gate, g.ldg = cx.Ntot, g.mm = cx.mm;
     rc = run_gemm<T, EPI_GATE_RES>(tn, g, cx.s);
   }
   if (!rc && ks) *pend = pending_red(cx.slab, cx.Mpad, cx.D, B.fc2.b, gate, ks);
@@ -196,16 +198,16 @@
 }
 
 template <class T>
-int run_blocks(float_fmt* h, int nclip, int bc, const float* modbuf, bool euler, float dt, float a, float r, float e, hipStream_t s,
-               float* vout_to = nullptr) {
+int run_blocks(float_fmt* h, int nclip, int bc, const ModMap& mm, const float* modbuf, bool euler, float dt, float a, float r, float e,
+               hipStream_t s, float* vout_to = nullptr) {
   const float_fmt_cfg_t& c = h->cfg;
   const FmtTune& tn = h->tune;
-  const FmtLaunch cx = launch_ctx(h, s);
+  const FmtLaunch cx = launch_ctx(h, s, mm);
   const int D = h->D, ntok = h->ntok, M = nclip * bc * ntok;
   int rc;
   if constexpr (!T::is32) {
     if (bc <= 4 && mega_shape_ok<T>(h, nclip, bc)) {
-      if (h->mega[bc].dev) return run_mega<T>(h, bc, modbuf, euler, dt, a, r, e, s, vout_to);
+      if (h->mega[bc].dev) return run_mega<T>(h, bc, mm, modbuf, euler, dt, a, r, e, s, vout_to);
     }
   }
   {
@@ -297,17 +299,6 @@
   return FLOAT_OK;
 }
 
-struct CfgMode {
-  int bc;
-  unsigned wr_mask, wa_mask, we_mask;
-  int nclip = 1;
-};
-
-CfgMode cfg_mode(float a, float r, float e, int include_r) {
-  if (a == 1.0f && r == 1.0f && e == 1.0f) return {1, 1u, 1u, 1u, 1};
-  if (!include_r) return {3, 0b111u, 0b110u, 0b010u, 1};
-  return {4, 0b1110u, 0b1100u, 0b0100u, 1};
-}
 
 template <class T>
 int stage_window(float_fmt* h, const CfgMode& m, const float* x0, const float* wa, const float* wr, const float* we,
@@ -376,17 +367,17 @@
   const Tableau& tb = tableau(h->method);
   const float_fmt_cfg_t& c = h->cfg;
   const size_t kstride = (size_t)h->Bmax * kMaxTok * c.dim_w;
-  const int n = m.nclip * c.n_cur * c.dim_w, rows = m.nclip * m.bc * h->ntok;
+  const int n = m.nclip * c.n_cur * c.dim_w;
   const int nev = n_evals(h->method, nfe), batch = h->tune.hoist ? kScSteps : 1;
   const bool euler = h->method == FLOAT_ODE_EULER;
   int rc;
   for (int ev = 0; ev < nev; ++ev) {
     const int i = ev / tb.s, j = ev - i * tb.s, z = ev % batch;
     const float dt = ts[i + 1] - ts[i];
-    if (z == 0 && (rc = run_mod_all<T>(h, rows, ev, std::min(batch, nev - ev), s))) return rc;
+    if (z == 0 && (rc = run_mod_all<T>(h, m.mm, m.nclip, ev, std::min(batch, nev - ev), s))) return rc;
     const float* mod = h->modall + (size_t)z * h->mod_zs;
     if (euler) {
-      if ((rc = run_blocks<T>(h, m.nclip, m.bc, mod, true, dt, a, r, e, s))) return rc;
+      if ((rc = run_blocks<T>(h, m.nclip, m.bc, m.mm, mod, true, dt, a, r, e, s))) return rc;
       continue;
     }
     if (j > 0) {
@@ -394,7 +385,7 @@
                          dt * tb.a[j][0], dt * tb.a[j][1], dt * tb.a[j][2], 0.f, 0, h->xin16, h->Kx / 32, c.n_prev, c.n_cur,
                          c.dim_w, m.nclip, h->sat);
     }
-    if ((rc = run_blocks<T>(h, m.nclip, m.bc, mod, false, 0.f, a, r, e, s, h->kbuf + (size_t)j * kstride))) return rc;
+    if ((rc = run_blocks<T>(h, m.nclip, m.bc, m.mm, mod, false, 0.f, a, r, e, s, h->kbuf + (size_t)j * kstride))) return rc;
     if (j == tb.s - 1) {
       hipLaunchKernelGGL((fmt_rk_combine_kernel<T>), dim3((n + 255) / 256), dim3(256), 0, s, h->xcur, h->kbuf, kstride, tb.s,
                          dt * tb.b[0], dt * tb.b[1], dt * tb.b[2], dt * tb.b[3], 1, h->xin16, h->Kx / 32, c.n_prev, c.n_cur,
@@ -422,6 +413,7 @@
   key.method = h->method;
   key.bc = m.bc;
   key.we_len = we_len;
+  key.modrows = h->tune.modrows;
   key.a = a;
   key.r = r;
   key.e = e;
@@ -477,6 +469,7 @@
                 float a, float r, float e, int include_r, hipStream_t s, int nclip = 1) {
   CfgMode m = cfg_mode(a, r, e, include_r);
   m.nclip = nclip;
+  m.mm = make_modmap(h->tune.modrows == 1 || (h->tune.modrows == 2 && nclip > 1), m, we_len, h->ntok, h->cfg.n_prev);
   int rc = check_cfg_rows(h, m);
   if (rc) return rc;
   if ((rc = stage_window<T>(h, m, x0, wa, wr, we, we_len, prev_x, prev_wa, prev_we, s))) return rc;
@@ -499,11 +492,12 @@
   tsp.t = t;
   int rc = prepare_time<T>(h, tsp, 1, s);
   if (rc) return rc;
-  const CfgMode m = cfg_mode(a, r, e, include_r);
+  CfgMode m = cfg_mode(a, r, e, include_r);
+  m.mm = make_modmap(h->tune.modrows == 1, m, we_len, h->ntok, h->cfg.n_prev);
   if ((rc = check_cfg_rows(h, m))) return rc;
   if ((rc = stage_window<T>(h, m, x, wa, wr, we, we_len, prev_x, prev_wa, prev_we, s))) return rc;
-  if ((rc = run_mod_all<T>(h, m.bc * h->ntok, 0, 1, s))) return rc;
-  if ((rc = run_blocks<T>(h, 1, m.bc, h->modall, false, 0.f, a, r, e, s))) return rc;
+  if ((rc = run_mod_all<T>(h, m.mm, 1, 0, 1, s))) return rc;
+  if ((rc = run_blocks<T>(h, 1, m.bc, m.mm, h->modall, false, 0.f, a, r, e, s))) return rc;
   return dev_copy(out, h->vout, (size_t)h->ntok * h->cfg.dim_w, s);
 }
 
diff --git a/comfyui-float_optimized_amd/csrc/fmt_kernels.hpp b/comfyui-float_optimized_amd/csrc/fmt_kernels.hpp
--- a/comfyui-float_optimized_amd/csrc/fmt_kernels.hpp
+++ b/comfyui-float_optimized_amd/csrc/fmt_kernels.hpp
@@ -62,7 +62,7 @@
     const int row = m0 + r, nb = n0 + cg * 8;
     if (r < ROWS && row < g.M) {
       const float* o = g.out_f32 + (size_t)row * g.ldo + nb;
-      const float* gt = g.gate + (size_t)row * g.ldg + nb;
+      const float* gt = g.gate + (size_t)modrow(g.mm, row) * g.ldg + nb;
       res_pf[0] = fh_load_f4<COH>(o);
       res_pf[1] = fh_load_f4<COH>(o + 4);
       gate_pf[0] = fh_load_f4_stream(gt);
@@ -209,7 +209,7 @@
         else T::template store8_wt<fh_site<COH>(8), WT>(o16 + fmt_pack_off(row, nb, g.ldo16), u);
       } else if constexpr (EPI == EPI_GATE_RES) {
         float* o = g.out_f32 + (size_t)row * g.ldo + nb;
-        const float* gt = g.gate + (size_t)row * g.ldg + nb;
+        const float* gt = g.gate + (size_t)modrow(g.mm, row) * g.ldg + nb;
 #pragma unroll
         for (int e = 0; e < 8; e += 4) {
           float4 x, gg;
@@ -604,7 +604,7 @@
 __device__ __forceinline__ void fmt_lnmod_body(float* __restrict__ x, int M, const float* __restrict__ shift,
                                                const float* __restrict__ scale, int ldm, u16* __restrict__ out, const LnRed& red,
                                                const TouchSpec& pf, int ntok, int perm, unsigned long long* sat, const unsigned bid,
-                                               const unsigned nblk, const int wpb) {
+                                               const unsigned nblk, const int wpb, const ModMap& mm) {
   constexpr int D = NV * 256;
   constexpr bool WT = WT_ || COH;
   const int lane = threadIdx.x & 63;
@@ -627,16 +627,17 @@
 #ifdef FMT_DIAG_HOTMOD
   const size_t mrow = 0;
 #else
-  const size_t mrow = (size_t)row;
+  const size_t mrow = (size_t)modrow(mm, row);
 #endif
+  float4 v[NV], a[NV], b[NV];
+  float s = 0.f;
+#pragma unroll
+  for (int i = 0; i < NV; ++i) v[i] = fh_load_f4<COH>(xr + i * 256 + lane * 4);
   const float* sh = shift + mrow * ldm;
   const float* sc = scale + mrow * ldm;
-  float4 v[NV], a[NV], b[NV];
-  float s = 0.f;
 #pragma unroll
   for (int i = 0; i < NV; ++i) {
     const int c = i * 256 + lane * 4;
-    v[i] = fh_load_f4<COH>(xr + c);
     a[i] = fh_load_f4_stream(sh + c);
     b[i] = fh_load_f4_stream(sc + c);
   }
@@ -703,9 +704,10 @@
 template <class T, int NV, int KS, bool TOUCH, bool WT>
 __global__ __launch_bounds__(256) void fmt_lnmod_kernel(float* __restrict__ x, int M, const float* __restrict__ shift,
                                                         const float* __restrict__ scale, int ldm, u16* __restrict__ out,
-                                                        LnRed red, TouchSpec pf, int ntok, int perm, unsigned long long* sat) {
+                                                        LnRed red, TouchSpec pf, int ntok, int perm, unsigned long long* sat,
+                                                        ModMap mm) {
   fmt_lnmod_body<T, NV, KS, TOUCH, WT, false>(x, M, shift, scale, ldm, out, red, pf, ntok, perm, sat, blockIdx.x, gridDim.x,
-                                              (int)(blockDim.x >> 6));
+                                              (int)(blockDim.x >> 6), mm);
 }
 
 template <class T, int LPQ, bool TOUCH, bool WT_, bool COH>
@@ -1029,6 +1031,7 @@
   float dt, a, r, e;
   int euler;
   float* vout;
+  ModMap mm;
 };
 struct MegaSync {
   unsigned* grp;
@@ -1095,10 +1098,10 @@
             const LnRed red{c.slab, c.slab_stride, st.red_bias, d.mod + st.red_gate_off};
             if (st.ks == 0)
               fmt_lnmod_body<T, 4, 0, true, true, true>(c.xres, c.M, d.mod + st.shift_off, d.mod + st.scale_off, c.ldm, st.ln_out, red,
-                                                        st.pf, c.ntok, st.perm, c.sat, bid, st.nblk, 1);
+                                                        st.pf, c.ntok, st.perm, c.sat, bid, st.nblk, 1, d.mm);
             else
               fmt_lnmod_body<T, 4, 4, true, true, true>(c.xres, c.M, d.mod + st.shift_off, d.mod + st.scale_off, c.ldm, st.ln_out, red,
-                                                        st.pf, c.ntok, st.perm, c.sat, bid, st.nblk, 1);
+                                                        st.pf, c.ntok, st.perm, c.sat, bid, st.nblk, 1, d.mm);
           }
           break;
         case MS_QKV:
@@ -1112,6 +1115,7 @@
         case MS_PROJ: {
           GemmArgs g = st.g;
           g.gate = d.mod + st.gate_off;
+          g.mm = d.mm;
           fmt_gemm_body<T, 3, 1, 8, EPI_GATE_RES, true>(g, bid, st.nblk);
           break;
         }
@@ -1219,16 +1223,17 @@
 
 template <class T>
 __global__ void fmt_silu_c_kernel(u16* __restrict__ out, const float* __restrict__ temb, const float* __restrict__ ccond,
-                                  int M, int D, size_t step_stride, int dense_rows, unsigned long long* sat) {
+                                  int M, int D, size_t step_stride, int dense_rows, unsigned long long* sat, ModMap mm) {
   const int idx = (blockIdx.x * blockDim.x + threadIdx.x) * 8;
   if (idx >= M * D) return;
-  const int c = idx % D, row = idx / D + (int)blockIdx.y * dense_rows;
+  const int c = idx % D, d = idx / D, row = d + (int)blockIdx.y * dense_rows;
+  ccond += (size_t)modsrc(mm, d) * D + c;
   typename T::elem* const o = reinterpret_cast<typename T::elem*>(out) + (dense_rows ? (size_t)0 : (size_t)blockIdx.y * step_stride);
   temb += (size_t)blockIdx.y * D;
   typename T::pack8 u;
 #pragma unroll
   for (int h = 0; h < 2; ++h) {
-    const float4 a = *reinterpret_cast<const float4*>(ccond + idx + 4 * h);
+    const float4 a = *reinterpret_cast<const float4*>(ccond + 4 * h);
     const float4 t = *reinterpret_cast<const float4*>(temb + c + 4 * h);
     T::set(u, 4 * h + 0, fh_silu(a.x + t.x));
     T::set(u, 4 * h + 1, fh_silu(a.y + t.y));
diff --git a/comfyui-float_optimized_amd/csrc/fmt_launch.hpp b/comfyui-float_optimized_amd/csrc/fmt_launch.hpp
--- a/comfyui-float_optimized_amd/csrc/fmt_launch.hpp
+++ b/comfyui-float_optimized_amd/csrc/fmt_launch.hpp
@@ -28,6 +28,7 @@
   float *xres, *slab;
   u16 *h16, *qkv16, *att16;
   int D, ntok, Ntot, Mpad, heads, attn_window;
+  ModMap mm{};
 };
 
 
@@ -410,7 +411,7 @@
     });
   });
   FH_REQUIRE(kern, "dim_h %d unsupported (must be 256*{1,2,4,8})", cx.D);
-  hipLaunchKernelGGL(kern, grid, block, 0, cx.s, cx.xres, M, shift, scale, cx.Ntot, out ? out : cx.h16, red, pf, cx.ntok, perm, cx.sat);
+  hipLaunchKernelGGL(kern, grid, block, 0, cx.s, cx.xres, M, shift, scale, cx.Ntot, out ? out : cx.h16, red, pf, cx.ntok, perm, cx.sat, cx.mm);
   if (pend) pend->ks = 0;
   FH_CHECK_HIP(hipGetLastError());
   return FLOAT_OK;
diff --git a/comfyui-float_optimized_amd/csrc/fmt_mega.hpp b/comfyui-float_optimized_amd/csrc/fmt_mega.hpp
--- a/comfyui-float_optimized_amd/csrc/fmt_mega.hpp
+++ b/comfyui-float_optimized_amd/csrc/fmt_mega.hpp
@@ -185,9 +185,10 @@
 }
 
 template <class T>
-int run_mega(float_fmt* h, int bc, const float* modbuf, bool euler, float dt, float a, float r, float e, hipStream_t s, float* vout_to) {
+int run_mega(float_fmt* h, int bc, const ModMap& mm, const float* modbuf, bool euler, float dt, float a, float r, float e, hipStream_t s,
+             float* vout_to) {
   float_fmt::MegaPlan& P = h->mega[bc];
-  MegaDyn d{modbuf, dt, a, r, e, euler ? 1 : 0, vout_to ? vout_to : h->vout};
+  MegaDyn d{modbuf, dt, a, r, e, euler ? 1 : 0, vout_to ? vout_to : h->vout, mm};
   fh_launch_prof(0, (fmt_mega_kernel<T>), dim3(kMegaWgs), dim3(512), kMegaSmem, s, P.dev, P.nstage, d, P.ctx, mega_sync_of(h));
   FH_CHECK_HIP(hipGetLastError());
   return FLOAT_OK;
diff --git a/comfyui-float_optimized_amd/csrc/fmt_modmap.hpp b/comfyui-float_optimized_amd/csrc/fmt_modmap.hpp
--- /dev/null
+++ b/comfyui-float_optimized_amd/csrc/fmt_modmap.hpp
@@ -0,0 +1,120 @@
+#pragma once
+
+#if defined(__HIPCC__) || defined(__CUDACC__)
+#define FMT_MODMAP_HD __host__ __device__ __forceinline__
+#else
+#define FMT_MODMAP_HD inline
+#endif
+
+constexpr int kModMaxBc = 4;
+
+struct ModMap {
+  unsigned bits;
+  unsigned rpc;
+  unsigned mg_clip;
+  unsigned mg_tok;
+  unsigned long long prev16;
+  unsigned long long cur16;
+};
+
+FMT_MODMAP_HD bool modmap_active(const ModMap& m) { return (m.bits & 1u) != 0u; }
+FMT_MODMAP_HD int modmap_bc(const ModMap& m) { return (int)((m.bits >> 1) & 7u); }
+FMT_MODMAP_HD bool modmap_full(const ModMap& m, int b) { return ((m.bits >> (4 + b)) & 1u) != 0u; }
+FMT_MODMAP_HD bool modmap_own(const ModMap& m, int b) { return ((m.bits >> (8 + b)) & 1u) != 0u; }
+FMT_MODMAP_HD int modmap_n_prev(const ModMap& m) { return (int)((m.bits >> 12) & 0xffu); }
+FMT_MODMAP_HD int modmap_ntok(const ModMap& m) { return (int)((m.bits >> 20) & 0xffu); }
+FMT_MODMAP_HD int modmap_prev(const ModMap& m, int b) { return (int)((m.prev16 >> (16 * b)) & 0xffffu); }
+FMT_MODMAP_HD int modmap_cur(const ModMap& m, int b) { return (int)((m.cur16 >> (16 * b)) & 0xffffu); }
+FMT_MODMAP_HD unsigned modmap_div(unsigned n, unsigned magic) { return (unsigned)(((unsigned long long)n * magic) >> 32); }
+
+FMT_MODMAP_HD int modrow(const ModMap& m, int row) {
+  if (!modmap_active(m)) return row;
+  const int ntok = modmap_ntok(m);
+  const int q = (int)modmap_div((unsigned)row, m.mg_clip);
+  const int rem = row - q * (modmap_bc(m) * ntok);
+  const int b = (int)modmap_div((unsigned)rem, m.mg_tok);
+  const int i = rem - b * ntok, j = i - modmap_n_prev(m);
+  const int off = j < 0 ? modmap_prev(m, b) + i : modmap_cur(m, b) + (modmap_full(m, b) ? j : 0);
+  return q * (int)m.rpc + off;
+}
+
+FMT_MODMAP_HD int modsrc(const ModMap& m, int d) {
+  if (!modmap_active(m)) return d;
+  const int rpc = (int)m.rpc, bc = modmap_bc(m), ntok = modmap_ntok(m), n_prev = modmap_n_prev(m);
+  const int q = d / rpc, o = d - q * rpc;
+  int src = 0;
+  for (int b = 0; b < kModMaxBc; ++b) {
+    if (b >= bc) break;
+    const int p = modmap_prev(m, b), c = modmap_cur(m, b);
+    const int nc = modmap_full(m, b) ? ntok - n_prev : 1;
+    if (modmap_own(m, b) && o >= p && o < p + n_prev) src = b * ntok + (o - p);
+    if (o >= c && o < c + nc) src = b * ntok + n_prev + (o - c);
+  }
+  return q * (bc * ntok) + src;
+}
+
+struct CfgMode {
+  int bc;
+  unsigned wr_mask, wa_mask, we_mask;
+  int nclip = 1;
+  ModMap mm{};
+};
+
+inline CfgMode cfg_mode(float a, float r, float e, int include_r) {
+  if (a == 1.0f && r == 1.0f && e == 1.0f) return {1, 1u, 1u, 1u, 1};
+  if (!include_r) return {3, 0b111u, 0b110u, 0b010u, 1};
+  return {4, 0b1110u, 0b1100u, 0b0100u, 1};
+}
+
+inline ModMap make_modmap(bool enable, const CfgMode& cm, int we_len, int ntok, int n_prev) {
+  const int bc = cm.bc;
+  const unsigned wr_mask = cm.wr_mask, wa_mask = cm.wa_mask, we_mask = cm.we_mask;
+  ModMap m{};
+  m.rpc = (unsigned)(bc * ntok);
+  if (!enable || bc <= 1 || bc > kModMaxBc || ntok <= 0 || ntok > 255 || n_prev < 0 || n_prev >= ntok) return m;
+  const int n_cur = ntok - n_prev;
+  auto on = [](unsigned mask, int b) { return (mask >> b) & 1u; };
+  bool shared[kModMaxBc] = {};
+  bool any = false;
+  for (int b = 0; b < bc; ++b) {
+    shared[b] = !on(wa_mask, b) && (!on(we_mask, b) || we_len == 1) && n_cur > 1;
+    any = any || shared[b];
+  }
+  if (!any) return m;
+  int base[kModMaxBc] = {}, prev[kModMaxBc] = {}, cur[kModMaxBc] = {};
+  int next = 0;
+  for (int b = 0; b < bc; ++b) {
+    if (!shared[b]) {
+      m.bits |= (1u << (4 + b)) | (1u << (8 + b));
+      base[b] = prev[b] = next, cur[b] = next + n_prev;
+      next += ntok;
+      continue;
+    }
+    int alias = -1;
+    for (int f = 0; f < bc && n_prev > 0; ++f)
+      if (!shared[f] && on(wr_mask, f) == on(wr_mask, b) && on(we_mask, f) == on(we_mask, b)) {
+        alias = f;
+        break;
+      }
+    if (alias < 0 && n_prev > 0) {
+      m.bits |= 1u << (8 + b);
+      prev[b] = next;
+      next += n_prev;
+    } else {
+      prev[b] = -1 - alias;
+    }
+    cur[b] = next;
+    next += 1;
+  }
+  for (int b = 0; b < bc; ++b)
+    if (prev[b] < 0) prev[b] = n_prev > 0 ? base[-1 - prev[b]] : 0;
+  for (int b = 0; b < bc; ++b) {
+    m.prev16 |= (unsigned long long)(unsigned)prev[b] << (16 * b);
+    m.cur16 |= (unsigned long long)(unsigned)cur[b] << (16 * b);
+  }
+  m.rpc = (unsigned)next;
+  m.bits |= 1u | ((unsigned)bc << 1) | ((unsigned)n_prev << 12) | ((unsigned)ntok << 20);
+  m.mg_clip = (unsigned)((0x100000000ull + (unsigned)(bc * ntok) - 1) / (unsigned)(bc * ntok));
+  m.mg_tok = (unsigned)((0x100000000ull + (unsigned)ntok - 1) / (unsigned)ntok);
+  return m;
+}
diff --git a/comfyui-float_optimized_amd/csrc/fmt_pack.hpp b/comfyui-float_optimized_amd/csrc/fmt_pack.hpp
--- a/comfyui-float_optimized_amd/csrc/fmt_pack.hpp
+++ b/comfyui-float_optimized_amd/csrc/fmt_pack.hpp
@@ -1,5 +1,6 @@
 #pragma once
 #include "common.hpp"
+#include "fmt_modmap.hpp"
 
 enum {
   EPI_F32 = 0,
@@ -74,4 +75,5 @@
   size_t a_zstride, o_zstride;
   int tokblk;
   unsigned long long* sat;
+  ModMap mm;
 };
diff --git a/comfyui-float_optimized_amd/csrc/tuning.hpp b/comfyui-float_optimized_amd/csrc/tuning.hpp
--- a/comfyui-float_optimized_amd/csrc/tuning.hpp
+++ b/comfyui-float_optimized_amd/csrc/tuning.hpp
@@ -57,6 +57,7 @@
   int proj_split = 0;
   int touch = 230;
   bool hoist = true;
+  int modrows = 2;
   int zgroup = 0;
   int ln_rows = 1;
   int attn_qpw = 8, attn_lpq = 16;
@@ -88,6 +89,7 @@
     t.proj_split = env_atoi("FLOAT_FMT_PROJ_SPLIT", t.proj_split);
     t.touch = env_atoi("FLOAT_FMT_TOUCH", t.touch);
     t.hoist = env_atoi("FLOAT_FMT_HOIST", 1) != 0;
+    t.modrows = std::max(0, std::min(2, env_atoi("FLOAT_FMT_MODROWS", t.modrows)));
     t.zgroup = std::max(0, env_atoi("FLOAT_FMT_ZGROUP", 0));
     t.ln_rows = std::max(1, std::min(4, env_atoi("FLOAT_FMT_LN_ROWS", 1)));
     int attn[2] = {t.attn_qpw, t.attn_lpq};
```

After: 2358 frames/s. -1.1%, worse.
